# OpenDriveLab/Vista

Hardware: AMD Instinct MI355X
Metric: denoise steps/sec, 25-frame 576x1024 latent, 50-step EDM @ 1/2/4/8 GPU (higher is better)
Workload: dtype bf16; 1 GPU; 1xMI355X single GPU: 25x576x1024 (latent 25x4x72x128), 50-step EulerEDM, VanillaCFG 2.5 (N=50 images per UNet call), bf16, random-init 1.65B VideoUNet, synthetic latents; frames=25, cfg_images_per_call=50, sampler=EulerEDM s_churn=0, 50-step schedule, parallelism=single GPU

## Files before the change

### include/vista_hip.h

```cpp
#ifndef VISTA_HIP_H
#define VISTA_HIP_H
#include <stdint.h>
#ifdef __cplusplus
extern "C" {
#endif

enum { VK_AMODE_DENSE = 0, VK_AMODE_CONV3X3 = 1, VK_AMODE_TEMPORAL3 = 2, VK_AMODE_CONV3D = 3, VK_AMODE_UPCONV2X2 = 4 };
enum { VK_EPI_LINEAR = 0, VK_EPI_GEGLU = 1, VK_EPI_TRANS = 2 };

typedef struct VkGemmDesc {
    const void* A;
    const void* Wt;
    void* out;
    const float* bias;
    const float* rowvec;
    const void* res1;
    const void* res2;
    int32_t M, N, K;
    int32_t lda, ldc, ld_res1, ld_res2, ldv, rows_per_vec;
    float alpha, beta;
    int32_t amode, epi, out_f32;
    int32_t H, Wd, Cin, Hout, Wout, stride, ups;
    int32_t T, S;
    int32_t tile_cfg;
    const void* halo_prev;
    const void* halo_next;
    void* splitk_ws;
    int64_t splitk_ws_bytes;
    int32_t asym_pad;
    int32_t k_split;
    const void* A2;
    int32_t lda2;
    int32_t ln_parts;
    const float* ln_stats;
    const float* ln_colsum;
    float ln_eps;
    float* rowstat_out;
    const float* rowvec2;
    int32_t act;
    void* mx8_out;
    void* mx8_scales;
    int32_t mx8_cols, ld_mx8, ld_mx8s;
    int32_t m_begin, m_end;
    float* gnstat_out;
    int32_t gn_rows;
    int32_t alt_cols_from;
} VkGemmDesc;

int vk_gemm_bf16(const VkGemmDesc* d, void* stream);

int vk_gemm_rowstat_parts(const VkGemmDesc* d);
int vk_gemm_tile_choice(const VkGemmDesc* d);
int vk_gemm_tail_split(const VkGemmDesc* d);
int vk_gemm_gnstat_fit(const VkGemmDesc* d);

int vk_gemm_fp8(const VkGemmDesc* desc, const float* a_scale, const float* w_scale, int32_t k_real, void* stream);

typedef struct VkFp8Args {
    const float* a_scale;
    const float* w_scale;
    int32_t k_real;
    const void* a_mx;
    int32_t ld_mx;
    void* mx_out;
    int32_t ld_mx_out;
    int32_t a_scale_rows;
} VkFp8Args;
int vk_gemm_fp8_mx(const VkGemmDesc* desc, const VkFp8Args* args, void* stream);
int vk_gemm_fp8_rowstat_parts(const VkGemmDesc* d);

int vk_ff_fused_bf16(const VkGemmDesc* geglu, const VkGemmDesc* out_proj, void* stream);
int vk_ff_fused_rowstat_parts(void);

int vk_groupnorm_silu_fp8(const void* x1, const void* x2, void* y8, float* scale_out, const float* gamma, const float* beta, float* stats_ws,
                          int32_t n_img, int32_t S, int32_t C1, int32_t C2, int32_t frames_per_group, float eps, int32_t silu, void* stream);

int vk_layernorm_quant_fp8(const void* x, void* q, float* scale, const float* gamma, const float* beta, int32_t rows, int32_t C, float eps,
                           void* stream);

int vk_quantize_rows_fp8(const void* x, void* q, float* scale, int32_t M, int32_t K, int64_t ldx, int64_t ldq, void* stream);

int vk_attn_spatial_bf16(const void* q, const void* k, const void* vt, void* o, int32_t n_img, int32_t heads,
                         int32_t S, int32_t ldq, int32_t ldk, int32_t ldo, float scale, void* stream);

int vk_attn_spatial_qkv_bf16(const void* q, const void* k, const void* v, void* o, int32_t n_img, int32_t heads,
                             int32_t S, int32_t ldq, int32_t ldk, int32_t ldv, int32_t ldo, float scale, void* stream);

int vk_attn_spatial_qkv_log2_bf16(const void* q, const void* k, const void* v, void* o, int32_t n_img, int32_t heads,
                                  int32_t S, int32_t ldq, int32_t ldk, int32_t ldv, int32_t ldo, void* stream);

int vk_attn_small_bf16(const void* qkv, void* o, int32_t n_img, int32_t heads, int32_t S, int32_t D, int32_t ld, int32_t k_off,
                       int32_t v_off, int32_t ldo, float scale, void* stream);

int vk_clip_preprocess_patches(const float* img, void* out, int32_t n_img, int32_t H, int32_t W, int32_t out_hw, int32_t patch, int32_t ldo,
                               float sigma_y, float sigma_x, int32_t ks_y, int32_t ks_x, const float* mean3, const float* std3, void* stream);

int vk_attn_spatial_fp8qk(const void* q8, const void* k8, const void* q_scales, const void* k_scales, const void* v, void* o, void* o8,
                          void* o_scales, int32_t n_img, int32_t heads, int32_t S, int32_t ldq8, int32_t ldk8, int32_t ldqs, int32_t ldks,
                          int32_t ldv, int32_t ldo, int32_t ldo8, int32_t ldos, float scale, void* stream);

int vk_attn_temporal_bf16(const void* qkv, void* o, int32_t B, int32_t T, int32_t S, int32_t heads, int32_t ld,
                          int32_t k_off, int32_t v_off, int32_t ldo, float scale, void* stream);

int vk_softmax_rows_f32_bf16(const float* x, void* y, int64_t rows, int32_t cols, int64_t ldx, int64_t ldy, void* stream);

int vk_groupnorm_silu_bf16(const void* x, void* y, const float* gamma, const float* beta, float* stats_ws,
                           int32_t n_img, int32_t S, int32_t C, int32_t frames_per_group, float eps, int32_t silu,
                           void* stream);

int vk_groupnorm_stats_bf16(const void* x, float* sums, float* partial_ws, int32_t n_img, int32_t S, int32_t C,
                            int32_t frames_per_group, void* stream);
int vk_groupnorm_apply_bf16(const void* x, void* y, const float* gamma, const float* beta, const float* sums, int32_t n_img,
                            int32_t S, int32_t C, int32_t frames_per_group, float count, float eps, int32_t silu, void* stream);
int vk_groupnorm_finalize_partials(float* partial, float* sums, int32_t n_img, int32_t nchunks, int32_t frames_per_group, void* stream);
int vk_groupnorm_fold_max(void);
int vk_groupnorm_apply_partials_bf16(const void* x, void* y, const float* gamma, const float* beta, const float* partial, int32_t n_img,
                                     int32_t S, int32_t C, int32_t nchunks, int32_t frames_per_group, float count, float eps, int32_t silu,
                                     void* stream);

int vk_layernorm_bf16(const void* x, void* y, void* sum_out, const float* gamma, const float* beta,
                      const float* addvec, int32_t rows, int32_t C, int32_t rows_per_vec, int32_t ldv, float eps,
                      void* stream);

int vk_rowstats_bf16(const void* x, float* stats, int32_t rows, int32_t C, int64_t ldx, void* stream);

int vk_groupnorm_silu_cat_bf16(const void* x1, const void* x2, void* y, const float* gamma, const float* beta, float* stats_ws,
                               int32_t n_img, int32_t S, int32_t C1, int32_t C2, int32_t frames_per_group, float eps, int32_t silu,
                               void* stream);

int vk_concat_channels_bf16(const void* a, const void* b, void* out, int64_t rows, int32_t C1, int32_t C2, void* stream);

int vk_nchw_to_tokens_bf16(const float* x, void* out, int32_t n_img, int32_t C, int32_t HW, int32_t Cpad, void* stream);
int vk_tokens_to_nchw_f32(const float* x, float* out, int32_t n_img, int32_t C, int32_t HW, int32_t ldx, void* stream);

int vk_timestep_embedding_bf16(const float* t, void* out, int32_t n, int32_t dim, float max_period, void* stream);
int vk_timestep_embedding_f32(const float* t, float* out, int32_t n, int32_t dim, float max_period, void* stream);

int vk_emb_combine(const float* a, const float* b, const float* c, const float* mask, float* emb, void* silu_out,
                   int32_t n, int32_t dim, void* stream);

int vk_silu_f32_to_bf16(const float* x, void* y, int64_t count, void* stream);
int vk_cast_f32_to_bf16(const float* x, void* y, int64_t count, void* stream);

int vk_sampler_prepare(float* x, const float* cond_frame, const float* mask, const float* concat_uc,
                       const float* concat_c, void* net_in, int32_t T, int32_t HW, int32_t Cpad, float c_in,
                       int32_t replace, void* stream);
int vk_sampler_update(float* x, const float* net_out, const float* scale, int32_t T, int32_t HW, int32_t ld,
                      float c_out, float c_skip, float sigma, float sigma_next, void* stream);
int vk_sampler_update_2m(float* x, const float* net_out, const float* scale, float* hist, int32_t T, int32_t HW, int32_t ld,
                         float c_out, float c_skip, float a, float b, float c, int32_t first, void* stream);
int vk_dpmpp2m_step(const float* x, const float* den, const float* den_old, float* out, float a, float b, float c, int64_t n,
                    void* stream);

int vk_denoiser_combine(const float* net, const float* x, const float* c_out, const float* c_skip, float* out,
                        int32_t n_img, int32_t chw, void* stream);
int vk_cfg_combine(const float* x2, const float* scale, float* out, int32_t T, int32_t chw, void* stream);
int vk_euler_step(const float* x, const float* den, const float* sigma, const float* sigma_next, float* out,
                  int32_t n_img, int32_t chw, void* stream);
int vk_mask_replace(const float* x, const float* cond, const float* mask, float* out, int32_t n_img, int32_t chw,
                    void* stream);
int vk_scale_rows(const float* x, const float* s, float* out, int32_t n_img, int32_t chw, void* stream);

int vk_gaussian_sample(const float* moments, const float* noise, float* out, int32_t n_img, int32_t C, int32_t hw, float scale,
                       void* stream);

int vk_ensemble_variance_sum(const float* x, double* out, double* partial_ws, int32_t E, int64_t n, void* stream);

int vk_lanczos_resize_u8(const void* src, void* tmp, float* out, const int32_t* bounds_x, const int32_t* coef_x, int32_t ksize_x,
                         const int32_t* bounds_y, const int32_t* coef_y, int32_t ksize_y, const float* lut256, int32_t n_img,
                         int32_t src_h, int32_t src_w, int32_t left, int32_t top, int32_t crop_h, int32_t crop_w, int32_t out_h,
                         int32_t out_w, void* stream);
// ... 83 lines not shown
```

### vista_amd/_lib.py

```python
import ctypes as C
import os

_HERE = os.path.dirname(os.path.abspath(__file__))
ACT_DTYPE = os.environ.get("VISTA_ACT_DTYPE", "bf16").lower()
if ACT_DTYPE not in ("bf16", "fp16"):
    raise ValueError(f"VISTA_ACT_DTYPE must be 'bf16' or 'fp16', not {ACT_DTYPE!r}")
CURRENT = ACT_DTYPE
_LIB_FILES = {"bf16": "libvista_hip.so", "fp16": "libvista_hip_f16.so"}
LIB_PATH = os.environ.get("VISTA_HIP_LIB") or os.path.join(_HERE, "lib", _LIB_FILES[ACT_DTYPE])


def lib_path(dtype_name):
    return LIB_PATH if dtype_name == ACT_DTYPE else os.path.join(_HERE, "lib", _LIB_FILES[dtype_name])


_vp = C.c_void_p
_i32 = C.c_int32
_i64 = C.c_int64
_f32 = C.c_float


class VkFp8Args(C.Structure):
    _fields_ = [("a_scale", _vp), ("w_scale", _vp), ("k_real", _i32), ("a_mx", _vp), ("ld_mx", _i32), ("mx_out", _vp), ("ld_mx_out", _i32),
                ("a_scale_rows", _i32)]


class VkGemmDesc(C.Structure):
    _fields_ = [
        ("A", _vp), ("Wt", _vp), ("out", _vp), ("bias", _vp), ("rowvec", _vp), ("res1", _vp), ("res2", _vp),
        ("M", _i32), ("N", _i32), ("K", _i32),
        ("lda", _i32), ("ldc", _i32), ("ld_res1", _i32), ("ld_res2", _i32), ("ldv", _i32), ("rows_per_vec", _i32),
        ("alpha", _f32), ("beta", _f32),
        ("amode", _i32), ("epi", _i32), ("out_f32", _i32),
        ("H", _i32), ("Wd", _i32), ("Cin", _i32), ("Hout", _i32), ("Wout", _i32), ("stride", _i32), ("ups", _i32),
        ("T", _i32), ("S", _i32), ("tile_cfg", _i32), ("halo_prev", _vp), ("halo_next", _vp), ("splitk_ws", _vp), ("splitk_ws_bytes", _i64), ("asym_pad", _i32),
        ("k_split", _i32), ("A2", _vp), ("lda2", _i32),
        ("ln_parts", _i32), ("ln_stats", _vp), ("ln_colsum", _vp), ("ln_eps", _f32),
        ("rowstat_out", _vp), ("rowvec2", _vp), ("act", _i32),
        ("mx8_out", _vp), ("mx8_scales", _vp), ("mx8_cols", _i32), ("ld_mx8", _i32), ("ld_mx8s", _i32),
        ("m_begin", _i32), ("m_end", _i32),
        ("gnstat_out", _vp), ("gn_rows", _i32),
        ("alt_cols_from", _i32),
    ]


VK_RESHARD_MAX_BOXES = 32


class VkRowBox(C.Structure):
    _fields_ = [("src_row", _i64), ("dst_row", _i64), ("src_stride_b", _i64), ("src_stride_t", _i64), ("dst_stride_b", _i64), ("dst_stride_t", _i64),
                ("nb", _i32), ("nt", _i32), ("ns", _i32), ("reserved", _i32)]


class VkRowBoxes(C.Structure):
    _fields_ = [("n", _i32), ("reserved", _i32), ("box", VkRowBox * VK_RESHARD_MAX_BOXES)]


VK_OVERLAY_MAX_SETS, VK_OVERLAY_MAX_STROKES, VK_OVERLAY_MAX_SEGMENTS = 8, 32, 64


class VkStrokeSegment(C.Structure):
    _fields_ = [("ax", _f32), ("ay", _f32), ("bx", _f32), ("by", _f32), ("inv_len2", _f32)]


class VkStroke(C.Structure):
    _fields_ = [("color", _f32 * 3), ("alpha", _f32), ("r", _f32), ("seg_begin", _i32), ("seg_count", _i32)]


class VkStrokeSet(C.Structure):
    _fields_ = [("stroke_begin", _i32), ("stroke_count", _i32)]


class VkStrokePlan(C.Structure):
    _fields_ = [("n_sets", _i32), ("n_strokes", _i32), ("n_segments", _i32), ("reserved", _i32), ("set", VkStrokeSet * VK_OVERLAY_MAX_SETS),
                ("stroke", VkStroke * VK_OVERLAY_MAX_STROKES), ("seg", VkStrokeSegment * VK_OVERLAY_MAX_SEGMENTS)]


class VkJpegQuant(C.Structure):
    _fields_ = [("quality", _i32), ("reserved", _i32), ("luma", C.c_uint16 * 64), ("chroma", C.c_uint16 * 64)]


ABI_VERSION = 9

SIGNATURES = {
    "vk_gemm_bf16": [C.POINTER(VkGemmDesc), _vp],
    "vk_gemm_rowstat_parts": [C.POINTER(VkGemmDesc)],
    "vk_gemm_tile_choice": [C.POINTER(VkGemmDesc)],
    "vk_gemm_tail_split": [C.POINTER(VkGemmDesc)],
    "vk_gemm_gnstat_fit": [C.POINTER(VkGemmDesc)],
    "vk_gemm_fp8": [C.POINTER(VkGemmDesc), _vp, _vp, _i32, _vp],
    "vk_gemm_fp8_mx": [C.POINTER(VkGemmDesc), C.POINTER(VkFp8Args), _vp],
    "vk_gemm_fp8_rowstat_parts": [C.POINTER(VkGemmDesc)],
    "vk_ff_fused_bf16": [C.POINTER(VkGemmDesc), C.POINTER(VkGemmDesc), _vp],
    "vk_ff_fused_rowstat_parts": [],
    "vk_layernorm_quant_fp8": [_vp, _vp, _vp, _vp, _vp, _i32, _i32, _f32, _vp],
    "vk_groupnorm_silu_fp8": [_vp, _vp, _vp, _vp, _vp, _vp, _vp, _i32, _i32, _i32, _i32, _i32, _f32, _i32, _vp],
    "vk_quantize_rows_fp8": [_vp, _vp, _vp, _i32, _i32, _i64, _i64, _vp],
    "vk_attn_spatial_bf16": [_vp, _vp, _vp, _vp, _i32, _i32, _i32, _i32, _i32, _i32, _f32, _vp],
    "vk_attn_spatial_qkv_bf16": [_vp, _vp, _vp, _vp, _i32, _i32, _i32, _i32, _i32, _i32, _i32, _f32, _vp],
    "vk_attn_spatial_qkv_log2_bf16": [_vp, _vp, _vp, _vp, _i32, _i32, _i32, _i32, _i32, _i32, _i32, _vp],
    "vk_attn_spatial_fp8qk": [_vp, _vp, _vp, _vp, _vp, _vp, _vp, _vp, _i32, _i32, _i32, _i32, _i32, _i32, _i32, _i32, _i32, _i32, _i32, _f32, _vp],
    "vk_attn_small_bf16": [_vp, _vp, _i32, _i32, _i32, _i32, _i32, _i32, _i32, _i32, _f32, _vp],
    "vk_clip_preprocess_patches": [_vp, _vp, _i32, _i32, _i32, _i32, _i32, _i32, _f32, _f32, _i32, _i32, C.POINTER(_f32), C.POINTER(_f32), _vp],
    "vk_attn_temporal_bf16": [_vp, _vp, _i32, _i32, _i32, _i32, _i32, _i32, _i32, _i32, _f32, _vp],
    "vk_softmax_rows_f32_bf16": [_vp, _vp, _i64, _i32, _i64, _i64, _vp],
    "vk_groupnorm_silu_bf16": [_vp, _vp, _vp, _vp, _vp, _i32, _i32, _i32, _i32, _f32, _i32, _vp],
    "vk_groupnorm_stats_bf16": [_vp, _vp, _vp, _i32, _i32, _i32, _i32, _vp],
    "vk_groupnorm_apply_bf16": [_vp, _vp, _vp, _vp, _vp, _i32, _i32, _i32, _i32, _f32, _f32, _i32, _vp],
    "vk_groupnorm_finalize_partials": [_vp, _vp, _i32, _i32, _i32, _vp],
    "vk_groupnorm_fold_max": [],
    "vk_groupnorm_apply_partials_bf16": [_vp, _vp, _vp, _vp, _vp, _i32, _i32, _i32, _i32, _i32, _f32, _f32, _i32, _vp],
    "vk_layernorm_bf16": [_vp, _vp, _vp, _vp, _vp, _vp, _i32, _i32, _i32, _i32, _f32, _vp],
    "vk_rowstats_bf16": [_vp, _vp, _i32, _i32, _i64, _vp],
    "vk_groupnorm_silu_cat_bf16": [_vp, _vp, _vp, _vp, _vp, _vp, _i32, _i32, _i32, _i32, _i32, _f32, _i32, _vp],
    "vk_concat_channels_bf16": [_vp, _vp, _vp, _i64, _i32, _i32, _vp],
    "vk_nchw_to_tokens_bf16": [_vp, _vp, _i32, _i32, _i32, _i32, _vp],
    "vk_tokens_to_nchw_f32": [_vp, _vp, _i32, _i32, _i32, _i32, _vp],
    "vk_timestep_embedding_bf16": [_vp, _vp, _i32, _i32, _f32, _vp],
    "vk_timestep_embedding_f32": [_vp, _vp, _i32, _i32, _f32, _vp],
    "vk_emb_combine": [_vp, _vp, _vp, _vp, _vp, _vp, _i32, _i32, _vp],
    "vk_silu_f32_to_bf16": [_vp, _vp, _i64, _vp],
    "vk_cast_f32_to_bf16": [_vp, _vp, _i64, _vp],
    "vk_sampler_prepare": [_vp, _vp, _vp, _vp, _vp, _vp, _i32, _i32, _i32, _f32, _i32, _vp],
    "vk_sampler_update": [_vp, _vp, _vp, _i32, _i32, _i32, _f32, _f32, _f32, _f32, _vp],
    "vk_sampler_update_2m": [_vp, _vp, _vp, _vp, _i32, _i32, _i32, _f32, _f32, _f32, _f32, _f32, _i32, _vp],
    "vk_dpmpp2m_step": [_vp, _vp, _vp, _vp, _f32, _f32, _f32, _i64, _vp],
    "vk_denoiser_combine": [_vp, _vp, _vp, _vp, _vp, _i32, _i32, _vp],
    "vk_cfg_combine": [_vp, _vp, _vp, _i32, _i32, _vp],
    "vk_euler_step": [_vp, _vp, _vp, _vp, _vp, _i32, _i32, _vp],
    "vk_mask_replace": [_vp, _vp, _vp, _vp, _i32, _i32, _vp],
    "vk_scale_rows": [_vp, _vp, _vp, _i32, _i32, _vp],
    "vk_gaussian_sample": [_vp, _vp, _vp, _i32, _i32, _i32, _f32, _vp],
    "vk_ensemble_variance_sum": [_vp, _vp, _vp, _i32, _i64, _vp],
    "vk_lanczos_resize_u8": [_vp, _vp, _vp, _vp, _vp, _i32, _vp, _vp, _i32, _vp, _i32, _i32, _i32, _i32, _i32, _i32, _i32, _i32, _i32, _vp],
    "vk_frames_to_u8": [_vp, _vp, _i32, _i32, _i32, _i32, _i32, _i32, _vp],
    "vk_ensemble_frame_stats": [_vp, _vp, _vp, _vp, _i32, _i32, _i32, _i32, _vp],
    "vk_candidate_frame_stats": [_vp, _vp, _vp, _vp, _vp, _vp, _i32, _i32, _i32, _i32, _i32, _i32, _vp],
    "vk_heat_overlay_u8": [_vp, _vp, _vp, _i32, _i32, _i32, _i32, _f32, _f32, _vp],
    "vk_frame_fidelity_ws_bytes": [_i32, _i32],
    "vk_frame_fidelity_u8": [_vp, _vp, _vp, _vp, _vp, C.POINTER(_f32), _i32, _i32, _i32, _vp],
    "vk_copy_row_boxes": [_vp, _vp, C.POINTER(VkRowBoxes), _i64, _i64, _i32, _vp],
    "vk_stroke_overlay_u8": [_vp, _vp, _vp, C.POINTER(VkStrokePlan), _i32, _i32, _i32, _vp],
    "vk_loss_noise_input": [_vp, _vp, _vp, _vp, _vp, _f32, _vp, _i32, _i32, _i32, _vp],
    "vk_fourier_highpass_lds_bytes": [_i32, _i32],
    "vk_fourier_highpass": [_vp, _vp, _vp, _vp, _f32, _vp, _i32, _i32, _i32, _i32, _vp],
    "vk_loss_stats": [_vp, _vp, _vp, _vp, _vp, _vp, _i32, _i32, _i32, _i32, _i32, _vp],
    "vk_jpeg_dct_quant_u8": [_vp, _vp, C.POINTER(VkJpegQuant), _i32, _i32, _i32, _vp],
    "vk_jpeg_interval_sizes": [_vp, _vp, _i32, _i32, _i32, _i32, _vp],
    "vk_jpeg_entropy_write": [_vp, _vp, _vp, _i64, _i32, _i32, _i32, _i32, _vp],
    "vk_abi_version": [],
    "vk_act_dtype": [],
}

_libs = {}


class VistaHipError(RuntimeError):
    pass


def load(dtype_name=None):
    name = CURRENT if dtype_name is None else dtype_name
    lib = _libs.get(name)
    if lib is not None:
# ... 25 lines not shown
```

### vista_amd/csrc/gemm.hip

```cpp
#include <stdlib.h>

#include "common.h"
#include "vista_hip.h"

#include "gemm_common.h"

extern "C" int vk_gemm_pipe_fit(const VkGemmDesc* d);
extern "C" int vk_gemm_pipe_launch(const VkGemmDesc* d, void* stream, int ksplit);
extern "C" int vk_gemm_pipe_gnstat_ok(const VkGemmDesc* d, int ksplit);
extern "C" int vk_gemm_pipe2_fit(const VkGemmDesc* d);
extern "C" int vk_gemm_pipe2_launch(const VkGemmDesc* d, void* stream);
extern "C" int vk_gemm_stream_fit(const VkGemmDesc* d);
extern "C" int vk_gemm_stream_launch(const VkGemmDesc* d, void* stream);

namespace {

constexpr int TILE5_MAX_K_DEFAULT = 320;

__device__ uint4 g_zero16;

template <int AMODE, int EPI, bool OUT_F32, int WM, int WN, int FM, int FN>
__global__ __launch_bounds__(WM * WN * 64, (WM * WN == 16) ? 4 : 2) void gemm_kernel(const VkGemmDesc p, const int ksplit) {
    constexpr int BM = WM * FM * 32, BN = WN * FN * 32;
    constexpr int NT = WM * WN * 64;
// ... 284 lines not shown
            v[0] += b.x; v[1] += b.y; v[2] += b.z; v[3] += b.w;
        }
        if (p.rowvec) {
            const float4 b = *(const float4*)(p.rowvec + (size_t)(m / p.rows_per_vec) * p.ldv + n);
            v[0] += b.x; v[1] += b.y; v[2] += b.z; v[3] += b.w;
        }
        if (res1) {
            const uint2 r = *(const uint2*)(res1 + (size_t)m * p.ld_res1 + n);
            v[0] += bf16_lo(r.x); v[1] += bf16_hi(r.x); v[2] += bf16_lo(r.y); v[3] += bf16_hi(r.y);
        }
#pragma unroll
        for (int e = 0; e < 4; ++e) v[e] *= p.alpha;
        if (res2) {
            const uint2 r = *(const uint2*)(res2 + (size_t)m * p.ld_res2 + n);
            float t[4] = {bf16_lo(r.x), bf16_hi(r.x), bf16_lo(r.y), bf16_hi(r.y)};
            if (p.rowvec2) {
                const float4 b = *(const float4*)(p.rowvec2 + (size_t)(m / p.rows_per_vec) * p.ldv + n);
                t[0] += b.x; t[1] += b.y; t[2] += b.z; t[3] += b.w;
            }
            v[0] = fmaf(p.beta, t[0], v[0]); v[1] = fmaf(p.beta, t[1], v[1]); v[2] = fmaf(p.beta, t[2], v[2]); v[3] = fmaf(p.beta, t[3], v[3]);
        }
        if (OUT_F32) *(float4*)((float*)p.out + (size_t)m * p.ldc + n) = make_float4(v[0], v[1], v[2], v[3]);
        else *(uint2*)((uint16_t*)p.out + (size_t)m * p.ldc + n) = make_uint2(pack_bf16(v[0], v[1]), pack_bf16(v[2], v[3]));
    }
}

template <int AMODE, int EPI, bool OUT_F32, int WM, int WN, int FM, int FN>
int launch_cfg(const VkGemmDesc* d, hipStream_t stream, int ksplit = 1) {
    constexpr int BM = WM * FM * 32, BN = WN * FN * 32;
    const int tilesN = (d->N + BN - 1) / BN;
    const int tilesM = (d->m_end - d->m_begin + BM - 1) / BM;
    VkGemmDesc desc = *d;
    desc.tile_cfg = (desc.tile_cfg & ~32) | ((AMODE == AMODE_DENSE && tilesN <= 4) ? 32 : 0);
    int grid = tilesM * tilesN * ksplit;
    if (EPI == EPI_GEGLU) {
        const int resident = 256 * ((WM * WN == 16) ? 1 : 2);
        if (grid > resident) grid = resident;
    }
    hipLaunchKernelGGL((gemm_kernel<AMODE, EPI, OUT_F32, WM, WN, FM, FN>), dim3(grid), dim3(WM * WN * 64), 0, stream, desc, ksplit);
    VK_CHECK_LAUNCH();
    return VK_OK;
}

int launch_splitk_finish(const VkGemmDesc* d, hipStream_t stream, int ksplit) {
    const long long quads = (long long)d->M * (d->N >> 2);
    const int grid = (int)((quads + 255) / 256 < 4096 ? (quads + 255) / 256 : 4096);
    if (d->out_f32) hipLaunchKernelGGL((splitk_finish_kernel<true>), dim3(grid), dim3(256), 0, stream, *d, ksplit);
    else hipLaunchKernelGGL((splitk_finish_kernel<false>), dim3(grid), dim3(256), 0, stream, *d, ksplit);
    VK_CHECK_LAUNCH();
    return VK_OK;
}

struct TileChoice { int cfg, ksplit; };

inline bool cfg5_ok(const VkGemmDesc* d) { return d->amode == AMODE_DENSE && d->epi == EPI_LINEAR && !d->out_f32 && (d->N % 160) == 0; }
inline TileChoice choose_tile(const VkGemmDesc* d, bool rowstat, bool gnstat) {
    static const int tile5_max_k = [] { const char* e = getenv("VISTA_TILE5_MAXK"); return e ? atoi(e) : TILE5_MAX_K_DEFAULT; }();
    const int amode = d->amode, epi = d->epi;
    const int force = d->tile_cfg & 7;
    if ((d->tile_cfg & 16) && force == 0 && !gnstat && vk_gemm_pipe2_fit(d)) return {7, 1};
    int cfg = force;
    if (d->mx8_out) cfg = 4;
    if (cfg == 5 && !cfg5_ok(d)) cfg = 4;
    if (cfg == 7 && !vk_gemm_pipe_fit(d)) cfg = 4;
    if (cfg == 4 && amode == AMODE_CONV3D) cfg = 3;
    if (cfg == 0) {
        const int rows = d->m_end - d->m_begin;
        auto wgs = [&](int bm, int bn) { return (long long)((rows + bm - 1) / bm) * ((d->N + bn - 1) / bn); };
        const int n256 = (d->N + 255) / 256 * 256;
        const bool ok320 = (epi != EPI_GEGLU) && (amode != AMODE_CONV3D) && (d->N % 320 == 0);
        const bool ok256 = n256 * 10 <= d->N * 11;
        const long long need = 192;
        if (cfg5_ok(d) && tile5_max_k > 0 && d->K <= tile5_max_k && d->N <= d->K && wgs(128, 160) >= 1024) cfg = 5;
        else if (ok320 && wgs(256, 320) >= need) cfg = 4;
        else if (ok256 && wgs(256, 256) >= need) cfg = 3;
        else if (wgs(256, 128) >= need) cfg = 2;
        else cfg = 1;
        if (epi == EPI_GEGLU && amode == AMODE_DENSE && (d->N % 320) == 0 && cfg == 3) {
            const long long r3 = (wgs(256, 256) + 255) / 256, r4 = (wgs(256, 320) + 255) / 256;
            if (r4 * 320 * 100 < r3 * 256 * (d->K >= 640 ? 103 : 95)) cfg = 4;
        }
        if (cfg5_ok(d) && cfg != 5 && tile5_max_k > 0 && wgs(128, 160) >= need) {
            int bm = 256, bn = 320, slots = 256;
            if (cfg == 3) bn = 256;
            else if (cfg == 2) bn = 128;
            else if (cfg == 1) { bm = 128; bn = 128; slots = 512; }
            const long long w = wgs(bm, bn), rounds = (w + slots - 1) / slots;
            if (w * 100 < rounds * slots * 75) cfg = 5;
        }
    }
    int ksplit = 1;
    if (epi == EPI_LINEAR && force == 0 && d->splitk_ws && cfg != 4 && cfg != 3 && cfg != 5 && !d->ln_stats && !rowstat && !d->act && !d->alt_cols_from &&
        d->m_begin == 0 && d->m_end == d->M) {
        const bool ok320s = (amode != AMODE_CONV3D) && (d->N % 320 == 0);
        const int bn = ok320s ? 320 : 256;
        const long long tiles = (long long)((d->m_end - d->m_begin + 255) / 256) * ((d->N + bn - 1) / bn);
        const int nk = d->K / BK;
        int s = (int)(256 / tiles);
        if (s > 8) s = 8;
        if (s > nk / 8) s = nk / 8;
        if (s >= 2 && tiles * s >= 128 && (long long)s * d->M * d->N * 4 <= d->splitk_ws_bytes) {
            ksplit = s;
            cfg = ok320s ? 4 : 3;
        }
    }
    static const bool pipe_on = [] { const char* e = getenv("VISTA_GEMM_PIPE"); return !e || atoi(e) != 0; }();
    if (cfg == 4 && force == 0 && pipe_on && !d->out_f32 && vk_gemm_pipe_fit(d)) cfg = 7;
    if (epi == EPI_GEGLU && (cfg == 3 || cfg == 4) && force == 0 && pipe_on && d->K >= 640 && vk_gemm_pipe_fit(d)) cfg = 7;
    if (epi == EPI_GEGLU && cfg == 7 && force == 0 && d->K < 640) cfg = 3;
    return {cfg, ksplit};
}

inline void tile_geometry(int cfg, int& bn, int& wn) {
    if (cfg == 5) { bn = 160; wn = 1; }
    else if (cfg == 4 || cfg == 7) { bn = 320; wn = 2; }
    else if (cfg == 3) { bn = 256; wn = 4; }
    else if (cfg == 2) { bn = 128; wn = 4; }
    else { bn = 128; wn = 2; }
}

inline int tail_split_row(const VkGemmDesc* d, const TileChoice& t) {
    const int max_pct = 40;
    if (!(d->tile_cfg & 64) || t.cfg != 7 || t.ksplit != 1 || (d->tile_cfg & 7) != 0 || d->epi != EPI_LINEAR || d->out_f32 || (d->N % 320) != 0) return 0;
    const int rows = d->m_end - d->m_begin;
    const long long tilesN = d->N / 320, tilesM = (rows + 255) / 256, ntiles = tilesM * tilesN;
    const long long full = ntiles / 256, rem = ntiles % 256;
    if (full == 0 || rem == 0 || rem * 100 > (long long)max_pct * 256) return 0;
    const long long tm_main = full * 256 / tilesN;
    if (tm_main <= 0 || tm_main >= tilesM) return 0;
    const int m_split = d->m_begin + (int)tm_main * 256;
    const long long small = (long long)((d->m_end - m_split + 127) / 128) * (d->N / 160);
    if (small > 512) return 0;
    return m_split;
}

inline bool pipe2_wanted(const VkGemmDesc* d, const TileChoice& t, bool gnstat) {
    if (!(d->tile_cfg & 16) || gnstat || t.ksplit != 1 || d->amode != AMODE_DENSE || d->out_f32) return false;
    if (d->epi == EPI_LINEAR && t.cfg != 4 && t.cfg != 5 && t.cfg != 7) return false;
    return vk_gemm_pipe2_fit(d) != 0;
}

enum GemmFamily { FAM_NONE = -1, FAM_STREAM, FAM_PIPE2, FAM_PIPE, FAM_TILED };
struct GemmPlan {
    int family;
    int cfg;
    int ksplit;
    int tail_row;
    int rowstat_slabs;
    int gnstat_slots;
};

GemmPlan plan_gemm(VkGemmDesc& d, bool rowstat, bool gnstat) {
    static const bool stream_on = [] { const char* e = getenv("VISTA_GEMM_STREAM"); return !e || atoi(e) != 0; }();
    const int force = d.tile_cfg & 7;
    if (d.amode == AMODE_UPCONV2X2) {
        VkGemmDesc nine = d;
        nine.amode = AMODE_CONV3X3;
        nine.K = 9 * d.Cin;
        nine.tile_cfg &= ~8;
        const TileChoice t = choose_tile(&nine, false, false);
        const bool ok = t.cfg == 7 && t.ksplit == 1 && !rowstat && !gnstat && vk_gemm_pipe_fit(&d);
        return {ok ? FAM_PIPE : FAM_NONE, 7, 1, 0, 0, 0};
    }
    if (d.m_begin == 0 && d.m_end == d.M && !(d.tile_cfg & 16) && (force == 6 || (stream_on && !rowstat))) {
        if (const int fit = vk_gemm_stream_fit(&d)) return {FAM_STREAM, 6, 1, 0, d.N / (32 * fit), 0};
    }
    if (force == 6) d.tile_cfg &= ~7;
    const TileChoice t = choose_tile(&d, rowstat, gnstat);
    GemmPlan p{FAM_TILED, t.cfg, t.ksplit, 0, 0, 0};
    if (pipe2_wanted(&d, t, gnstat)) p.family = FAM_PIPE2;
    else if (t.cfg == 7) p.family = FAM_PIPE;
    if (p.family == FAM_PIPE) p.tail_row = tail_split_row(&d, t);
    int bn, wn;
    tile_geometry(t.cfg, bn, wn);
    p.rowstat_slabs = ((d.N + bn - 1) / bn) * wn;
    if (p.family == FAM_PIPE && p.ksplit == 1 && p.tail_row == 0 && !rowstat && vk_gemm_pipe_gnstat_ok(&d, 1)) p.gnstat_slots = d.M / 64;
    return p;
}

template <int AMODE, int EPI, bool OUT_F32>
int launch(const VkGemmDesc* d, hipStream_t stream, int cfg, int ksplit) {
    if constexpr (EPI == EPI_LINEAR && !OUT_F32 && AMODE != AMODE_CONV3D) {
        if (cfg == 5) return launch_cfg<AMODE, EPI, OUT_F32, 4, 1, 1, 5>(d, stream);
    }
    if constexpr (AMODE != AMODE_CONV3D) {
        if (cfg == 4) return launch_cfg<AMODE, EPI, OUT_F32, 8, 2, 1, 5>(d, stream, ksplit);
    }
    if (cfg == 3) return launch_cfg<AMODE, EPI, OUT_F32, 4, 4, 2, 2>(d, stream, ksplit);
    if (cfg == 2) return launch_cfg<AMODE, EPI, OUT_F32, 4, 4, 2, 1>(d, stream);
    return launch_cfg<AMODE, EPI, OUT_F32, 4, 2, 1, 2>(d, stream);
}

int launch_tiled(const VkGemmDesc* d, hipStream_t stream, int cfg, int ksplit) {
    const bool f32 = d->out_f32 != 0;
    switch (d->epi) {
        case EPI_LINEAR:
            if (d->amode == AMODE_DENSE) return f32 ? launch<AMODE_DENSE, EPI_LINEAR, true>(d, stream, cfg, ksplit) : launch<AMODE_DENSE, EPI_LINEAR, false>(d, stream, cfg, ksplit);
            if (d->amode == AMODE_CONV3X3) return f32 ? launch<AMODE_CONV3X3, EPI_LINEAR, true>(d, stream, cfg, ksplit) : launch<AMODE_CONV3X3, EPI_LINEAR, false>(d, stream, cfg, ksplit);
            if (d->amode == AMODE_TEMPORAL3) return f32 ? launch<AMODE_TEMPORAL3, EPI_LINEAR, true>(d, stream, cfg, ksplit) : launch<AMODE_TEMPORAL3, EPI_LINEAR, false>(d, stream, cfg, ksplit);
            if (d->amode == AMODE_CONV3D) return f32 ? launch<AMODE_CONV3D, EPI_LINEAR, true>(d, stream, cfg, ksplit) : launch<AMODE_CONV3D, EPI_LINEAR, false>(d, stream, cfg, ksplit);
            return VK_EINVAL;
        case EPI_GEGLU: return launch<AMODE_DENSE, EPI_GEGLU, false>(d, stream, cfg, ksplit);
        case EPI_TRANS: return launch<AMODE_DENSE, EPI_TRANS, false>(d, stream, cfg, ksplit);
    }
    return VK_EINVAL;
}

inline int check_epilogue(const VkGemmDesc* d) {
    if (d->epi == EPI_LINEAR) return (d->ldc % 4) != 0 ? VK_EINVAL : VK_OK;
    if (d->amode != AMODE_DENSE || d->out_f32) return VK_EINVAL;
    if (d->epi == EPI_GEGLU) return (d->N % 32) != 0 ? VK_EINVAL : VK_OK;
    if (d->epi == EPI_TRANS) return (d->S <= 0 || (d->S % 4) != 0) ? VK_EINVAL : VK_OK;
    return VK_EINVAL;
}

int run_plan(const VkGemmDesc* d, const GemmPlan& p, hipStream_t stream) {
    if (p.family == FAM_STREAM) return vk_gemm_stream_launch(d, stream);
    int rc = check_epilogue(d);
    if (rc != VK_OK) return rc;
    if (p.family == FAM_PIPE2) return vk_gemm_pipe2_launch(d, stream);
    if (p.family == FAM_PIPE && p.tail_row) {
        VkGemmDesc head = *d, tail = *d;
        head.m_end = p.tail_row;
        tail.m_begin = p.tail_row;
        rc = vk_gemm_pipe_launch(&head, stream, 1);
        return rc != VK_OK ? rc : launch_tiled(&tail, stream, 5, 1);
    }
    rc = (p.family == FAM_PIPE) ? vk_gemm_pipe_launch(d, stream, p.ksplit) : launch_tiled(d, stream, p.cfg, p.ksplit);
    if (rc != VK_OK || p.ksplit == 1) return rc;
    return launch_splitk_finish(d, stream, p.ksplit);
}

inline int validate(const VkGemmDesc* d) {
    if (!d || !d->A || !d->Wt || !d->out) return VK_EINVAL;
    const int upc_bits = d->amode == AMODE_UPCONV2X2 ? 8 : 0;
    if (d->M <= 0 || d->N <= 0 || d->K <= 0 || (d->K % BK) != 0 || (d->N % 4) != 0 || d->tile_cfg < 0 || (d->tile_cfg & ~(64 | 16 | upc_bits)) > 7) return VK_EINVAL;
    if (d->amode < AMODE_DENSE || d->amode > AMODE_UPCONV2X2) return VK_EINVAL;
    if (d->m_begin < 0 || d->m_end < 0 || d->m_end > d->M || (d->m_end != 0 && d->m_begin >= d->m_end) || (d->m_end == 0 && d->m_begin >= d->M)) return VK_EINVAL;
    if ((d->m_begin != 0 || (d->m_end != 0 && d->m_end != d->M)) && d->epi == EPI_TRANS) return VK_EINVAL;
    if (d->amode != AMODE_DENSE && (d->Cin <= 0 || (d->Cin % BK) != 0)) return VK_EINVAL;
    if (d->amode == AMODE_DENSE && (d->lda % 8) != 0) return VK_EINVAL;
    if (d->amode == AMODE_CONV3X3 && (d->K != 9 * d->Cin || d->stride < 1 || d->stride > 2 || d->ups < 1 || d->ups > 2)) return VK_EINVAL;
    if (d->amode == AMODE_TEMPORAL3 && (d->K != 3 * d->Cin || d->T <= 0 || d->S <= 0)) return VK_EINVAL;
    if (d->amode == AMODE_UPCONV2X2) {
        if (d->K != 4 * d->Cin || d->ups != 2 || d->stride != 1 || d->asym_pad || d->H <= 0 || d->Wd <= 0 || d->Hout != 2 * d->H || d->Wout != 2 * d->Wd) return VK_EINVAL;
        const long long hw4 = 4ll * d->H * d->Wd;
        if ((d->M % hw4) != 0 || (d->rowvec && d->rows_per_vec != hw4)) return VK_EINVAL;
        if (d->epi != EPI_LINEAR || d->out_f32 || d->res1 || d->res2 || d->rowvec2 || d->gnstat_out || d->rowstat_out || d->mx8_out || d->ln_stats || d->A2 ||
            d->halo_prev || d->halo_next || d->act || d->alt_cols_from)
            return VK_EINVAL;
        if (d->m_begin != 0 || (d->m_end != 0 && d->m_end != d->M)) return VK_EINVAL;
        if ((d->tile_cfg & (64 | 16)) != 0 || ((d->tile_cfg & 7) != 0 && (d->tile_cfg & 7) != 7)) return VK_EINVAL;
    }
    if (d->amode == AMODE_CONV3D && (d->K != 27 * d->Cin || d->T <= 0 || d->H <= 0 || d->Wd <= 0 || d->H >= 4096 || d->Wd >= 4096 ||
                                     (long long)d->M != (long long)(d->M / (d->H * d->Wd)) * d->H * d->Wd)) return VK_EINVAL;
    if ((d->rowvec || d->rowvec2) && d->rows_per_vec <= 0) return VK_EINVAL;
    if (d->rowvec2 && (!d->res2 || d->epi != EPI_LINEAR)) return VK_EINVAL;
    if (d->A2 && (d->amode != AMODE_DENSE || d->k_split <= 0 || d->k_split >= d->K || (d->k_split % BK) != 0 || (d->lda2 % 8) != 0)) return VK_EINVAL;
    if (d->ln_stats && (d->amode != AMODE_DENSE || d->A2 || !d->ln_colsum || d->ln_parts <= 0 || d->ln_parts > 64 || !(d->ln_eps > 0.f))) return VK_EINVAL;
    if (d->rowstat_out && (d->epi != EPI_LINEAR || d->out_f32)) return VK_EINVAL;
    if (d->act != 0 && (d->act != 1 || d->epi != EPI_LINEAR)) return VK_EINVAL;
    if (d->mx8_out && (!d->mx8_scales || d->epi != EPI_LINEAR || d->out_f32 || (d->N % 320) != 0 || d->mx8_cols <= 0 || (d->mx8_cols % 320) != 0 ||
                       d->mx8_cols > d->N || (d->ld_mx8 % 16) != 0 || d->ld_mx8 < d->mx8_cols || d->ld_mx8s * 32 < d->mx8_cols ||
                       (((size_t)d->mx8_out) & 15) != 0 || d->rowstat_out || (d->ldc % 8) != 0 || (((size_t)d->out) & 15) != 0 ||
                       (d->amode != AMODE_DENSE) || d->res1 || d->res2 || d->rowvec || d->rowvec2 ||
                       (unsigned long long)d->M * 2ull * (unsigned)d->ldc >= 0xfffff000ull))
        return VK_EINVAL;
    if (d->alt_cols_from != 0 && (d->alt_cols_from < 0 || (d->alt_cols_from % 32) != 0 || d->alt_cols_from >= d->N || d->epi != EPI_LINEAR || d->out_f32 ||
                                  d->rowstat_out || d->gnstat_out || d->mx8_out))
        return VK_EINVAL;
    return operands_ok(d) ? VK_OK : VK_EINVAL;
}

int plan_for(const VkGemmDesc* d, VkGemmDesc& q, bool rowstat, bool gnstat, GemmPlan& p) {
    const int rc = validate(d);
    if (rc != VK_OK) return rc;
    q = *d;
    norm_row_range(q);
    p = plan_gemm(q, rowstat || q.rowstat_out != nullptr, gnstat || q.gnstat_out != nullptr);
    return p.family == FAM_NONE ? VK_EINVAL : VK_OK;
}

}

extern "C" int vk_gemm_rowstat_parts(const VkGemmDesc* d) {
    VkGemmDesc q;
    GemmPlan p;
    const int rc = plan_for(d, q, true, false, p);
    if (rc != VK_OK) return rc;
    return (q.epi != EPI_LINEAR || q.out_f32) ? VK_EINVAL : p.rowstat_slabs;
}

extern "C" int vk_gemm_tile_choice(const VkGemmDesc* d) {
    VkGemmDesc q;
    GemmPlan p;
    const int rc = plan_for(d, q, false, false, p);
    return rc != VK_OK ? rc : p.cfg * 16 + p.ksplit;
}

extern "C" int vk_gemm_tail_split(const VkGemmDesc* d) {
    VkGemmDesc q;
    GemmPlan p;
    const int rc = plan_for(d, q, false, false, p);
    return rc != VK_OK ? rc : p.tail_row;
}

extern "C" int vk_gemm_gnstat_fit(const VkGemmDesc* d) {
    VkGemmDesc q;
// ... 14 lines not shown
```

### vista_amd/csrc/gemm_common.h

```cpp
#pragma once
#include "common.h"
#include "vista_hip.h"

namespace {

enum { AMODE_DENSE = 0, AMODE_CONV3X3 = 1, AMODE_TEMPORAL3 = 2, AMODE_CONV3D = 3, AMODE_UPCONV2X2 = 4 };
enum { EPI_LINEAR = 0, EPI_GEGLU = 1, EPI_TRANS = 2 };

constexpr int BK = 64;

inline bool norm_row_range(VkGemmDesc& d) {
    if (d.m_end == 0) d.m_end = d.M;
    return d.m_begin >= 0 && d.m_begin < d.m_end && d.m_end <= d.M;
}



#ifndef VK_EPI_NT_STORES
#define VK_EPI_NT_STORES 0
#endif
__device__ __forceinline__ void epi_st16(void* p, const uint4 v) {
#if VK_EPI_NT_STORES
    typedef unsigned epi_u32x4_t __attribute__((ext_vector_type(4)));
    const epi_u32x4_t w = {v.x, v.y, v.z, v.w};
// ... 284 lines not shown
    if (p.out_f32 || epi == EPI_TRANS) return false;
    if ((p.ldc % 8) != 0 || (((size_t)p.out) & 15) != 0) return false;
    const unsigned long long lim = 0xfffff000ull, rows = (unsigned long long)p.M * 2ull;
    if (rows * (unsigned)p.ldc >= lim || (p.res1 && rows * (unsigned)p.ld_res1 >= lim) || (p.res2 && rows * (unsigned)p.ld_res2 >= lim)) return false;
    if (p.bias && (((size_t)p.bias) & 15) != 0) return false;
    if (p.ln_stats && (((size_t)p.ln_colsum) & 15) != 0) return false;
    if (epi == EPI_GEGLU) return true;
    if (p.res1 && ((p.ld_res1 % 8) != 0 || (((size_t)p.res1) & 15) != 0)) return false;
    if (p.res2 && ((p.ld_res2 % 8) != 0 || (((size_t)p.res2) & 15) != 0)) return false;
    if (p.rowvec || p.rowvec2) {
        if ((p.ldv % 4) != 0 || (p.rowvec && (((size_t)p.rowvec) & 15) != 0) || (p.rowvec2 && (((size_t)p.rowvec2) & 15) != 0)) return false;
        if ((bm - 1) / p.rows_per_vec + 2 > EPI_NI) return false;
    }
    return true;
}

inline bool epilogue_operands_ok(const VkGemmDesc* d) {
    if (!aligned_to(d->out, d->out_f32 ? 16 : 8)) return false;
    if (d->epi != EPI_TRANS && (d->ldc % 4) != 0) return false;
    if (d->res1 && (!aligned_to(d->res1, 8) || (d->ld_res1 % 4) != 0)) return false;
    if (d->res2 && (!aligned_to(d->res2, 8) || (d->ld_res2 % 4) != 0)) return false;
    const size_t vec = d->epi == EPI_TRANS ? 4 : 16;
    if (!aligned_to(d->bias, vec) || (d->ln_stats && !aligned_to(d->ln_colsum, vec))) return false;
    if ((d->rowvec || d->rowvec2) && (!aligned_to(d->rowvec, 16) || !aligned_to(d->rowvec2, 16) || (d->ldv % 4) != 0)) return false;
    if (!aligned_to(d->ln_stats, 8) || !aligned_to(d->rowstat_out, 8) || !aligned_to(d->gnstat_out, 4) || !aligned_to(d->splitk_ws, 16)) return false;
    return true;
}
inline bool operands_ok(const VkGemmDesc* d) {
    if (!aligned_to(d->A, 16) || !aligned_to(d->Wt, 16) || !aligned_to(d->A2, 16) || !aligned_to(d->halo_prev, 16) || !aligned_to(d->halo_next, 16)) return false;
    return epilogue_operands_ok(d);
}

template <int BN, int NT>
__device__ __forceinline__ void epi_stage_vectors(const VkGemmDesc& p, float* ev, int n0, const EpiPlan& e, int tid) {
    constexpr int QN = BN / 4, NSEC = 2 + 2 * EPI_NI;
#pragma unroll
    for (int idx0 = 0; idx0 < NSEC * QN; idx0 += NT) {
        const int idx = idx0 + tid;
        if (idx < NSEC * QN) {
            const int sec = idx / QN, q = idx - sec * QN;
            const float* src = nullptr;
            if (sec == 0) src = p.bias;
            else if (sec == 1) src = p.ln_stats ? p.ln_colsum : nullptr;
            else if (sec < 2 + EPI_NI) { if (p.rowvec && sec - 2 < e.nimg) src = p.rowvec + (size_t)(e.img0 + sec - 2) * p.ldv; }
            else { if (p.rowvec2 && sec - 2 - EPI_NI < e.nimg) src = p.rowvec2 + (size_t)(e.img0 + sec - 2 - EPI_NI) * p.ldv; }
            float4 v = make_float4(0.f, 0.f, 0.f, 0.f);
            if (src) v = *(const float4*)(src + n0 + 4 * q);
            *(float4*)(ev + sec * BN + 4 * q) = v;
        }
    }
}

template <int NG>
__device__ __forceinline__ void gn_reduce_store(float (&gs)[NG], float (&gq)[NG], float* __restrict__ slot, int gb, int lane, bool valid) {
    static_assert(NG == 16 || NG == 8 || NG == 4, "160-column wave tiles of 10 / 20 / 40-channel groups");
    float r[NG];
#pragma unroll
    for (int i = 0; i < NG; ++i) {
        const auto sw = __builtin_amdgcn_permlane32_swap(__builtin_bit_cast(uint32_t, gs[i]), __builtin_bit_cast(uint32_t, gq[i]), false, false);
        r[i] = __builtin_bit_cast(float, (uint32_t)sw[0]) + __builtin_bit_cast(float, (uint32_t)sw[1]);
    }
    int k = 16;
#pragma unroll
    for (int n = NG; n > 1; n >>= 1, k >>= 1) {
        const bool up = (lane & k) != 0;
#pragma unroll
        for (int i = 0; i < n / 2; ++i) {
            float lo = r[i], hi = r[i + n / 2];
            asm volatile("" : "+v"(lo), "+v"(hi));
            const float keep = up ? hi : lo;
            const float give = up ? lo : hi;
            r[i] = keep + __shfl_xor(give, k, 64);
        }
    }
#pragma unroll
    for (; k >= 1; k >>= 1) r[0] += __shfl_xor(r[0], k, 64);
    constexpr int SH = NG == 16 ? 1 : (NG == 8 ? 2 : 3);
    if (valid && (lane & ((1 << SH) - 1)) == 0) slot[32 * (lane >> 5) + gb + ((lane & 31) >> SH)] = r[0];
}

template <int CPG, int NG>
__device__ __forceinline__ void gn_accumulate_quad(float (&gs)[NG], float (&gq)[NG], const int fi, const int g, const uint2 packed, const uint32_t lo_mask) {
    constexpr uint32_t one = VK_ONE_PAIR;
#pragma unroll
    for (int h = 0; h < 2; ++h) {
        const uint32_t w = h ? packed.y : packed.x;
        const int c0 = 32 * fi + 8 * g + 2 * h;
        const int G0 = c0 / CPG, G1 = (c0 + 4) / CPG;
        if (G0 == G1) {
            gs[G0] = vk_dot2(w, one, gs[G0]);
            gq[G0] = vk_dot2(w, w, gq[G0]);
        } else {
            const uint32_t v0 = w & lo_mask, v1 = w & ~lo_mask;
            gs[G0] = vk_dot2(v0, one, gs[G0]);
            gq[G0] = vk_dot2(v0, v0, gq[G0]);
            gs[G1] = vk_dot2(v1, one, gs[G1]);
            gq[G1] = vk_dot2(v1, v1, gq[G1]);
        }
    }
}

template <int NRES, bool LN, bool MX, int FX, int FY, int FM, int FN, int BN, int CAP, int GNC = 0, bool UPC = false>
__device__ __forceinline__ void epilogue_linear_lds_body(const VkGemmDesc& p, f32x16_t (&acc)[FX][FY], int m0, int n0, int wm, int wn, int l31, int lh,
                                                         int stat_part, const float2* lnrow, const float* ev, int img0, int cls = 0) {
    constexpr int MW = FM * 32, NW = FN * 32, U = FX * FY;
    constexpr int GN_NG = GNC ? NW / GNC : 1;
    constexpr int ROOM = (CAP - 16 * U - 36) / 8;
    constexpr int DA = NRES == 0 ? 0 : ((ROOM / NRES < 1 ? 1 : ROOM / NRES) < U ? (ROOM / NRES < 1 ? 1 : ROOM / NRES) : U);
    constexpr bool mx_tile = MX;
    const bool a_is_r1 = p.res1 != nullptr;
    const uint16_t* __restrict__ ra = (const uint16_t*)(a_is_r1 ? p.res1 : p.res2);
    const uint16_t* __restrict__ rb = (const uint16_t*)p.res2;
    const int lda_ = a_is_r1 ? p.ld_res1 : p.ld_res2;
    const int c0 = wn * NW + 4 * lh;
    const int wide_off = n0 + wn * NW + 8 * lh;
    bool row_ok[FY];
    int mrow[FY];
    uint32_t rao[FY], rbo[FY], oo[FY];
    char* const outb = (char*)p.out;
#pragma unroll
    for (int fj = 0; fj < FY; ++fj) {
        const int m = m0 + wm * MW + fj * 32 + l31;
        row_ok[fj] = m < p.m_end;
        mrow[fj] = row_ok[fj] ? m : p.m_end - 1;
        if (NRES >= 1) rao[fj] = ((uint32_t)mrow[fj] * (uint32_t)lda_ + (uint32_t)wide_off) * 2u;
        if (NRES == 2) rbo[fj] = ((uint32_t)mrow[fj] * (uint32_t)p.ld_res2 + (uint32_t)wide_off) * 2u;
        if constexpr (UPC) {
            const int hw = p.H * p.Wd, img = mrow[fj] / hw, rem = mrow[fj] - img * hw, sy = rem / p.Wd, sx = rem - sy * p.Wd;
            const uint32_t orow = (uint32_t)(img * 4 * hw + (2 * sy + (cls >> 1)) * 2 * p.Wd + 2 * sx + (cls & 1));
            oo[fj] = (orow * (uint32_t)p.ldc + (uint32_t)wide_off) * 2u;
        } else
        oo[fj] = ((uint32_t)mrow[fj] * (uint32_t)p.ldc + (uint32_t)(wide_off - (p.mx8_out ? p.mx8_cols : 0))) * 2u;
    }
    static_assert(GNC == 0 || (MW % 64 == 0 && NW == 160 && NW % GNC == 0 && !MX), "gnstat_out: wave tiles of 64-row blocks x 160 columns of whole channel groups");
    float gs[GN_NG], gq[GN_NG];
    if constexpr (GNC != 0) {
#pragma unroll
        for (int i = 0; i < GN_NG; ++i) { gs[i] = 0.f; gq[i] = 0.f; }
    }
    const uint32_t gn_lo_mask = lh ? 0u : 0xffffffffu;
    uint4 wa[U][2], wb[U][2];
    auto issue = [&](int fj, int fi, int u) {
        if (NRES >= 1) { wa[u][0] = *(const uint4*)((const char*)ra + rao[fj] + fi * 64); wa[u][1] = *(const uint4*)((const char*)ra + rao[fj] + fi * 64 + 32); }
        if (NRES == 2) { wb[u][0] = *(const uint4*)((const char*)rb + rbo[fj] + fi * 64); wb[u][1] = *(const uint4*)((const char*)rb + rbo[fj] + fi * 64 + 32); }
    };
#pragma unroll
    for (int u = 0; u < DA; ++u) issue(u / FX, u % FX, u);
    __builtin_amdgcn_sched_barrier(0);
#pragma unroll
    for (int fj = 0; fj < FY; ++fj) {
        float nrm = 0.f, rs = 1.f;
        if (LN) { const float2 t = lnrow[mrow[fj] - m0]; rs = t.y; nrm = -t.x * t.y; }
        const int iv = (p.rowvec || p.rowvec2) ? mrow[fj] / p.rows_per_vec - img0 : 0;
        const float* evb = ev + c0;
        const float* evc = ev + BN + c0;
        const float* evr = ev + (2 + iv) * BN + c0;
        const float* evr2 = ev + (2 + EPI_NI + iv) * BN + c0;
        float ssum = 0.f, qsum = 0.f;
#pragma unroll
        for (int fi = 0; fi < FX; ++fi) {
            const int u = fj * FX + fi;
            uint2 packed[4], qa[4], qb[4];
            [[maybe_unused]] float vq[4][4];
            if (NRES >= 1) { unwiden_pair(wa[u][0], qa[0], qa[1]); unwiden_pair(wa[u][1], qa[2], qa[3]); }
            if (NRES == 2) { unwiden_pair(wb[u][0], qb[0], qb[1]); unwiden_pair(wb[u][1], qb[2], qb[3]); }
#pragma unroll
            for (int g = 0; g < 4; ++g) {
                const int co = fi * 32 + 8 * g;
                const float4 b = *(const float4*)(evb + co);
                const float4 rv = *(const float4*)(evr + co);
                float v[4];
#pragma unroll
                for (int e = 0; e < 4; ++e) v[e] = acc[fi][fj][4 * g + e];
                if (LN) {
                    const float4 c = *(const float4*)(evc + co);
                    v[0] = fmaf(rs, v[0], fmaf(nrm, c.x, b.x)); v[1] = fmaf(rs, v[1], fmaf(nrm, c.y, b.y));
                    v[2] = fmaf(rs, v[2], fmaf(nrm, c.z, b.z)); v[3] = fmaf(rs, v[3], fmaf(nrm, c.w, b.w));
                } else {
                    v[0] += b.x; v[1] += b.y; v[2] += b.z; v[3] += b.w;
                }
                v[0] += rv.x; v[1] += rv.y; v[2] += rv.z; v[3] += rv.w;
                if (GNC == 0 && p.act == 1) { v[0] = gelu_erf_f(v[0]); v[1] = gelu_erf_f(v[1]); v[2] = gelu_erf_f(v[2]); v[3] = gelu_erf_f(v[3]); }
                if (NRES >= 1 && a_is_r1) {
                    const uint2 r = qa[g];
                    v[0] += bf16_lo(r.x); v[1] += bf16_hi(r.x); v[2] += bf16_lo(r.y); v[3] += bf16_hi(r.y);
                }
#pragma unroll
                for (int e = 0; e < 4; ++e) v[e] *= p.alpha;
                if (NRES == 2 || (NRES == 1 && !a_is_r1)) {
                    const uint2 r = NRES == 2 ? qb[g] : qa[g];
                    const float4 b2 = *(const float4*)(evr2 + co);
                    const float t0 = bf16_lo(r.x) + b2.x, t1 = bf16_hi(r.x) + b2.y, t2 = bf16_lo(r.y) + b2.z, t3 = bf16_hi(r.y) + b2.w;
                    v[0] = fmaf(p.beta, t0, v[0]); v[1] = fmaf(p.beta, t1, v[1]); v[2] = fmaf(p.beta, t2, v[2]); v[3] = fmaf(p.beta, t3, v[3]);
                }
                if constexpr (mx_tile) {
#pragma unroll
                    for (int e = 0; e < 4; ++e) vq[g][e] = v[e];
                }
                packed[g].x = pack_out(v[0], v[1], p, n0 + wn * NW + fi * 32);
                packed[g].y = pack_out(v[2], v[3], p, n0 + wn * NW + fi * 32);
                if (GNC == 0 && p.rowstat_out) {
                    const float a0 = bf16_lo(packed[g].x), a1 = bf16_hi(packed[g].x), a2 = bf16_lo(packed[g].y), a3 = bf16_hi(packed[g].y);
                    ssum += (a0 + a1) + (a2 + a3);
                    qsum = fmaf(a0, a0, fmaf(a1, a1, fmaf(a2, a2, fmaf(a3, a3, qsum))));
                }
                if constexpr (GNC != 0) gn_accumulate_quad<GNC, GN_NG>(gs, gq, fi, g, packed[g], gn_lo_mask);
                __builtin_amdgcn_sched_barrier(0);
            }
            if constexpr (mx_tile) {
                int e8;
                const uint4 q16 = mx_quant_block(vq, e8);
                if (row_ok[fj]) {
                    const int col = n0 + wn * NW + fi * 32;
                    *(uint4*)((uint8_t*)p.mx8_out + (size_t)mrow[fj] * p.ld_mx8 + col + 16 * lh) = q16;
                    if (lh == 0) ((uint8_t*)p.mx8_scales)[(size_t)mrow[fj] * p.ld_mx8s + (col >> 5)] = (uint8_t)e8;
                }
            } else {
                const uint4 s0 = widen_pair(packed[0], packed[1]), s1 = widen_pair(packed[2], packed[3]);
                if (row_ok[fj]) {
                    epi_st16(outb + oo[fj] + fi * 64, s0);
                    epi_st16(outb + oo[fj] + fi * 64 + 32, s1);
                }
            }
            if (NRES >= 1 && u + DA < U) issue((u + DA) / FX, (u + DA) % FX, u + DA);
            __builtin_amdgcn_sched_barrier(0);
        }
        if (GNC == 0 && p.rowstat_out) {
            const float so = __shfl_xor(ssum, 32, 64), qo = __shfl_xor(qsum, 32, 64);
            if (lh == 0 && row_ok[fj]) ((float2*)p.rowstat_out)[(size_t)stat_part * p.M + mrow[fj]] = make_float2(ssum + so, qsum + qo);
        }
        if constexpr (GNC != 0 && FY > 2) {
            if ((fj & 1) == 1) {
                const int mb = m0 + wm * MW + (fj >> 1) * 64;
                gn_reduce_store<GN_NG>(gs, gq, (float*)p.gnstat_out + (size_t)(mb >> 6) * 64, (n0 + wn * NW) / GNC, l31 | (lh << 5), mb < p.m_end);
#pragma unroll
                for (int i = 0; i < GN_NG; ++i) { gs[i] = 0.f; gq[i] = 0.f; }
            }
        }
    }
    if constexpr (GNC != 0 && FY == 2) {
        const int mb = m0 + wm * MW;
        gn_reduce_store<GN_NG>(gs, gq, (float*)p.gnstat_out + (size_t)(mb >> 6) * 64, (n0 + wn * NW) / GNC, l31 | (lh << 5), mb < p.m_end);
    }
}

template <int FX, int FY, int FM, int FN, int BN, int CAP = 128, int GN_CPG = 0, int GN_NRES = 0, bool UPC = false>
__device__ __forceinline__ void gemm_epilogue_linear_lds(const VkGemmDesc& p, f32x16_t (&acc)[FX][FY], int m0, int n0, int wm, int wn, int l31, int lh,
                                                         int stat_part, const float2* lnrow, const float* ev, int img0, int cls = 0) {
    if constexpr (UPC) {
        epilogue_linear_lds_body<0, false, false, FX, FY, FM, FN, BN, CAP, 0, true>(p, acc, m0, n0, wm, wn, l31, lh, stat_part, nullptr, ev, img0, cls);
        return;
    }
    if constexpr (GN_CPG != 0) {
        epilogue_linear_lds_body<GN_NRES, false, false, FX, FY, FM, FN, BN, CAP, GN_CPG>(p, acc, m0, n0, wm, wn, l31, lh, stat_part, nullptr, ev, img0);
        return;
    }
    const int nres = (p.res1 != nullptr) + (p.res2 != nullptr);
    if constexpr (BN == 320) {
        if (p.mx8_out != nullptr && n0 < p.mx8_cols) {
            if (lnrow != nullptr) epilogue_linear_lds_body<0, true, true, FX, FY, FM, FN, BN, CAP>(p, acc, m0, n0, wm, wn, l31, lh, stat_part, lnrow, ev, img0);
            else epilogue_linear_lds_body<0, false, true, FX, FY, FM, FN, BN, CAP>(p, acc, m0, n0, wm, wn, l31, lh, stat_part, lnrow, ev, img0);
            return;
        }
    }
#define VK_EPI_BODY(NR, LNF) epilogue_linear_lds_body<NR, LNF, false, FX, FY, FM, FN, BN, CAP>(p, acc, m0, n0, wm, wn, l31, lh, stat_part, lnrow, ev, img0)
    if (lnrow != nullptr) {
        if (nres == 0) VK_EPI_BODY(0, true);
        else if (nres == 1) VK_EPI_BODY(1, true);
        else VK_EPI_BODY(2, true);
    } else {
        if (nres == 0) VK_EPI_BODY(0, false);
        else if (nres == 1) VK_EPI_BODY(1, false);
        else VK_EPI_BODY(2, false);
    }
#undef VK_EPI_BODY
}

template <int FX, int FY, int FM, int FN, int BN>
__device__ __forceinline__ void gemm_epilogue_geglu_lds(const VkGemmDesc& p, f32x16_t (&acc)[FX][FY], int m0, int n0, int wm, int wn, int l31, int lh,
                                                        const float2* lnrow, const float* ev) {
    constexpr int MW = FM * 32, NW = FN * 32;
    const bool has_ln = lnrow != nullptr;
    const float* evb = ev + wn * NW + 4 * lh;
    const float* evc = evb + BN;
#pragma unroll
    for (int fj = 0; fj < FY; ++fj) {
        const int m = m0 + wm * MW + fj * 32 + l31;
        const bool row_ok = m < p.m_end;
        const int mc = row_ok ? m : p.m_end - 1;
        float nrm = 0.f, rs = 1.f;
        if (has_ln) { const float2 t = lnrow[mc - m0]; rs = t.y; nrm = -t.x * t.y; }
        uint16_t* op = (uint16_t*)p.out + (size_t)mc * p.ldc + ((n0 + wn * NW) >> 1) + 8 * lh;
#pragma unroll
        for (int fi = 0; fi < FX; ++fi) {
            uint2 packed[2];
#pragma unroll
            for (int g = 0; g < 2; ++g) {
                const int co = fi * 32 + 8 * g;
                float a[4], gt[4];
#pragma unroll
                for (int e = 0; e < 4; ++e) { a[e] = acc[fi][fj][4 * g + e]; gt[e] = acc[fi][fj][4 * (g + 2) + e]; }
                const float4 ba = *(const float4*)(evb + co), bg = *(const float4*)(evb + co + 16);
                if (has_ln) {
// ... 20 lines not shown
```

### vista_amd/csrc/gemm_pipe.hip

```cpp
#include "common.h"
#include "vista_hip.h"

#include "gemm_common.h"

namespace {

constexpr int PBM = 256, PBN = 320, PNT = 512;
constexpr int PFX = 5, PFY = 2;
constexpr int PRPP = PNT / 8;
constexpr int PAP = PBM / PRPP, PWP = PBN / PRPP;
constexpr int PA_BYTES = PBM * 128, PSTAGE = (PBM + PBN) * 128;
constexpr int PCAP = 256;
constexpr int APAR0 = 6 * PAP;
typedef unsigned amask_t;
constexpr unsigned P_OOB = 0xffffff00u;
constexpr unsigned long long P_LIMIT = 0xfffff000ull;
static_assert(PAP + PWP <= PFX * PFY && 8 * PAP <= 32, "the piece schedule issues one piece after each MFMA of the first k-substep");

typedef __attribute__((address_space(3))) void* lptr_t;

#define PIPE_MMA(FI, X, Y, C) C = vk_mfma(X, Y, C)

#define PIPE_SB() __builtin_amdgcn_sched_barrier(0)

template <int AMODE, int EPI, bool NT_A, bool SPLIT, int GN_CPG = 0, int GN_NRES = 0, bool PF = false>
__global__ __launch_bounds__(PNT, 2) void gemm_pipe_kernel(const VkGemmDesc p, const int ksplit) {
    static_assert(!PF || AMODE == AMODE_DENSE, "the L2 prefetch is written for the dense loader");
    constexpr int LN_OFF = 2 * PSTAGE, EV_OFF = LN_OFF + PBM * 8;
    constexpr int NTAPS = (AMODE == AMODE_CONV3X3) ? 9 : (AMODE == AMODE_TEMPORAL3) ? 3 : (AMODE == AMODE_UPCONV2X2) ? 4 : 1;
    constexpr bool UPC = (AMODE == AMODE_UPCONV2X2);
    static_assert(!UPC || (EPI == EPI_LINEAR && !SPLIT && GN_CPG == 0), "the folded upsample convolution: plain LINEAR epilogue, one launch");
    constexpr bool WALK = (EPI == EPI_GEGLU);
    __shared__ __attribute__((aligned(16))) char smem[2 * PSTAGE + PBM * 8 + epi_vec_floats(PBN) * 4];
#ifdef PIPE_TIMING
    unsigned long long tm_k0, tm_dma = 0, tm_bar = 0, tm_loop = 0, tm_epi = 0, tm_ksteps = 0;
    asm volatile("s_memtime %0\n s_waitcnt lgkmcnt(0)" : "=s"(tm_k0) :: "memory");
#endif

    const int tilesN = p.N / PBN;
    const int tilesM = (p.m_end - p.m_begin + PBM - 1) / PBM;
    const int ntiles = tilesM * tilesN;
    const int tid = threadIdx.x;
    const int lane = tid & 63, wave = tid >> 6;
    const int wm = wave >> 1, wn = wave & 1;
    const int l31 = lane & 31, lh = lane >> 5;
    int kslice = 0;
    int cls = 0;
    auto tile_of = [&](const int bid, int& tm, int& tn) __attribute__((always_inline)) {
        int logical = xcd_remap(bid, SPLIT ? ntiles * ksplit : UPC ? ntiles * 4 : ntiles);
        if (SPLIT) { kslice = logical / ntiles; logical -= kslice * ntiles; }
        if (UPC) {
            if (p.tile_cfg & 8) { cls = logical & 3; logical >>= 2; }
            else { cls = logical / ntiles; logical -= cls * ntiles; }
        }
        if (tilesN < 8 || (long long)p.N * p.K * 2 <= (3LL << 20)) {
            tn = logical % tilesN;
            tm = logical / tilesN;
        } else {
            constexpr int GM = 8;
            const int panel = logical / (GM * tilesN), r = logical - panel * (GM * tilesN);
            const int gm = (tilesM - panel * GM < GM) ? tilesM - panel * GM : GM;
            tm = panel * GM + r % gm;
            tn = r / gm;
        }
        if constexpr (AMODE == AMODE_TEMPORAL3) {
            if (p.tile_cfg & 8) return;
            const int nblk = p.S / PBM;
            if (nblk * PBM == p.S && p.m_begin == 0 && tilesM == (p.M / p.S) * nblk && (long long)p.S * p.Cin * 2 > (3LL << 20)) {
                const int per_clip = p.T * nblk, clip = tm / per_clip, r = tm - clip * per_clip;
                const int j = r / p.T, t = r - j * p.T;
                tm = clip * per_clip + t * nblk + j;
            }
        }
    };

    const int lc = tid & 7, lr = tid >> 3;
    const int lsrc = lc ^ ((lr >> 1) & 7);
    const int wave_u = __builtin_amdgcn_readfirstlane(wave);
    const unsigned voff_w = ((unsigned)lr * (unsigned)p.K + (unsigned)lsrc * 8u) * 2u;
    const unsigned wpass = (unsigned)PRPP * (unsigned)p.K * 2u;
    const unsigned apass = (unsigned)PRPP * (unsigned)(AMODE == AMODE_DENSE ? p.lda : p.Cin) * 2u;

    __amdgpu_buffer_rsrc_t rw, ra;
    unsigned voff_a[PAP];
// ... 265 lines not shown
        const int nbid = bid + (int)gridDim.x;
        const bool more = WALK && nbid < ntiles;
        int ntm = 0, ntn = 0;
        if (more) {
            tile_of(nbid, ntm, ntn);
            setup(p.m_begin + ntm * PBM, ntn * PBN);
            kb = 0; tap = 0; c0b = 0;
#pragma unroll
            for (int q = 0; q < PWP + PAP; ++q) dma_q(q, st ^ 1);
            dma_next();
        }
        PIPE_SB();

        int te = tid;
        asm volatile("" : "+v"(te));
        const int e_wave = te >> 6, e_l31 = te & 31, e_lh = (te >> 5) & 1;
        const int e_wm = e_wave >> 1, e_wn = e_wave & 1;
        const float2* const lnp = p.ln_stats != nullptr ? lnrow : nullptr;
        if constexpr (SPLIT) {
            VkGemmDesc q = p;
            q.out = (float*)p.splitk_ws + (size_t)kslice * p.M * p.N;
            q.ldc = p.N;
            q.bias = nullptr; q.rowvec = nullptr; q.res1 = nullptr; q.res2 = nullptr;
            q.alpha = 1.f; q.beta = 0.f;
            q.rowvec2 = nullptr; q.ln_stats = nullptr; q.rowstat_out = nullptr; q.act = 0;
            gemm_epilogue<EPI_LINEAR, true, PFX, PFY, PFY, 5>(q, acc, m0, n0, e_wm, e_wn, e_l31, e_lh);
        } else if constexpr (EPI == EPI_GEGLU) gemm_epilogue_geglu_lds<PFX, PFY, PFY, 5, PBN>(p, acc, m0, n0, e_wm, e_wn, e_l31, e_lh, lnp, epi_vec);
        else gemm_epilogue_linear_lds<PFX, PFY, PFY, 5, PBN, PCAP, GN_CPG, GN_NRES, UPC>(p, acc, m0, n0, e_wm, e_wn, e_l31, e_lh, tn * 2 + e_wn, lnp, epi_vec, eplan.img0, cls);
#ifdef PIPE_TIMING
        unsigned long long tm_t2;
        asm volatile("s_memtime %0\n s_waitcnt lgkmcnt(0)" : "=s"(tm_t2) :: "memory");
        tm_epi += tm_t2 - tm_t1;
#endif
        if (!more) break;
        __syncthreads();
        bid = nbid; tm = ntm; tn = ntn;
        m0 = p.m_begin + tm * PBM; n0 = tn * PBN;
        eplan = plan_of(m0);
        stage_tile_vectors(m0, n0, eplan);
        __syncthreads();
        st ^= 1;
    }
    if constexpr (PF) asm volatile("" :: "v"(pf_dummy));
#ifdef PIPE_TIMING
    if (blockIdx.x == 8 && lane == 0 && p.splitk_ws) {
        unsigned long long tm_end;
        asm volatile("s_waitcnt vmcnt(0)\n s_memtime %0\n s_waitcnt lgkmcnt(0)" : "=s"(tm_end) :: "memory");
        float* o = (float*)p.splitk_ws + wave * 8;
        o[0] = (float)tm_dma; o[1] = (float)tm_bar; o[2] = (float)tm_ksteps; o[3] = (float)tm_loop; o[4] = (float)tm_epi; o[5] = (float)(tm_end - tm_k0);
    }
#endif
}

template <int AMODE, int EPI>
int pipe_launch(const VkGemmDesc* d, hipStream_t stream, int ksplit) {
    const int tilesN = d->N / PBN, tilesM = (d->m_end - d->m_begin + PBM - 1) / PBM;
    const int ntiles = tilesM * tilesN;
    const bool nt_a = (AMODE == AMODE_DENSE && tilesN <= 4);
    if constexpr (EPI == EPI_LINEAR) {
        if (ksplit > 1) {
            if (nt_a) hipLaunchKernelGGL((gemm_pipe_kernel<AMODE, EPI, AMODE == AMODE_DENSE, true>), dim3(ntiles * ksplit), dim3(PNT), 0, stream, *d, ksplit);
            else hipLaunchKernelGGL((gemm_pipe_kernel<AMODE, EPI, false, true>), dim3(ntiles * ksplit), dim3(PNT), 0, stream, *d, ksplit);
            VK_CHECK_LAUNCH();
            return VK_OK;
        }
    }
    if (ksplit > 1) return VK_EINVAL;
    const int grid = (EPI == EPI_GEGLU && ntiles > 256) ? 256 : ntiles;
    if constexpr (EPI == EPI_LINEAR && AMODE != AMODE_DENSE) {
        if (d->gnstat_out) {
            const int nres = (d->res1 != nullptr) + (d->res2 != nullptr);
#define VK_PIPE_GN(CPG, NR) hipLaunchKernelGGL((gemm_pipe_kernel<AMODE, EPI, false, false, CPG, NR>), dim3(grid), dim3(PNT), 0, stream, *d, 1)
            if (d->N == 320) { if (nres == 0) VK_PIPE_GN(10, 0); else VK_PIPE_GN(10, 1); }
            else if (d->N == 640) { if (nres == 0) VK_PIPE_GN(20, 0); else VK_PIPE_GN(20, 1); }
            else { if (nres == 0) VK_PIPE_GN(40, 0); else VK_PIPE_GN(40, 1); }
#undef VK_PIPE_GN
            VK_CHECK_LAUNCH();
            return VK_OK;
        }
    }
    if constexpr (AMODE == AMODE_DENSE) {
        if (ntiles <= 256 && d->K >= 3 * BK && (d->lda % 64) == 0 && (((size_t)d->A) & 127) == 0) {
            if (nt_a) hipLaunchKernelGGL((gemm_pipe_kernel<AMODE, EPI, true, false, 0, 0, true>), dim3(grid), dim3(PNT), 0, stream, *d, 1);
            else hipLaunchKernelGGL((gemm_pipe_kernel<AMODE, EPI, false, false, 0, 0, true>), dim3(grid), dim3(PNT), 0, stream, *d, 1);
            VK_CHECK_LAUNCH();
            return VK_OK;
        }
    }
    if (nt_a) hipLaunchKernelGGL((gemm_pipe_kernel<AMODE, EPI, AMODE == AMODE_DENSE, false>), dim3(grid), dim3(PNT), 0, stream, *d, 1);
    else hipLaunchKernelGGL((gemm_pipe_kernel<AMODE, EPI, false, false>), dim3(grid), dim3(PNT), 0, stream, *d, 1);
    VK_CHECK_LAUNCH();
    return VK_OK;
}

inline VkGemmDesc upconv_class_desc(const VkGemmDesc* d) {
    VkGemmDesc q = *d;
    q.M = d->M / 4;
    q.m_begin = 0;
    q.m_end = q.M;
    q.rows_per_vec = d->H * d->Wd;
    return q;
}

int upconv_fit(const VkGemmDesc* d) {
    if (d->epi != EPI_LINEAR || d->out_f32 || (d->N % PBN) != 0 || d->mx8_out || d->A2 || d->res1 || d->res2 || d->rowvec2 || d->gnstat_out || d->rowstat_out ||
        d->ln_stats || d->act || d->alt_cols_from || d->halo_prev || d->halo_next)
        return 0;
    if (d->m_begin != 0 || (d->m_end != 0 && d->m_end != d->M)) return 0;
    VkGemmDesc q = *d;
    q.rows_per_vec = d->H * d->Wd;
    if (!epi_fast_everywhere(q, EPI_LINEAR, PBM)) return 0;
    if ((unsigned long long)PBN * d->K * 2ull >= P_LIMIT) return 0;
    return ((unsigned long long)(d->M / 4) * d->Cin * 2ull < P_LIMIT) ? 1 : 0;
}

int upconv_launch(const VkGemmDesc* d, hipStream_t stream) {
    const VkGemmDesc q = upconv_class_desc(d);
    const int tilesN = q.N / PBN, tilesM = (q.M + PBM - 1) / PBM;
    hipLaunchKernelGGL((gemm_pipe_kernel<AMODE_UPCONV2X2, EPI_LINEAR, false, false>), dim3(4 * tilesM * tilesN), dim3(PNT), 0, stream, q, 1);
    VK_CHECK_LAUNCH();
    return VK_OK;
}

}

extern "C" int vk_gemm_pipe_fit(const VkGemmDesc* d) {
    if (d->amode == AMODE_UPCONV2X2) return upconv_fit(d);
    if ((d->epi != EPI_LINEAR && d->epi != EPI_GEGLU) || d->out_f32 || (d->N % PBN) != 0 || d->mx8_out || d->A2) return 0;
    if (d->epi == EPI_GEGLU && d->amode != AMODE_DENSE) return 0;
    if (!epi_fast_everywhere(*d, d->epi, PBM)) return 0;
    if ((unsigned long long)PBN * d->K * 2ull >= P_LIMIT) return 0;
    if (d->amode == AMODE_DENSE) return ((unsigned long long)PBM * d->lda * 2ull < P_LIMIT) ? 1 : 0;
    if (d->amode == AMODE_CONV3X3) {
        if (d->ups == 2 && (d->stride != 1 || d->asym_pad)) return 0;
        const long long hw = (long long)d->Hout * d->Wout;
        if (hw <= 0 || (d->M % hw) != 0) return 0;
        return ((unsigned long long)(d->M / hw) * d->H * d->Wd * d->Cin * 2ull < P_LIMIT) ? 1 : 0;
    }
    if (d->amode == AMODE_TEMPORAL3) {
        if (d->halo_prev || d->halo_next) return 0;
        return ((unsigned long long)d->M * d->Cin * 2ull < P_LIMIT) ? 1 : 0;
    }
    return 0;
}

extern "C" int vk_gemm_pipe_gnstat_ok(const VkGemmDesc* d, int ksplit) {
    if (!vk_gemm_pipe_fit(d) || ksplit != 1 || d->epi != EPI_LINEAR || d->out_f32) return 0;
    if (d->amode != AMODE_CONV3X3 && d->amode != AMODE_TEMPORAL3) return 0;
    if (d->N != 320 && d->N != 640 && d->N != 1280) return 0;
    if (d->ln_stats || d->mx8_out || d->act || d->rowstat_out || (d->res1 && d->res2)) return 0;
    if (d->gn_rows <= 0 || (d->gn_rows % 64) != 0 || (d->M % d->gn_rows) != 0) return 0;
    if (d->m_begin != 0 || (d->m_end != 0 && d->m_end != d->M)) return 0;
    return 1;
}

extern "C" int vk_gemm_pipe_launch(const VkGemmDesc* d, void* stream_, int ksplit) {
    hipStream_t stream = (hipStream_t)stream_;
    if (!vk_gemm_pipe_fit(d)) return VK_EINVAL;
    if (d->amode == AMODE_UPCONV2X2) return ksplit == 1 ? upconv_launch(d, stream) : VK_EINVAL;
    if (ksplit > 1 && (d->epi != EPI_LINEAR || !d->splitk_ws || d->ln_stats || d->rowstat_out || d->act)) return VK_EINVAL;
    if (d->gnstat_out && !vk_gemm_pipe_gnstat_ok(d, ksplit)) return VK_EINVAL;
    if (d->amode == AMODE_DENSE) return d->epi == EPI_GEGLU ? pipe_launch<AMODE_DENSE, EPI_GEGLU>(d, stream, ksplit) : pipe_launch<AMODE_DENSE, EPI_LINEAR>(d, stream, ksplit);
    if (d->amode == AMODE_CONV3X3) return pipe_launch<AMODE_CONV3X3, EPI_LINEAR>(d, stream, ksplit);
    if (d->amode == AMODE_TEMPORAL3) return pipe_launch<AMODE_TEMPORAL3, EPI_LINEAR>(d, stream, ksplit);
    return VK_EINVAL;
}
```

### vista_amd/csrc/norm.hip

```cpp
#include <stdlib.h>

#include "common.h"
#include "vista_hip.h"

namespace {

constexpr int GN_TOK = 128;
constexpr bool GN_PIVOT = VK_F16 != 0;

__device__ __forceinline__ float gn_pivot(const uint16_t* __restrict__ x, const uint16_t* __restrict__ x2, int C1, int C, int S, int img0, int c0) {
    const bool second = x2 != nullptr && c0 >= C1;
    const int ld = x2 == nullptr ? C : (second ? C - C1 : C1);
    return bf16_to_f32((second ? x2 + (c0 - C1) : x + c0)[((size_t)img0 * S) * ld]);
}

template <bool AMAX, bool PIVOT>
__global__ void gn_stats_kernel(const uint16_t* __restrict__ x, const uint16_t* __restrict__ x2, int C1, float* __restrict__ partial, int S, int C,
                                int CG, int R, int tok_per_wg, float* __restrict__ amax_part, int frames_per_group) {
    __shared__ float wave_amax[16];
    extern __shared__ float lds[];
    const int tid = threadIdx.x;
    const int img = blockIdx.y;
    const int tok0 = blockIdx.x * tok_per_wg;
    const int tok1 = min(tok0 + tok_per_wg, S);
// ... 77 lines not shown
        dst[32 + tid] = b;
    }
}

__global__ void gn_finalize_kernel(float* __restrict__ partial, float* __restrict__ sums, int nparts, int per, int in_place) {
    __shared__ float red[4][64];
    const int v = threadIdx.x & 63, j = threadIdx.x >> 6;
    const int first = blockIdx.y * per;
    const int cnt = min(per, nparts - first);
    float* src = partial + ((size_t)blockIdx.x * nparts + first) * 64 + v;
    float a = 0.f;
    for (int i = j; i < cnt; i += 4) a += src[(size_t)i * 64];
    red[j][v] = a;
    __syncthreads();
    if (threadIdx.x < 64) {
        const float t = (red[0][v] + red[1][v]) + (red[2][v] + red[3][v]);
        if (in_place) src[0] = t;
        else sums[(size_t)blockIdx.x * 64 + v] = t;
    }
}

__global__ void gn_finalize_level2_kernel(const float* __restrict__ partial, float* __restrict__ sums, int nparts, int per, int splits) {
    __shared__ float red[4][64];
    const int v = threadIdx.x & 63, j = threadIdx.x >> 6;
    const float* src = partial + (size_t)blockIdx.x * nparts * 64 + v;
    float a = 0.f;
    for (int i = j; i < splits; i += 4) a += src[(size_t)i * per * 64];
    red[j][v] = a;
    __syncthreads();
    if (threadIdx.x < 64) sums[(size_t)blockIdx.x * 64 + v] = (red[0][v] + red[1][v]) + (red[2][v] + red[3][v]);
}

typedef unsigned gn_u32x4_t __attribute__((ext_vector_type(4)));
template <bool NT>
__device__ __forceinline__ uint4 gn_ld16(const uint16_t* p) {
    if constexpr (NT) {
        const gn_u32x4_t v = __builtin_nontemporal_load((const gn_u32x4_t*)p);
        return make_uint4(v[0], v[1], v[2], v[3]);
    } else {
        return *(const uint4*)p;
    }
}
template <bool NT>
__device__ __forceinline__ void gn_st16(uint16_t* p, const uint4 v) {
    if constexpr (NT) {
        const gn_u32x4_t w = {v.x, v.y, v.z, v.w};
        __builtin_nontemporal_store(w, (gn_u32x4_t*)p);
    } else {
        *(uint4*)p = v;
    }
}

constexpr int GN_FOLD_MAX = 256;
template <bool NTL, bool NTS, bool FOLD, bool PIVOT>
__global__ void gn_apply_kernel(const uint16_t* __restrict__ x, const uint16_t* __restrict__ x2, int C1, uint16_t* __restrict__ y, const float* __restrict__ gamma,
                                const float* __restrict__ beta, const float* __restrict__ stats, int S, int C, int CG, int R,
                                int frames_per_group, float inv_cnt, float eps, int do_silu, int tok_per_wg, int nparts) {
    __shared__ float fold_red[FOLD ? 4 : 1][64];
    __shared__ float fold_tot[64];
    const int tid = threadIdx.x;
    const int img = blockIdx.y;
    const int tok0 = blockIdx.x * tok_per_wg;
    const int tok1 = min(tok0 + tok_per_wg, S);
    const int chunk = tid % CG, r = tid / CG;
    const float* st = stats + (size_t)(img / frames_per_group) * 64;
    if constexpr (FOLD) {
        const float* src = stats + (size_t)(img / frames_per_group) * nparts * 64;
        for (int idx = tid; idx < 256; idx += blockDim.x) {
            const int v = idx & 63, j = idx >> 6;
            float a = 0.f;
            for (int i = j; i < nparts; i += 4) a += src[(size_t)i * 64 + v];
            fold_red[j][v] = a;
        }
        __syncthreads();
        if (tid < 64) fold_tot[tid] = (fold_red[0][tid] + fold_red[1][tid]) + (fold_red[2][tid] + fold_red[3][tid]);
        __syncthreads();
        st = fold_tot;
    }
    if (r >= R) return;
    const int cpg = C >> 5;
    float a[8], b[8];
#pragma unroll
    for (int e = 0; e < 8; ++e) {
        const int c = chunk * 8 + e;
        const int g = c / cpg;
        float mean = st[g] * inv_cnt;
        const float var = fmaxf(st[32 + g] * inv_cnt - mean * mean, 0.f);
        if constexpr (PIVOT) mean += gn_pivot(x, x2, C1, C, S, (img / frames_per_group) * frames_per_group, g * cpg);
        a[e] = gamma[c] * rsqrtf(var + eps);
        b[e] = beta[c] - mean * a[e];
    }
    const size_t base = ((size_t)img * S) * C + chunk * 8;
    const bool second = x2 != nullptr && chunk * 8 >= C1;
    const int ld = x2 == nullptr ? C : (second ? C - C1 : C1);
    const uint16_t* xs = (second ? x2 + (chunk * 8 - C1) : x + chunk * 8) + ((size_t)img * S) * ld;
    int t = tok0 + r;
    for (; t + 3 * R < tok1; t += 4 * R) {
        uint4 v[4];
#pragma unroll
        for (int u = 0; u < 4; ++u) v[u] = gn_ld16<NTL>(xs + (size_t)(t + u * R) * ld);
#pragma unroll
        for (int u = 0; u < 4; ++u) {
            float f[8];
            unpack8(v[u], f);
#pragma unroll
            for (int e = 0; e < 8; ++e) {
                const float w = fmaf(f[e], a[e], b[e]);
                f[e] = do_silu ? silu_f(w) : w;
            }
            gn_st16<NTS>(y + base + (size_t)(t + u * R) * C, pack8(f));
        }
    }
    for (; t < tok1; t += R) {
        const uint4 v = gn_ld16<NTL>(xs + (size_t)t * ld);
        float f[8];
        unpack8(v, f);
#pragma unroll
        for (int e = 0; e < 8; ++e) {
            const float w = fmaf(f[e], a[e], b[e]);
// ... 250 lines not shown
    g.tok = (g.R >= 2) ? GN_TOK : 32;
    g.nchunks = (S + g.tok - 1) / g.tok;
    g.ngroups = n_img / fpg;
    return true;
}
}

namespace {
int gn_finalize(float* partial_ws, float* sums, int ngroups, int nparts, hipStream_t stream) {
    if (nparts <= 256) {
        hipLaunchKernelGGL(gn_finalize_kernel, dim3(ngroups), dim3(256), 0, stream, partial_ws, sums, nparts, nparts, 0);
    } else {
        int per = 16;
        while ((long long)per * per < nparts) per += 4;
        const int splits = (nparts + per - 1) / per;
        hipLaunchKernelGGL(gn_finalize_kernel, dim3(ngroups, splits), dim3(256), 0, stream, partial_ws, sums, nparts, per, 1);
        VK_CHECK_LAUNCH();
        hipLaunchKernelGGL(gn_finalize_level2_kernel, dim3(ngroups), dim3(256), 0, stream, (const float*)partial_ws, sums, nparts, per, splits);
    }
    VK_CHECK_LAUNCH();
    return VK_OK;
}

int gn_stats(const void* x, const void* x2, int C1, float* sums, float* partial_ws, int32_t n_img, int32_t S, int32_t C, int32_t frames_per_group,
             void* stream_, float* amax_part = nullptr, bool finalize = true, bool pivot = false) {
    hipStream_t stream = (hipStream_t)stream_;
    GnGeom g;
    if (!x || !sums || !partial_ws || !gn_geom(n_img, S, C, frames_per_group, g) || (pivot && amax_part)) return VK_EINVAL;
    if (!aligned_to(x, 16) || !aligned_to(x2, 16) || !aligned_to(sums, 4) || !aligned_to(partial_ws, 4) || !aligned_to(amax_part, 4)) return VK_EINVAL;
    dim3 grid(g.nchunks, n_img);
    const size_t lds_bytes = (size_t)2 * g.R * C * sizeof(float);
    if (amax_part)
        hipLaunchKernelGGL((gn_stats_kernel<true, false>), grid, dim3(g.threads), lds_bytes, stream, (const uint16_t*)x, (const uint16_t*)x2, C1, partial_ws,
                           S, C, g.CG, g.R, g.tok, amax_part, frames_per_group);
    else if (pivot)
        hipLaunchKernelGGL((gn_stats_kernel<false, GN_PIVOT>), grid, dim3(g.threads), lds_bytes, stream, (const uint16_t*)x, (const uint16_t*)x2, C1, partial_ws,
                           S, C, g.CG, g.R, g.tok, (float*)nullptr, frames_per_group);
    else
        hipLaunchKernelGGL((gn_stats_kernel<false, false>), grid, dim3(g.threads), lds_bytes, stream, (const uint16_t*)x, (const uint16_t*)x2, C1, partial_ws,
                           S, C, g.CG, g.R, g.tok, (float*)nullptr, frames_per_group);
    VK_CHECK_LAUNCH();
    if (!finalize) return VK_OK;
    return gn_finalize(partial_ws, sums, g.ngroups, frames_per_group * g.nchunks, stream);
}

int gn_fold_parts(int32_t n_img, int32_t S, int32_t C, int32_t frames_per_group) {
    GnGeom g;
    if (!gn_geom(n_img, S, C, frames_per_group, g)) return 0;
    const long long np = (long long)frames_per_group * g.nchunks;
    return np <= GN_FOLD_MAX ? (int)np : 0;
}

int gn_apply(const void* x, const void* x2, int C1, void* y, const float* gamma, const float* beta, const float* sums, int32_t n_img, int32_t S,
             int32_t C, int32_t frames_per_group, float count, float eps, int32_t silu, void* stream_, int fold_nparts = 0, bool pivot = false) {
    hipStream_t stream = (hipStream_t)stream_;
    GnGeom g;
    if (!x || !y || !gamma || !beta || !sums || count <= 0.f || !gn_geom(n_img, S, C, frames_per_group, g)) return VK_EINVAL;
    if (!aligned_to(x, 16) || !aligned_to(x2, 16) || !aligned_to(y, 16) || !aligned_to(gamma, 4) || !aligned_to(beta, 4) || !aligned_to(sums, 4)) return VK_EINVAL;
    const int tok_per_wg = g.tok;
    dim3 grid(g.nchunks, n_img);
    static const int nt_env = [] { const char* e = getenv("VISTA_GN_NT"); return e ? atoi(e) & 3 : -1; }();
    const int nt_mode = nt_env >= 0 ? nt_env : ((long long)n_img * S * C * 2 >= (96LL << 20) ? 3 : 0);
    if (fold_nparts < 0 || fold_nparts > GN_FOLD_MAX) return VK_EINVAL;
    if (pivot && (y == x || y == x2)) return VK_EINVAL;
#define VK_GN_APPLY_(NL, NS, FO, PV) hipLaunchKernelGGL((gn_apply_kernel<NL, NS, FO, PV>), grid, dim3(g.threads), 0, stream, (const uint16_t*)x, (const uint16_t*)x2, C1, \
                                                       (uint16_t*)y, gamma, beta, sums, S, C, g.CG, g.R, frames_per_group, 1.f / count, eps, silu, tok_per_wg, fold_nparts)
#define VK_GN_APPLY(NL, NS, FO) do { if (pivot) VK_GN_APPLY_(NL, NS, FO, GN_PIVOT); else VK_GN_APPLY_(NL, NS, FO, false); } while (0)
    if (fold_nparts > 0) {
        if (nt_mode == 3) VK_GN_APPLY(true, true, true);
        else if (nt_mode == 2) VK_GN_APPLY(false, true, true);
        else if (nt_mode == 1) VK_GN_APPLY(true, false, true);
        else VK_GN_APPLY(false, false, true);
    } else {
        if (nt_mode == 3) VK_GN_APPLY(true, true, false);
        else if (nt_mode == 2) VK_GN_APPLY(false, true, false);
        else if (nt_mode == 1) VK_GN_APPLY(true, false, false);
        else VK_GN_APPLY(false, false, false);
    }
#undef VK_GN_APPLY
#undef VK_GN_APPLY_
    VK_CHECK_LAUNCH();
    return VK_OK;
}
}

extern "C" int vk_groupnorm_stats_bf16(const void* x, float* sums, float* partial_ws, int32_t n_img, int32_t S, int32_t C,
                                       int32_t frames_per_group, void* stream_) {
    return gn_stats(x, nullptr, 0, sums, partial_ws, n_img, S, C, frames_per_group, stream_);
}

extern "C" int vk_groupnorm_apply_bf16(const void* x, void* y, const float* gamma, const float* beta, const float* sums, int32_t n_img,
                                       int32_t S, int32_t C, int32_t frames_per_group, float count, float eps, int32_t silu, void* stream_) {
    return gn_apply(x, nullptr, 0, y, gamma, beta, sums, n_img, S, C, frames_per_group, count, eps, silu, stream_);
}

extern "C" int vk_groupnorm_fold_max(void) { return GN_FOLD_MAX; }

extern "C" int vk_groupnorm_apply_partials_bf16(const void* x, void* y, const float* gamma, const float* beta, const float* partial, int32_t n_img,
                                                int32_t S, int32_t C, int32_t nchunks, int32_t frames_per_group, float count, float eps, int32_t silu,
                                                void* stream_) {
    if (!partial || nchunks <= 0 || frames_per_group <= 0 || (long long)frames_per_group * nchunks > GN_FOLD_MAX) return VK_EINVAL;
    return gn_apply(x, nullptr, 0, y, gamma, beta, partial, n_img, S, C, frames_per_group, count, eps, silu, stream_, frames_per_group * nchunks);
}

extern "C" int vk_groupnorm_finalize_partials(float* partial, float* sums, int32_t n_img, int32_t nchunks, int32_t frames_per_group, void* stream_) {
    if (!partial || !sums || n_img <= 0 || nchunks <= 0 || frames_per_group <= 0 || (n_img % frames_per_group) != 0) return VK_EINVAL;
    if ((long long)frames_per_group * nchunks > (1LL << 24) || !aligned_to(partial, 4) || !aligned_to(sums, 4)) return VK_EINVAL;
    return gn_finalize(partial, sums, n_img / frames_per_group, frames_per_group * nchunks, (hipStream_t)stream_);
}

extern "C" int vk_groupnorm_silu_cat_bf16(const void* x1, const void* x2, void* y, const float* gamma, const float* beta, float* stats_ws,
                                          int32_t n_img, int32_t S, int32_t C1, int32_t C2, int32_t frames_per_group, float eps, int32_t silu,
                                          void* stream_) {
    if (!x1 || !x2 || !stats_ws || frames_per_group <= 0 || n_img <= 0 || C1 <= 0 || C2 <= 0 || (C1 % 8) != 0 || (C2 % 8) != 0) return VK_EINVAL;
    if (!y || !gamma || !beta || !aligned_to(x1, 16) || !aligned_to(x2, 16) || !aligned_to(y, 16) || !aligned_to(gamma, 4) || !aligned_to(beta, 4) || !aligned_to(stats_ws, 4))
        return VK_EINVAL;
    const int C = C1 + C2;
    float* partial = stats_ws + (size_t)(n_img / frames_per_group) * 64;
    const int fold = gn_fold_parts(n_img, S, C, frames_per_group);
    int rc = gn_stats(x1, x2, C1, stats_ws, partial, n_img, S, C, frames_per_group, stream_, nullptr, fold == 0, GN_PIVOT);
    if (rc != VK_OK) return rc;
    const float count = (float)(C / 32) * (float)S * (float)frames_per_group;
    return gn_apply(x1, x2, C1, y, gamma, beta, fold ? partial : stats_ws, n_img, S, C, frames_per_group, count, eps, silu, stream_, fold, GN_PIVOT);
}

extern "C" int vk_groupnorm_silu_fp8(const void* x1, const void* x2, void* y8, float* scale_out, const float* gamma, const float* beta,
                                     float* stats_ws, int32_t n_img, int32_t S, int32_t C1, int32_t C2, int32_t frames_per_group, float eps,
                                     int32_t silu, void* stream_) {
    if (!x1 || !y8 || !scale_out || !gamma || !beta || !stats_ws || frames_per_group <= 0 || n_img <= 0 || C1 <= 0 || C2 < 0 || (C1 % 8) != 0 ||
        (C2 % 8) != 0 || (x2 == nullptr) != (C2 == 0))
        return VK_EINVAL;
    const int C = C1 + C2;
    GnGeom g;
    if (!gn_geom(n_img, S, C, frames_per_group, g)) return VK_EINVAL;
    float* amax = stats_ws + (size_t)g.ngroups * 64;
    float* partial = amax + (size_t)n_img * g.nchunks;
    int rc = gn_stats(x1, x2, C1, stats_ws, partial, n_img, S, C, frames_per_group, stream_, amax);
    if (rc != VK_OK) return rc;
    const float count = (float)(C / 32) * (float)S * (float)frames_per_group;
    dim3 grid(g.nchunks, n_img);
    hipLaunchKernelGGL(gn_apply_fp8_kernel, grid, dim3(g.threads), 0, (hipStream_t)stream_, (const uint16_t*)x1, (const uint16_t*)x2, C1, (uint8_t*)y8,
                       scale_out, gamma, beta, (const float*)stats_ws, (const float*)amax, S, C, g.CG, g.R, frames_per_group, 1.f / count, eps, silu,
                       g.tok);
    VK_CHECK_LAUNCH();
    return VK_OK;
}

extern "C" int vk_rowstats_bf16(const void* x, float* stats, int32_t rows, int32_t C, int64_t ldx, void* stream_) {
    if (!x || !stats || rows <= 0 || C <= 0 || (C % 8) != 0 || C > 1536 || ldx < C || (ldx % 8) != 0) return VK_EINVAL;
    if (!aligned_to(x, 16) || !aligned_to(stats, 8)) return VK_EINVAL;
    long long want = ((long long)rows + 3) / 4;
    const long long cap = 256LL * 16;
    hipLaunchKernelGGL(rowstats_kernel, dim3((int)(want < cap ? want : cap)), dim3(256), 0, (hipStream_t)stream_, (const uint16_t*)x, (float2*)stats,
                       rows, C, (long long)ldx);
    VK_CHECK_LAUNCH();
// ... 56 lines not shown
```

### vista_amd/modules/diffusionmodules/openaimodel.py

```python
import os
from typing import Iterable

import torch.nn as nn

from ... import ops
from ..attention import FP8, Packable
from .util import Dropout, SiLU, conv_nd, linear, normalization, timestep_embedding, zero_module


class TimestepBlock(nn.Module):
    """Any module where forward() takes timestep embeddings as a second argument."""


class TimestepEmbedSequential(nn.Sequential, TimestepBlock):

    def forward(self, x, emb_silu, context=None, frame_idx=None, num_frames=None, H=None, W=None, shard=None, full=None):
        from ..video_attention import SpatialVideoTransformer
        from .video_model import VideoResBlock
        layers = list(self)
        x_gn = None
        for i, layer in enumerate(layers):
            if isinstance(layer, VideoResBlock):
                x_gn = ops.GnPartials() if i + 1 < len(layers) and isinstance(layers[i + 1], SpatialVideoTransformer) else None
                x = layer(x, emb_silu, num_frames, H, W, shard=shard, full=full, out_gn=x_gn)
            elif isinstance(layer, SpatialVideoTransformer):
                x = layer(x, context, frame_idx, num_frames, H, W, shard=shard, full=full, x_gn=x_gn)
                x_gn = None
            elif isinstance(layer, (Upsample, Downsample)):
                x, H, W = layer(x, H, W)
            else:
                raise TypeError(f"unexpected layer {type(layer).__name__} in TimestepEmbedSequential")
        return x, H, W


class Upsample(nn.Module, Packable):
    def __init__(self, channels, use_conv, dims=2, out_channels=None, padding=1, third_up=False, kernel_size=3, scale_factor=2):
        super().__init__()
        if dims != 2 or not use_conv or kernel_size != 3 or scale_factor != 2 or padding != 1:
            raise NotImplementedError("Vista uses Upsample(dims=2, use_conv=True, k=3, x2)")
        self.channels = channels
        self.out_channels = out_channels or channels
        self.use_conv, self.dims = use_conv, dims
        self.conv = conv_nd(dims, self.channels, self.out_channels, kernel_size, padding=padding)

    _nine = None

    def _pack(self, dev):
        if os.environ.get("VISTA_UPCONV_FOLD", "1") != "0" and self.channels % 64 == 0:
            return ops.pack_upconv2x2(self.conv.weight, self.conv.bias, device=dev)
        return ops.pack_conv3x3(self.conv.weight, self.conv.bias, device=dev)

    def forward(self, x, H, W):
        assert x.shape[-1] == self.channels
        pw = self.packed()
        if pw.classes == 4:
            if ops.upconv2x2_fits(x, pw, x.shape[0], H, W):
                return ops.upconv2x2(x, pw, x.shape[0], H, W)
            if self._nine is None or self._nine[1] is not pw:
                object.__setattr__(self, "_nine", (ops.pack_conv3x3(self.conv.weight, self.conv.bias, device=x.device), pw))
            pw = self._nine[0]
        out, Ho, Wo = ops.conv3x3(x, pw, x.shape[0], H, W, ups=2)
        return out, Ho, Wo


class Downsample(nn.Module, Packable):
    def __init__(self, channels, use_conv, dims=2, out_channels=None, padding=1, third_down=False):
        super().__init__()
        if dims != 2 or not use_conv or padding != 1:
            raise NotImplementedError("Vista uses Downsample(dims=2, use_conv=True)")
        self.channels = channels
        self.out_channels = out_channels or channels
        self.use_conv, self.dims = use_conv, dims
        self.op = conv_nd(dims, self.channels, self.out_channels, 3, stride=2, padding=padding)

    def _pack(self, dev):
        return ops.pack_conv3x3(self.op.weight, self.op.bias, device=dev)

    def forward(self, x, H, W):
        assert x.shape[-1] == self.channels
        out, Ho, Wo = ops.conv3x3(x, self.packed(), x.shape[0], H, W, stride=2)
        return out, Ho, Wo


class ResBlock(TimestepBlock, Packable):

    def __init__(self, channels, emb_channels, dropout, out_channels=None, use_conv=False, use_scale_shift_norm=False, dims=2,
                 use_checkpoint=False, up=False, down=False, kernel_size=3, exchange_temb_dims=False, skip_t_emb=False, causal=False):
        super().__init__()
        if up or down or use_scale_shift_norm or use_conv or causal:
            raise NotImplementedError("resblock_updown / scale-shift norm / causal are not used by Vista")
        self.channels, self.emb_channels, self.dropout = channels, emb_channels, dropout
        self.out_channels = out_channels or channels
        self.use_checkpoint = use_checkpoint
        self.exchange_temb_dims = exchange_temb_dims and not skip_t_emb
        self.skip_t_emb = skip_t_emb
        self.dims = dims
        if isinstance(kernel_size, Iterable):
            kernel_size = tuple(kernel_size)
            padding = [k // 2 for k in kernel_size]
        else:
            padding = kernel_size // 2
        if dims == 2 and kernel_size not in (3, (3, 3)):
            raise NotImplementedError("2-D ResBlock kernel must be 3x3")
        if dims == 3 and kernel_size not in (3, (3, 3, 3), (3, 1, 1)):
            raise NotImplementedError("3-D ResBlock kernel must be (3,1,1) (video_kernel_size: [3,1,1]) or 3x3x3")
        self.full3d = dims == 3 and kernel_size != (3, 1, 1)
        self.in_layers = nn.Sequential(normalization(channels), SiLU(), conv_nd(dims, channels, self.out_channels, kernel_size, padding=padding))
        self.updown = False
        self.emb_layers = None if skip_t_emb else nn.Sequential(SiLU(), linear(emb_channels, self.out_channels))
        self.out_layers = nn.Sequential(normalization(self.out_channels), SiLU(), Dropout(p=dropout),
                                        zero_module(conv_nd(dims, self.out_channels, self.out_channels, kernel_size, padding=padding)))
        if self.out_channels == channels:
            self.skip_connection = nn.Identity()
        else:
            self.skip_connection = conv_nd(dims, channels, self.out_channels, 1)

    def _pack(self, dev):
        pc = ops.pack_conv3x3 if self.dims == 2 else (ops.pack_conv3d if self.full3d else ops.pack_conv_t3)
        pk = {"conv1": pc(self.in_layers[2].weight, self.in_layers[2].bias, device=dev),
              "conv2": pc(self.out_layers[3].weight, self.out_layers[3].bias, device=dev)}
        if self.emb_layers is not None:
            pk["emb"] = ops.pack_linear(self.emb_layers[1].weight, self.emb_layers[1].bias, dev)
        if not isinstance(self.skip_connection, nn.Identity):
            pk["skip"] = ops.pack_linear(self.skip_connection.weight, self.skip_connection.bias, dev)
        if FP8["conv"] and not self.full3d and self.emb_layers is not None:
            pc8 = ops.pack_conv3x3_fp8 if self.dims == 2 else ops.pack_conv_t3_fp8
            pk["conv1_8"] = pc8(self.in_layers[2].weight, self.in_layers[2].bias, device=dev)
            pk["conv2_8"] = pc8(self.out_layers[3].weight, self.out_layers[3].bias, device=dev)
        return pk

    def forward(self, x, emb_silu, H, W, T=None, out_alpha=1.0, shard=None, T_global=None, x_gn=None, out_gn=None):
        pk = self.packed()
        xb = None
        if isinstance(x, tuple):
            x, xb = x
            if self.dims != 2 or "skip" not in pk:
                raise ValueError("a concatenated input needs the 2-D ResBlock with a 1x1 skip convolution")
        n_img, S, _ = x.shape
        gn1, gn2 = self.in_layers[0], self.out_layers[0]
        fpg = 1 if self.dims == 2 else T
        src = getattr(self, "_emb_src", None)
        table = getattr(src[0], "table", None) if src is not None else None
        table = table.get("emb") if table is not None else None
        if self.emb_layers is None:
            emb_out = None
        elif table is not None and table.shape[0] == n_img:
            emb_out = table[:, src[1]:src[1] + src[2]]
        else:
            emb_out = ops.linear(emb_silu, pk["emb"], out_f32=True)

        def gnorm(t, gn, part=None):
            if shard is None or self.dims == 2:
                return ops.groupnorm(t, gn.weight, gn.bias, gn.eps, silu=True, frames_per_group=fpg, gn=part)
            cnt = float(t.shape[-1] // 32) * float(S) * float(T_global)
            return ops.groupnorm_sharded(t, gn.weight, gn.bias, gn.eps, True, fpg, shard.all_reduce_sum, cnt, gn=part)

        def halo(t):
            return shard.halo_exchange(t) if (shard is not None and self.dims == 3) else (None, None)
        if FP8["conv"] and shard is None and not self.full3d and self.emb_layers is not None:
            if "conv1_8" not in pk:
                self.invalidate_packed()
                pk = self.packed()
            h8, hs = ops.groupnorm_fp8(x, gn1.weight, gn1.bias, gn1.eps, True, fpg, x2=xb)
            if self.dims == 2:
                h = ops.conv3x3_fp8(h8, hs, pk["conv1_8"], n_img, H, W, rowvec=emb_out)
                h8, hs = ops.groupnorm_fp8(h, gn2.weight, gn2.bias, gn2.eps, True)
                skip = x if "skip" not in pk else ops.linear(x, pk["skip"], x2=xb)
                return ops.conv3x3_fp8(h8, hs, pk["conv2_8"], n_img, H, W, res1=skip)
            h = ops.conv_t3_fp8(h8, hs, pk["conv1_8"], T, S, rowvec=emb_out)
            h8, hs = ops.groupnorm_fp8(h, gn2.weight, gn2.bias, gn2.eps, True, fpg)
            return ops.conv_t3_fp8(h8, hs, pk["conv2_8"], T, S, alpha=out_alpha, res2=x, beta=1.0)
        h = gnorm(x, gn1, x_gn) if xb is None else ops.groupnorm_cat(x, xb, gn1.weight, gn1.bias, gn1.eps, silu=True)
        mid_gn = ops.GnPartials()
        if self.dims == 2:
            h, _, _ = ops.conv3x3(h, pk["conv1"], n_img, H, W, rowvec=emb_out, gn=mid_gn)
            h = ops.groupnorm(h, gn2.weight, gn2.bias, gn2.eps, silu=True, gn=mid_gn)
            skip = x if "skip" not in pk else ops.linear(x, pk["skip"], x2=xb)
            out, _, _ = ops.conv3x3(h, pk["conv2"], n_img, H, W, res1=skip, gn=out_gn)
            return out
        if self.full3d:
            if shard is not None or emb_out is not None:
                raise NotImplementedError("3x3x3 time_stack: no frame sharding / embedding branch")
            h = ops.conv3d(h, pk["conv1"], T, H, W)
            h = gnorm(h, gn2)
            return ops.conv3d(h, pk["conv2"], T, H, W, alpha=out_alpha, res2=x, beta=1.0)
        prev, nxt = halo(h)
        h = ops.conv_t3(h, pk["conv1"], T, S, rowvec=emb_out, halo_prev=prev, halo_next=nxt, gn=mid_gn)
        h = gnorm(h, gn2, mid_gn)
        prev, nxt = halo(h)
        return ops.conv_t3(h, pk["conv2"], T, S, alpha=out_alpha, res2=x, beta=1.0, halo_prev=prev, halo_next=nxt, gn=out_gn)


class Timestep(nn.Module):
    def __init__(self, dim):
        super().__init__()
        self.dim = dim

    def forward(self, t):
        return timestep_embedding(t, self.dim)
```

### vista_amd/modules/diffusionmodules/sampling.py

```python
import os
from typing import Dict, Union

import torch

from ... import ops
from ...util import append_dims, default, instantiate_from_config
from .guiders import IdentityGuider


class FusedDenoiser:

    def __init__(self, denoiser, network):
        self.denoiser, self.network = denoiser, network

    def __call__(self, x, sigma, cond, cond_mask):
        return self.denoiser(self.network, x, sigma, cond, cond_mask)


class BaseDiffusionSampler:
    def __init__(self, discretization_config: Union[Dict, None], num_steps: Union[int, None] = None,
                 guider_config: Union[Dict, None] = None, verbose: bool = False, device: str = "cuda"):
        self.num_steps = num_steps
        self.discretization = instantiate_from_config(discretization_config)
        self.guider = instantiate_from_config(default(guider_config, {"target": "vista_amd.modules.diffusionmodules.guiders.IdentityGuider"}))
# ... 128 lines not shown
    def _unet(self, net_in, n_ts, c_noise):
        use = self._graph_mode == "force" or (self._graph_mode == "1" and self.unet_shard is None)
        if self._split:
            return self._unet_halves(net_in, c_noise, use)
        if use and self.unet_shard is not None and getattr(self.unet_shard.comm, "backend", None) == "nccl" \
                and os.environ.get("VISTA_HIPGRAPH_RCCL", "0") != "1":
            raise RuntimeError("VISTA_HIPGRAPH=force / bench.py --graph with a frame-sharded forward over RCCL: capturing its collectives hangs on this "
                               "software stack (see DESIGN section 6); run the sharded step eagerly, or set VISTA_HIPGRAPH_RCCL=1 to try anyway")
        if not use:
            ts = torch.full((n_ts,), c_noise, device=self.xw.device)
            return self.unet.forward_tokens(net_in, ts, self.ctx2, self.y2, self.mask2, self.T, self.H, self.W, shard=self.unet_shard)
        g = self._graph
        if g is None:
            g = self._graph = self._graph_for(net_in, n_ts)
        g["in"].copy_(net_in)
        g["ts"].fill_(c_noise)
        g["graph"].replay()
        return g["out"]

    def _unet_halves(self, net_in, c_noise, graph):
        n = self.n
        half = lambda t, h: t[h * n:(h + 1) * n]
        if not graph:
            ts = torch.full((n,), c_noise, device=self.xw.device)
            return torch.cat([self.unet.forward_tokens(half(net_in, h), ts, half(self.ctx2, h), half(self.y2, h), half(self.mask2, h), self.T, self.H, self.W)
                              for h in (0, 1)])
        gs = self._graph
        if gs is None:
            gs = self._graph = [self._graph_for(half(net_in, h), n, ctx=half(self.ctx2, h), y=half(self.y2, h), mask=half(self.mask2, h), slot=h) for h in (0, 1)]
        for h in (0, 1):
            gs[h]["in"].copy_(half(net_in, h))
            gs[h]["ts"].fill_(c_noise)
        dev = net_in.device
        side = FusedLoop._CFG_STREAMS.get(dev.index)
        if side is None:
            side = FusedLoop._CFG_STREAMS[dev.index] = torch.cuda.Stream(device=dev)
        cur = torch.cuda.current_stream()
        side.wait_stream(cur)
        with torch.cuda.stream(side):
            gs[1]["graph"].replay()
        gs[0]["graph"].replay()
        cur.wait_stream(side)
        return torch.cat([gs[0]["out"], gs[1]["out"]])

    _WARM_STREAMS = {}
    _CFG_STREAMS = {}

    def _graph_for(self, net_in, n_ts, ctx=None, y=None, mask=None, slot=0):
        unet = self.unet
        cache = unet.__dict__.setdefault("_hipgraph_cache", {})
        from .. import attention as _att
        if ctx is None:
            ctx, y, mask = self.ctx2, self.y2, self.mask2
        switches = (tuple(sorted(_att.FP8.items())), _att.FF_FUSED, _att.QKV_SPLIT, _att.Q_LOG2, ops.TILE_CFG, ops.GN_EPI,
                    None if self.unet_shard is None else getattr(self.unet_shard, "a2a_chunks", None))
        key = (tuple(net_in.shape), n_ts, tuple(ctx.shape), tuple(y.shape), tuple(mask.shape), self.T, self.H, self.W,
               None if self.unet_shard is None else id(self.unet_shard), str(net_in.device), switches, slot)
        g = cache.get(key)
        wkey = (_att.pack_generation(),) + tuple((id(q), _att.Packable._param_version(q)) for q in unet.parameters())
        if g is not None and g["wkey"] != wkey:
            g = None
        if g is None:
            if ops.PROFILE_ATTN is not None:
                raise RuntimeError("ops.PROFILE_ATTN records timing events around attention launches; clear it before capturing a hipGraph")
            dev = net_in.device
            g = {"in": torch.empty_like(net_in), "ts": torch.empty((n_ts,), device=dev), "ctx": ctx.clone(), "y": y.clone(),
                 "mask": mask.clone(), "wkey": wkey}
            g["in"].copy_(net_in)
            g["ts"].fill_(0.0)
            fwd = lambda: unet.forward_tokens(g["in"], g["ts"], g["ctx"], g["y"], g["mask"], self.T, self.H, self.W, shard=self.unet_shard)
            side = FusedLoop._WARM_STREAMS.get(dev.index)
            if side is None:
                side = FusedLoop._WARM_STREAMS[dev.index] = torch.cuda.Stream(device=dev)
            with ops.graph_workspace(slot):
                side.wait_stream(torch.cuda.current_stream())
                with torch.cuda.stream(side):
                    fwd()
                torch.cuda.current_stream().wait_stream(side)
                g["wkey"] = (_att.pack_generation(),) + tuple((id(q), _att.Packable._param_version(q)) for q in unet.parameters())
                g["ws"] = ops.graph_workspace_tensor()
                g["graph"] = torch.cuda.CUDAGraph()
                mode = "global" if self.unet_shard is None else "thread_local"
                with torch.cuda.graph(g["graph"], capture_error_mode=mode):
                    g["out"] = fwd()
            cache[key] = g
        else:
            g["ctx"].copy_(ctx)
            g["y"].copy_(y)
            g["mask"].copy_(mask)
        return g

    def step(self, i):
        c_skip, c_out, c_in, c_noise = self.coef[i]
        net_in = ops.sampler_prepare(self.xw, self.cf, self.maskf, self.cu, self.cc, self.cin_pad, c_in, self.replace)
        if self.half is None:
            net_out = self._unet(net_in, 2 * self.n, c_noise)
        else:
            tl = self.xw.shape[0]
            mine = self._unet(net_in[self.half * tl:(self.half + 1) * tl], self.n, c_noise)
            net_out = self.shard.exchange_cfg_halves(mine)
        self._update(i, net_out, c_out, c_skip)

    def _update(self, i, net_out, c_out, c_skip):
        ops.sampler_update(self.xw, net_out, self.scales, c_out, c_skip, self.sig[i], self.sig[i + 1])

    def finish(self):
        if self.replace:
# ... 75 lines not shown
```

### vista_amd/modules/diffusionmodules/video_model.py

```python
from typing import List, Optional, Union

import threading

import torch
import torch.nn as nn

from ... import ops
from ...util import default, repeat_as_img_seq
from ..attention import Packable, _invalidate_after_load as _drop_packs_after_load
from ..video_attention import SpatialVideoTransformer
from .openaimodel import Downsample, ResBlock, Timestep, TimestepEmbedSequential, Upsample
from .util import AlphaBlender, SiLU, conv_nd, linear, mlp_f32, normalization, timestep_embedding, zero_module

CIN_PAD = 64


class _ThreadTable:

    def __init__(self):
        self._slots = {}

    @property
    def table(self):
        return self._slots.get(threading.get_ident())

    @table.setter
    def table(self, value):
        if value is None:
            self._slots.pop(threading.get_ident(), None)
        else:
            self._slots[threading.get_ident()] = value

    def __deepcopy__(self, memo):
        return _ThreadTable()

    def __reduce__(self):
        return (_ThreadTable, ())


class VideoResBlock(ResBlock):

    def __init__(self, channels, emb_channels, dropout, video_kernel_size=3, merge_strategy="fixed", merge_factor=0.5,
                 out_channels=None, use_conv=False, use_scale_shift_norm=False, dims=2, use_checkpoint=False, up=False, down=False):
        super().__init__(channels, emb_channels, dropout, out_channels=out_channels, use_conv=use_conv,
                         use_scale_shift_norm=use_scale_shift_norm, dims=dims, use_checkpoint=use_checkpoint, up=up, down=down)
        oc = default(out_channels, channels)
        self.time_stack = ResBlock(oc, emb_channels, dropout=dropout, dims=3, out_channels=oc, use_scale_shift_norm=False,
                                   use_conv=False, up=False, down=False, kernel_size=video_kernel_size, use_checkpoint=use_checkpoint,
                                   exchange_temb_dims=True, causal=False)
        self.time_mixer = AlphaBlender(alpha=merge_factor, merge_strategy=merge_strategy, rearrange_pattern="b t -> b 1 t 1 1")

    def _pack_params(self):
        return [p for n, p in self.named_parameters() if not n.startswith("time_stack.")]

    def _pack(self, dev):
        pk = super()._pack(dev)
        pk["alpha"] = self.time_mixer.alpha_value()
        return pk

    def forward(self, x, emb_silu, num_frames, H, W, shard=None, full=None, out_gn=None):
        mid = ops.GnPartials()
        x = super().forward(x, emb_silu, H, W, out_gn=mid)
        alpha = self.packed()["alpha"]
        if shard is None:
            return self.time_stack(x, emb_silu, H, W, T=num_frames, out_alpha=1.0 - alpha, x_gn=mid, out_gn=out_gn)
        return self.time_stack(x, emb_silu, H, W, T=shard.t_local, out_alpha=1.0 - alpha, shard=shard, T_global=num_frames, x_gn=mid, out_gn=out_gn)


class VideoUNet(nn.Module, Packable):
    def __init__(
            self,
            in_channels: int,
            model_channels: int,
            out_channels: int,
            num_res_blocks: int,
            attention_resolutions: int,
            dropout: float = 0.0,
            channel_mult: List[int] = (1, 2, 4, 8),
            conv_resample: bool = True,
            dims: int = 2,
            num_classes: Optional[int] = None,
            use_checkpoint: bool = False,
            num_heads: int = -1,
            num_head_channels: int = -1,
            num_heads_upsample: int = -1,
            use_scale_shift_norm: bool = False,
            resblock_updown: bool = False,
            transformer_depth: Union[List[int], int] = 1,
            transformer_depth_middle: Optional[int] = None,
            context_dim: Optional[int] = None,
            time_downup: bool = False,
            time_context_dim: Optional[int] = None,
            extra_ff_mix_layer: bool = False,
            use_spatial_context: bool = False,
            merge_strategy: str = "learned_with_images",
            merge_factor: float = 0.5,
            spatial_transformer_attn_type: str = "softmax",
            video_kernel_size: Union[int, List[int]] = 3,
            use_linear_in_transformer: bool = False,
            adm_in_channels: Optional[int] = None,
            disable_temporal_crossattention: bool = False,
            max_ddpm_temb_period: int = 10000,
            add_lora: bool = False,
            action_control: bool = False
    ):
        super().__init__()
        assert context_dim is not None
        if num_heads_upsample == -1:
            num_heads_upsample = num_heads
        if num_heads == -1:
            assert num_head_channels != -1
        if num_head_channels == -1:
            assert num_heads != -1
        if dims != 2 or resblock_updown or time_downup or not conv_resample or use_scale_shift_norm:
            raise NotImplementedError("only the shipped Vista topology options are implemented (dims=2, conv resample)")
# ... 147 lines not shown
        key = (n_img, T, str(device))
        if key not in self._frame_idx_cache:
            self._frame_idx_cache[key] = torch.arange(T, dtype=torch.float32).repeat(n_img // T).to(device)
        return self._frame_idx_cache[key]

    @torch.no_grad()
    def forward(self, x: torch.Tensor, timesteps: torch.Tensor, context: Optional[torch.Tensor] = None, y: Optional[torch.Tensor] = None,
                time_context: Optional[torch.Tensor] = None, cond_mask: Optional[torch.Tensor] = None, num_frames: Optional[int] = None):
        assert (y is not None) == (self.num_classes is not None), "Must specify y if and only if the model is class-conditional"
        if time_context is not None:
            raise NotImplementedError("separate time_context is not used with use_spatial_context=True")
        n_img, _, H, W = x.shape
        T = int(num_frames)
        assert n_img % T == 0
        tokens = ops.nchw_to_tokens(x.float(), CIN_PAD)
        out_tok = self.forward_tokens(tokens, timesteps, context, y, cond_mask, T, H, W)
        return ops.tokens_to_nchw(out_tok, n_img, self.out_channels, H, W).to(x.dtype)

    @torch.no_grad()
    def forward_tokens(self, tokens, timesteps, context, y, cond_mask, T, H, W, shard=None):
        pk = self.packed()
        n_img = timesteps.shape[0]
        dev = tokens.device
        t_emb = timestep_embedding(timesteps, self.model_channels, max_period=10000)
        te = mlp_f32(t_emb, *pk["time_embed"])
        if context.shape[0] != n_img:
            assert context.shape[0] == n_img // T, f"{context.shape} {n_img}"
            context = repeat_as_img_seq(context, T)
        if y.shape[0] != n_img:
            assert y.shape[0] == n_img // T, f"{y.shape} {n_img}"
            y = repeat_as_img_seq(y, T)
        le = mlp_f32(ops.cast_to_bf16(y.float()), *pk["label"])
        if cond_mask is not None:
            ce = mlp_f32(t_emb, *pk["cond"])
            emb, emb_silu = ops.emb_combine(ce, te, le, cond_mask.float().contiguous())
        else:
            emb, emb_silu = ops.emb_combine(None, te, le, None)
        if context.dim() != 3 or context.shape[1] != 1:
            raise NotImplementedError("Vista's cross-attention context is one token per image (crossattn: (N, 1, 3456))")
        ctx = ops.cast_to_bf16(context.float().reshape(n_img, -1))
        frame_idx = self._frame_idx(n_img, T, dev)
        full = None
        if shard is not None:
            full = {"emb_silu": emb_silu, "ctx": ctx}
            emb_silu = shard.take_local_rows(emb_silu)
            ctx = shard.take_local_rows(ctx)
        kw = dict(frame_idx=frame_idx, num_frames=T, shard=shard, full=full)

        clip_ctx = (ctx if full is None else full["ctx"]).view(n_img // T, T, -1)[:, 0]
        self._emb_tls.table = {"emb": ops.linear(emb_silu, pk["emb_cat"], out_f32=True),
                               "ctx_s": ops.linear(ctx, pk["ctx_s"], out_f32=True) if "ctx_s" in pk else None,
                               "ctx_t": ops.linear(clip_ctx, pk["ctx_t"], out_f32=True) if "ctx_t" in pk else None}
        try:
            hs = []
            h = tokens
            for module in self.input_blocks:
                h, H, W = module(h, emb_silu, context=ctx, H=H, W=W, **kw)
                hs.append(h)
            h, H, W = self.middle_block(h, emb_silu, context=ctx, H=H, W=W, **kw)
            for module in self.output_blocks:
                h, H, W = module((h, hs.pop()), emb_silu, context=ctx, H=H, W=W, **kw)
        finally:
            self._emb_tls.table = None
        gn = self.out[0]
        h = ops.groupnorm(h, gn.weight, gn.bias, gn.eps, silu=True)
        out, _, _ = ops.conv3x3(h, pk["out"], tokens.shape[0], H, W, out_f32=True)
        return out


class _InputConv(TimestepEmbedSequential, Packable):

    def __init__(self, in_channels, model_channels):
        super().__init__(conv_nd(2, in_channels, model_channels, 3, padding=1))

    def _pack(self, dev):
        return ops.pack_conv3x3(self[0].weight, self[0].bias, cin_pad=CIN_PAD, device=dev)

    def forward(self, x, emb_silu, context=None, frame_idx=None, num_frames=None, H=None, W=None, shard=None, full=None):
        out, H, W = ops.conv3x3(x, self.packed(), x.shape[0], H, W)
        return out, H, W
```

### vista_amd/modules/video_attention.py

```python
import torch
import torch.nn as nn

from .. import ops
from .attention import FeedForward, MemoryEfficientCrossAttention, Packable, SpatialTransformer
from .diffusionmodules.util import AlphaBlender, LayerNorm, Linear, SiLU, mlp_f32, timestep_embedding


class VideoTransformerBlock(nn.Module, Packable):
    ATTENTION_MODES = {"softmax": MemoryEfficientCrossAttention, "softmax-xformers": MemoryEfficientCrossAttention}

    def __init__(self, dim, n_heads, d_head, dropout=0.0, context_dim=None, gated_ff=True, use_checkpoint=False, timesteps=None,
                 ff_in=False, inner_dim=None, attn_mode="softmax", disable_self_attn=False, disable_temporal_crossattention=False,
                 switch_temporal_ca_to_sa=False, add_lora=False, action_control=False):
        super().__init__()
        attn_cls = self.ATTENTION_MODES[attn_mode]
        self.ff_in = ff_in or inner_dim is not None
        if inner_dim is None:
            inner_dim = dim
        assert int(n_heads * d_head) == inner_dim
        self.is_res = inner_dim == dim
        if not self.is_res:
            raise NotImplementedError("inner_dim != dim is not the Vista configuration")
        if disable_self_attn or switch_temporal_ca_to_sa:
            raise NotImplementedError("disable_self_attn / switch_temporal_ca_to_sa are not used by Vista")
# ... 35 lines not shown
            cv = self.attn2.context_vector(clip_context)
            x, st = ops.linear(att, a1["out"], res1=x, rowvec=cv, rows_per_vec=T * S, emit_stats=True)
        else:
            x, st = ops.linear(att, a1["out"], res1=x, emit_stats=True)
        r = self.ff.forward_folded(x, st, pk["ff_in"], self.norm3, res1=x, alpha=1.0 - alpha, res2=x_mix, rowvec2=emb_rows.neg_rows,
                                   beta=alpha, rows_per_vec=S, emit_stats=emit_stats)
        return r if emit_stats else (r, None)


class _EmbRows:

    __slots__ = ("rows", "neg_rows")

    def __init__(self, rows):
        self.rows, self.neg_rows = rows, rows.neg()


class SpatialVideoTransformer(SpatialTransformer):

    def __init__(self, in_channels, n_heads, d_head, depth=1, dropout=0.0, use_linear=False, context_dim=None,
                 use_spatial_context=False, timesteps=None, merge_strategy="fixed", merge_factor=0.5, time_context_dim=None,
                 ff_in=False, use_checkpoint=False, time_depth=1, attn_mode="softmax", disable_self_attn=False,
                 disable_temporal_crossattention=False, max_time_embed_period=10000, add_lora=False, action_control=False):
        super().__init__(in_channels, n_heads, d_head, depth=depth, dropout=dropout, attn_type=attn_mode, use_checkpoint=use_checkpoint,
                         context_dim=context_dim, use_linear=use_linear, disable_self_attn=disable_self_attn, add_lora=add_lora,
                         action_control=action_control)
        self.time_depth = time_depth
        self.depth = depth
        self.max_time_embed_period = max_time_embed_period
        inner_dim = n_heads * d_head
        if not use_spatial_context:
            raise NotImplementedError("use_spatial_context=False (separate time_context) is not the Vista configuration")
        time_context_dim = context_dim
        self.time_stack = nn.ModuleList([
            VideoTransformerBlock(inner_dim, n_heads, d_head, dropout=dropout, context_dim=time_context_dim, timesteps=timesteps,
                                  use_checkpoint=use_checkpoint, ff_in=ff_in, inner_dim=inner_dim, attn_mode=attn_mode,
                                  disable_self_attn=disable_self_attn, disable_temporal_crossattention=disable_temporal_crossattention,
                                  add_lora=add_lora, action_control=action_control) for _ in range(self.depth)])
        assert len(self.time_stack) == len(self.transformer_blocks)
        self.use_spatial_context = use_spatial_context
        self.in_channels = in_channels
        time_embed_dim = in_channels * 4
        self.time_pos_embed = nn.Sequential(Linear(in_channels, time_embed_dim), SiLU(), Linear(time_embed_dim, in_channels))
        self.time_mixer = AlphaBlender(alpha=merge_factor, merge_strategy=merge_strategy, rearrange_pattern="b t -> (b t) 1 1")
        self.n_heads = n_heads

    def _pack(self, dev):
        return {"proj_in": ops.pack_linear(self.proj_in.weight, self.proj_in.bias, dev),
                "proj_out": ops.pack_linear(self.proj_out.weight, self.proj_out.bias, dev),
                "tpe0": ops.pack_linear(self.time_pos_embed[0].weight, self.time_pos_embed[0].bias, dev),
                "tpe2": ops.pack_linear(self.time_pos_embed[2].weight, self.time_pos_embed[2].bias, dev),
                "alpha": self.time_mixer.alpha_value()}

    def forward(self, x, context, frame_idx, T, H, W, shard=None, full=None, x_gn=None):
        pk = self.packed()
        n_img, S, C = x.shape
        x_in = x
        h = ops.groupnorm(x, self.norm.weight, self.norm.bias, self.norm.eps, silu=False, gn=x_gn)
        h, st = ops.linear(h, pk["proj_in"], emit_stats=True)
        tc = pk.get("_tpe_rows")
        fv = Packable._param_version(frame_idx)
        if tc is not None and tc[0] is frame_idx and tc[1] == fv:
            emb = tc[2]
        else:
            emb = _EmbRows(mlp_f32(timestep_embedding(frame_idx, self.in_channels, self.max_time_embed_period), pk["tpe0"], pk["tpe2"]))
            pk["_tpe_rows"] = (frame_idx, fv, emb)
        ctx_full = context if shard is None else full["ctx"]
        B = ctx_full.shape[0] // T
        clip_context = ctx_full.view(B, T, -1)[:, 0]
        emb_local = emb.rows if shard is None else shard.take_local_rows(emb.rows)
        last = len(self.transformer_blocks) - 1
        for i, (block, mix_block) in enumerate(zip(self.transformer_blocks, self.time_stack)):
            h, st = block(h, st, context, n_img, S, out_rowvec=emb_local, emit_stats=shard is None)
            if shard is None:
                h, st = mix_block(h, st, emb, clip_context, B, T, S, alpha=pk["alpha"], emit_stats=i != last)
            else:
                hp = shard.to_pixels(h.view(n_img, S, C))
                s_r = hp.shape[1]
                nch = min(getattr(shard, "a2a_chunks", 1), min(shard.pixel_counts(S)))
                if nch <= 1:
                    hp = hp.view(-1, C)
                    hp, _ = mix_block(hp, ops.rowstats(hp), emb, clip_context, B, T, s_r, alpha=pk["alpha"])
                    h = shard.to_frames(hp.view(B * T, s_r, C), S).view(-1, C)
                else:
                    out = torch.empty((n_img, S, C), dtype=hp.dtype, device=hp.device)
                    pending = []
                    for ci, (lo, hi) in enumerate(shard.pixel_chunks(S, nch)):
                        part = hp[:, lo:hi].contiguous().view(-1, C)
                        part, _ = mix_block(part, ops.rowstats(part), emb, clip_context, B, T, hi - lo, alpha=pk["alpha"])
                        pending.append(shard.to_frames_begin(part.view(B * T, hi - lo, C), S, nch, ci))
                    for pnd in pending:
                        shard.to_frames_end(pnd, out)
                    h = out.view(-1, C)
                st = ops.rowstats(h) if i != last else None
        out = ops.linear(h, pk["proj_out"], res1=x_in)
        return out.view(n_img, S, C)
```

### vista_amd/ops.py

```python
import ctypes as C
import math
import os
import threading

import torch

from . import _lib
from ._lib import VkFp8Args, VkGemmDesc, check

AMODE_DENSE, AMODE_CONV3X3, AMODE_TEMPORAL3, AMODE_CONV3D, AMODE_UPCONV2X2 = 0, 1, 2, 3, 4
EPI_LINEAR, EPI_GEGLU, EPI_TRANS = 0, 1, 2
ACT = torch.float16 if _lib.ACT_DTYPE == "fp16" else torch.bfloat16
BF16 = ACT
F32 = torch.float32


class storage:

    def __init__(self, dtype):
        if dtype not in (torch.bfloat16, torch.float16):
            raise ValueError("ops.storage: torch.bfloat16 or torch.float16")
        self.dtype, self.name = dtype, ("fp16" if dtype is torch.float16 else "bf16")

    def __enter__(self):
# ... 284 lines not shown
            if torch.cuda.is_current_stream_capturing():
                raise RuntimeError("ops.graph_workspace must be entered before the capture starts")
            _GRAPH_TLS.ws[key] = torch.empty(SPLITK_WS_BYTES // 4, dtype=F32, device=f"cuda:{dev}")
        _GRAPH_TLS.depth += 1
        self._outer, _GRAPH_TLS.slot = _GRAPH_TLS.slot, self.slot
        return self

    def __exit__(self, *exc):
        _GRAPH_TLS.depth -= 1
        _GRAPH_TLS.slot = self._outer
        return False


def _graph_ws_key():
    dev, slot = torch._C._cuda_getDevice(), _GRAPH_TLS.slot
    return dev if slot == 0 else (dev, slot)


def graph_workspace_tensor():
    return _GRAPH_TLS.ws.get(_graph_ws_key())


def _splitk_workspace(stream):
    if _GRAPH_TLS.depth > 0:
        return _GRAPH_TLS.ws[_graph_ws_key()]
    key = (torch._C._cuda_getDevice(), stream.value)
    ws = _SPLITK_WS.ws.get(key)
    if ws is None:
        ws = _SPLITK_WS.ws[key] = torch.empty(SPLITK_WS_BYTES // 4, dtype=F32, device=f"cuda:{key[0]}")
    return ws


class RowStats:

    __slots__ = ("t", "parts", "M")

    def __init__(self, t, parts, M):
        self.t, self.parts, self.M = t, parts, M


ROW_RANGE = None

GN_EPI = int(os.environ.get("VISTA_GN_EPI", "1"))


class GnPartials:

    __slots__ = ("t", "nchunks", "rows", "C")

    def __init__(self):
        self.t, self.nchunks, self.rows, self.C = None, 0, 0, 0


def _prepare(desc):
    desc.tile_cfg = TILE_CFG
    if ROW_RANGE is not None:
        desc.m_begin, desc.m_end = ROW_RANGE
    stream = _stream()
    if SPLITK_WS_BYTES:
        ws = _splitk_workspace(stream)
        desc.splitk_ws, desc.splitk_ws_bytes = _p(ws), ws.numel() * 4
    return stream


def _ask_gn(d, gn, rows_per_image, device):
    if gn is None or not GN_EPI or ROW_RANGE is not None:
        return
    d.gn_rows = int(rows_per_image)
    _prepare(d)
    slots = _lib.load().vk_gemm_gnstat_fit(C.byref(d))
    if slots < 0:
        raise _lib.VistaHipError(f"vk_gemm_gnstat_fit failed with code {slots}")
    if slots > 0:
        gn.t = torch.empty(slots * 64, dtype=F32, device=device)
        gn.nchunks, gn.rows, gn.C = int(rows_per_image) // 64, d.M, d.N
        d.gnstat_out = _p(gn.t)


def _gemm(desc, emit_stats=False, device=None):
    lib = _lib.load()
    stream = _prepare(desc)
    stats = None
    if emit_stats:
        parts = lib.vk_gemm_rowstat_parts(C.byref(desc))
        if parts <= 0:
            raise _lib.VistaHipError(f"vk_gemm_rowstat_parts failed with code {parts}")
        stats = RowStats(torch.empty((parts, desc.M, 2), dtype=F32, device=device), parts, desc.M)
        desc.rowstat_out = _p(stats.t)
    check(lib.vk_gemm_bf16(C.byref(desc), stream), "vk_gemm_bf16")
    return stats


def _fill_ln(d, pw, ln, M):
    if (ln is None) != (pw.colsum is None):
        raise ValueError("a weight packed with a folded LayerNorm needs the input's RowStats (ln=...), and only such a weight takes them")
    if ln is not None:
        if ln.M != M:
            raise ValueError(f"RowStats of {ln.M} rows passed to a GEMM over {M} rows")
        d.ln_stats, d.ln_parts, d.ln_colsum, d.ln_eps = _p(ln.t), ln.parts, _p(pw.colsum), pw.ln_eps


def _fill_epilogue(d, pw, out, M, rowvec, rows_per_vec, res1, res2, alpha, beta, rowvec2=None, ncols=None, out_dtype=None):
    dev = pw.wt.get_device()
    d.Wt = _p(pw.wt)
    d.bias = _p(pw.bias)
    d.M, d.N, d.K = M, pw.N, pw.K
    if out is None:
        f32, d.out, d.ldc = False, d.Wt, pw.N
    else:
        f32 = out.dtype is F32
        d.ldc = _operand(out, "out", out_dtype or (F32 if f32 else BF16), dev, 16 if (f32 or out_dtype is not None) else 8, M, pw.N if ncols is None else ncols, 4,
                         exact_cols=True)
        d.out = _p(out)
    d.out_f32 = 1 if f32 else 0
    d.alpha, d.beta = float(alpha), float(beta)
    if rowvec is not None or rowvec2 is not None:
        if int(rows_per_vec) <= 0:
            raise ValueError("rowvec / rowvec2: rows_per_vec must be positive")
        nvec = (M + int(rows_per_vec) - 1) // int(rows_per_vec)
    if rowvec is not None:
        d.rowvec, d.ldv, d.rows_per_vec = _p(rowvec), _operand(rowvec, "rowvec", F32, dev, 16, nvec, pw.N, 4), int(rows_per_vec)
    if res1 is not None:
        r, ld = _rows2d(res1, "res1")
        d.res1, d.ld_res1 = _p(r), _operand(r, "res1", BF16, dev, 8, M, pw.N, 4)
    if res2 is not None:
        r, ld = _rows2d(res2, "res2")
        d.res2, d.ld_res2 = _p(r), _operand(r, "res2", BF16, dev, 8, M, pw.N, 4)
    if rowvec2 is not None:
        if res2 is None:
            raise ValueError("rowvec2 is added to res2 (out = alpha*(...) + beta*(res2 + rowvec2))")
        if rowvec is not None and rowvec.stride(0) != rowvec2.stride(0):
            raise ValueError("rowvec and rowvec2 share one row stride")
        d.rowvec2, d.ldv, d.rows_per_vec = _p(rowvec2), _operand(rowvec2, "rowvec2", F32, dev, 16, nvec, pw.N, 4), int(rows_per_vec)


def linear(x, pw, *, out=None, out_f32=False, rowvec=None, rows_per_vec=0, res1=None, res2=None, alpha=1.0, beta=0.0, rowvec2=None,
           x2=None, ln=None, emit_stats=False, act=None, mx8_cols=0, alt_cols_from=0):
    x2d, lda = _rows2d(x, "x")
    M = x2d.shape[0]
    k_in = x2d.shape[1]
    _operand(x2d, "x", BF16, pw.wt.get_device(), 16, M, k_in, 8)
    d = VkGemmDesc()
    if x2 is not None:
        b2d, ldb = _rows2d(x2, "x2")
        if b2d.shape[0] != M:
            raise ValueError("linear: x and x2 must have the same rows")
        _operand(b2d, "x2", BF16, pw.wt.get_device(), 16, M, b2d.shape[1], 8)
        d.A2, d.lda2, d.k_split = _p(b2d), ldb, k_in
        k_in += b2d.shape[1]
    if k_in != pw.K:
        raise ValueError(f"linear: K mismatch {k_in} vs {pw.K}")
    if pw.ffout:
        raise ValueError("linear: this weight is laid out for ff_fused (pack_ff_out), not for vk_gemm_bf16")
    if pw.geglu:
        nout = pw.N // 2
        if out is None:
            out = torch.empty((M, nout), dtype=BF16, device=x.device)
    elif out is None:
        out = torch.empty((M, pw.N - mx8_cols), dtype=F32 if out_f32 else BF16, device=x.device)
    d.A, d.lda = _p(x2d), lda
    d.amode = AMODE_DENSE
    d.epi = EPI_GEGLU if pw.geglu else EPI_LINEAR
    _fill_epilogue(d, pw, out, M, rowvec, rows_per_vec, res1, res2, alpha, beta, rowvec2, ncols=pw.N // 2 if pw.geglu else pw.N - mx8_cols)
    _fill_ln(d, pw, ln, M)
    mx = None
    if mx8_cols:
        if pw.geglu or emit_stats or mx8_cols % 320 or pw.N % 320 or out.shape[1] != pw.N - mx8_cols:
            raise ValueError("linear: mx8_cols needs a LINEAR weight, N and mx8_cols multiples of 320, no emit_stats")
        mx = (torch.empty((M, mx8_cols), dtype=torch.uint8, device=x.device), torch.empty((M, mx8_cols // 32), dtype=torch.uint8, device=x.device))
        d.mx8_out, d.mx8_scales, d.mx8_cols, d.ld_mx8, d.ld_mx8s = _p(mx[0]), _p(mx[1]), mx8_cols, mx8_cols, mx8_cols // 32
    if act is not None:
        if act != "gelu" or pw.geglu:
            raise ValueError("linear: act must be None or 'gelu' (exact-erf GELU in the LINEAR epilogue)")
        d.act = 1
    d.alt_cols_from = int(alt_cols_from)
    stats = _gemm(d, emit_stats, x.device)
    if mx is not None:
        return out, mx[0], mx[1]
    return (out, stats) if emit_stats else out


def linear_vt(x, pw, S, out=None, ln=None):
    x2, lda = _rows2d(x, "x")
    M = x2.shape[0]
    _operand(x2, "x", BF16, pw.wt.get_device(), 16, M, pw.K, 8, exact_cols=True)
    if S <= 0 or M % S:
        raise ValueError(f"linear_vt: x has {M} rows, not a multiple of S = {S}")
    if out is None:
        out = torch.empty((M // S, pw.N, S), dtype=BF16, device=x.device)
    elif out.dtype != BF16 or not out.is_contiguous() or out.shape != (M // S, pw.N, S):
        raise ValueError("linear_vt: out must be contiguous bf16 (n_img, N, S)")
    _dense(out, "out", BF16, pw.wt.get_device(), 8, M * pw.N)
    d = VkGemmDesc()
    d.A, d.lda = _p(x2), lda
    d.amode, d.epi = AMODE_DENSE, EPI_TRANS
    d.bias = _p(pw.bias)
    d.Wt, d.M, d.N, d.K, d.out, d.ldc, d.S = _p(pw.wt), M, pw.N, pw.K, _p(out), S, S
    d.alpha = 1.0
    _fill_ln(d, pw, ln, M)
    _gemm(d)
    return out


def rowstats(x):
    x2, ldx = _rows2d(x, "x")
    M, Cc = x2.shape
    _operand(x2, "x", BF16, x.get_device(), 16, M, Cc, 8)
    st = torch.empty((1, M, 2), dtype=F32, device=x.device)
    check(_lib.load().vk_rowstats_bf16(_p(x2), _p(st), M, Cc, ldx, _stream()), "vk_rowstats_bf16")
    return RowStats(st, 1, M)


FF_FUSED_WIDTH, FF_FUSED_MAX_HIDDEN = 320, 1280
FF_FUSED_DBG_BUF = None
FF_FUSED_DBG = 0


def ff_fused_ok(pw_in, pw_out):
    return (pw_in.geglu and pw_in.K == FF_FUSED_WIDTH and pw_out.N == FF_FUSED_WIDTH and pw_in.N == 2 * pw_out.K
            and pw_out.K % 64 == 0 and 128 <= pw_out.K <= FF_FUSED_MAX_HIDDEN)


def ff_fused(x, pw_in, pw_out, *, out=None, rowvec=None, rows_per_vec=0, res1=None, res2=None, alpha=1.0, beta=0.0, rowvec2=None, ln=None,
             emit_stats=False):
    x2d, lda = _rows2d(x, "x")
    M = x2d.shape[0]
    _operand(x2d, "x", BF16, pw_in.wt.get_device(), 16, M, x2d.shape[1], 8)
    if not ff_fused_ok(pw_in, pw_out) or not pw_out.ffout or x2d.shape[1] != pw_in.K:
# ... 19 lines not shown
    if emit_stats:
        parts = lib.vk_ff_fused_rowstat_parts()
        stats = RowStats(torch.empty((parts, M, 2), dtype=F32, device=x.device), parts, M)
        d.rowstat_out = _p(stats.t)
    check(lib.vk_ff_fused_bf16(C.byref(g), C.byref(d), _stream()), "vk_ff_fused_bf16")
    return (out, stats) if emit_stats else out


def conv3x3(x, pw, n_img, H, W, *, stride=1, ups=1, out=None, out_f32=False, rowvec=None, res1=None, res2=None, alpha=1.0,
            beta=0.0, asym_pad=False, gn=None):
    cin = x.shape[-1]
    _dense(x, "x", BF16, pw.wt.get_device(), 16, n_img * H * W * cin)
    if pw.K != 9 * cin:
        raise ValueError(f"conv3x3: weight K {pw.K} != 9*{cin}")
    He, We = H * ups, W * ups
    pad = 1 if asym_pad else 2
    Hout = (He + pad - 3) // stride + 1
    Wout = (We + pad - 3) // stride + 1
    M = n_img * Hout * Wout
    if out is None:
        out = torch.empty((M, pw.N), dtype=F32 if out_f32 else BF16, device=x.device)
    d = VkGemmDesc()
    d.A, d.lda = _p(x), cin
    d.amode, d.epi = AMODE_CONV3X3, EPI_LINEAR
    d.H, d.Wd, d.Cin, d.Hout, d.Wout, d.stride, d.ups = H, W, cin, Hout, Wout, stride, ups
    d.asym_pad = 1 if asym_pad else 0
    _fill_epilogue(d, pw, out, M, rowvec, Hout * Wout, res1, res2, alpha, beta)
    _ask_gn(d, gn, Hout * Wout, x.device)
    _gemm(d)
    return (out.view(n_img, Hout * Wout, pw.N) if out.is_contiguous() else out), Hout, Wout


UPCONV_CLASS_FASTEST = int(os.environ.get("VISTA_UPCONV_ORDER", "0")) != 0


def _upconv_desc(x, pw, n_img, H, W, rowvec, out):
    cin = x.shape[-1]
    d = VkGemmDesc()
    d.A, d.lda = _p(x), cin
    d.amode, d.epi = AMODE_UPCONV2X2, EPI_LINEAR
    d.H, d.Wd, d.Cin, d.Hout, d.Wout, d.stride, d.ups = H, W, cin, 2 * H, 2 * W, 1, 2
    _fill_epilogue(d, pw, out, n_img * 4 * H * W, rowvec, 4 * H * W, None, None, 1.0, 0.0)
    stream = _prepare(d)
    if UPCONV_CLASS_FASTEST:
        d.tile_cfg |= 8
    return d, stream


def upconv2x2_fits(x, pw, n_img, H, W, rowvec=None, out=None):
    d, _ = _upconv_desc(x, pw, n_img, H, W, rowvec, out)
    return _lib.load().vk_gemm_tile_choice(C.byref(d)) > 0


def upconv2x2(x, pw, n_img, H, W, rowvec=None, out=None):
    cin = x.shape[-1]
    _dense(x, "x", BF16, pw.wt.get_device(), 16, n_img * H * W * cin)
    if pw.classes != 4 or pw.K != 4 * cin:
        raise ValueError(f"upconv2x2: needs a pack_upconv2x2 weight with K = 4*{cin}")
    M = n_img * 4 * H * W
    if out is None:
        out = torch.empty((M, pw.N), dtype=BF16, device=x.device)
    d, stream = _upconv_desc(x, pw, n_img, H, W, rowvec, out)
    check(_lib.load().vk_gemm_bf16(C.byref(d), stream), "vk_gemm_bf16 (folded upsample convolution)")
    return (out.view(n_img, 4 * H * W, pw.N) if out.is_contiguous() else out), 2 * H, 2 * W


def conv_t3(x, pw, T, S, *, out=None, out_f32=False, rowvec=None, res1=None, res2=None, alpha=1.0, beta=0.0, halo_prev=None,
            halo_next=None, gn=None):
    cin = x.shape[-1]
    if x.dim() != 3 or T <= 0 or x.shape[0] % T or x.shape[1] != S:
        raise ValueError(f"conv_t3: x must be ((b t), S, C) with (b t) a multiple of T = {T} and S = {S}, got {tuple(x.shape)}")
    _dense(x, "x", BF16, pw.wt.get_device(), 16, x.shape[0] * S * cin)
    if pw.K != 3 * cin:
        raise ValueError("conv_t3: weight K mismatch")
    M = x.shape[0] * x.shape[1]
    if out is None:
        out = torch.empty((M, pw.N), dtype=F32 if out_f32 else BF16, device=x.device)
    d = VkGemmDesc()
    d.A, d.lda = _p(x), cin
    d.amode, d.epi = AMODE_TEMPORAL3, EPI_LINEAR
    d.Cin, d.T, d.S = cin, T, S
    for name, h in (("halo_prev", halo_prev), ("halo_next", halo_next)):
        if h is not None:
            if h.shape != (x.shape[0] // T, S, cin):
                raise ValueError(f"{name}: expected contiguous (clips, S, C) = {(x.shape[0] // T, S, cin)}, got {tuple(h.shape)}")
            _dense(h, name, BF16, pw.wt.get_device(), 16, h.numel())
            setattr(d, name, _p(h))
    _fill_epilogue(d, pw, out, M, rowvec, S, res1, res2, alpha, beta)
    _ask_gn(d, gn, S, x.device)
    _gemm(d)
    return out.view(x.shape[0], S, pw.N)


def pack_conv3d(weight, bias=None, device="cuda", cin_pad=None):
    w = weight.detach().float().permute(0, 2, 3, 4, 1).contiguous()
    cout, _, _, _, cin = w.shape
    cp = cin_pad or ceil_to(cin, 64)
    if cp != cin:
        w = torch.nn.functional.pad(w, (0, cp - cin))
    return _finish_pack(_slab_major(w.reshape(cout, 27, cp)), None if bias is None else bias.detach().float(), device)


def conv3d(x, pw, T, H, W, *, out=None, out_f32=False, res1=None, res2=None, alpha=1.0, beta=0.0):
    cin = x.shape[-1]
    if T <= 0 or x.shape[0] % T:
        raise ValueError(f"conv3d: x has {x.shape[0]} frames, not a multiple of T = {T}")
    _dense(x, "x", BF16, pw.wt.get_device(), 16, x.shape[0] * H * W * cin)
    if pw.K != 27 * cin:
        raise ValueError(f"conv3d: weight K {pw.K} != 27*{cin}")
    M = x.shape[0] * H * W
    if out is None:
        out = torch.empty((M, pw.N), dtype=F32 if out_f32 else BF16, device=x.device)
    d = VkGemmDesc()
    d.A, d.lda = _p(x), cin
    d.amode, d.epi = AMODE_CONV3D, EPI_LINEAR
# ... 271 lines not shown
    sigma = max((factor - 1.0) / 2.0, 0.001)
    ks = int(max(2.0 * 2 * sigma, 3))
    if ks % 2 == 0:
        ks += 1
    return sigma, ks


CLIP_MEAN = (0.48145466, 0.4578275, 0.40821073)
CLIP_STD = (0.26862954, 0.26130258, 0.27577711)


def clip_preprocess_patches(img, out_hw=224, patch=14, kpad=None, antialias=True, mean=CLIP_MEAN, std=CLIP_STD):
    _need(img, F32, "img")
    img = img.contiguous()
    n, c, H, W = img.shape
    if c != 3:
        raise ValueError("clip_preprocess_patches: 3-channel images")
    g = out_hw // patch
    kp = kpad or ceil_to(3 * patch * patch, 64)
    out = torch.zeros((n * (1 + g * g), kp), dtype=BF16, device=img.device)
    down = antialias and max(H / out_hw, W / out_hw) > 1
    (sy, ky), (sx, kx) = (antialias_blur_params(H, out_hw), antialias_blur_params(W, out_hw)) if down else ((1.0, 1), (1.0, 1))
    m3, s3 = (C.c_float * 3)(*mean), (C.c_float * 3)(*std)
    check(_lib.load().vk_clip_preprocess_patches(_p(img), _p(out), n, H, W, out_hw, patch, kp, sy, sx, ky, kx, m3, s3, _stream()),
          "vk_clip_preprocess_patches")
    return out


def attn_temporal(qkv, B, T, S, heads, scale=None):
    c = heads * 64
    _operand(qkv, "qkv", BF16, qkv.get_device(), 16, B * T * S, 3 * c, 8, exact_cols=True)
    if qkv.shape[0] != B * T * S:
        _refuse("qkv", qkv, f"must be ((b t) s, 3*heads*64) = {(B * T * S, 3 * c)}")
    o = torch.empty((B * T * S, c), dtype=BF16, device=qkv.device)
    lib = _lib.load()
    check(lib.vk_attn_temporal_bf16(_p(qkv), _p(o), B, T, S, heads, qkv.stride(0), c, 2 * c, o.stride(0),
                                    float(scale if scale is not None else 1.0 / math.sqrt(64)), _stream()), "vk_attn_temporal_bf16")
    return o


def softmax_rows(x, out=None):
    if x.dim() != 2:
        _refuse("x", x, "must be 2-D")
    rows, cols = x.shape
    _operand(x, "x", F32, x.get_device(), 16, rows, cols, 4)
    if out is None:
        out = torch.empty((rows, cols), dtype=BF16, device=x.device)
    else:
        _operand(out, "out", BF16, x.get_device(), 8, rows, cols, 4, exact_cols=True)
    check(_lib.load().vk_softmax_rows_f32_bf16(_p(x), _p(out), rows, cols, x.stride(0), out.stride(0), _stream()), "vk_softmax_rows_f32_bf16")
    return out


def _gn_partials_ok(gn, n_img, S, Cc):
    if gn is None or gn.t is None:
        return False
    if gn.rows != n_img * S or gn.C != Cc or gn.nchunks * 64 != S:
        raise ValueError(f"GnPartials of a ({gn.rows} rows, {gn.C} channels, {gn.nchunks * 64} rows per image) tensor passed to a GroupNorm over ({n_img}, {S}, {Cc})")
    return True


def groupnorm(x, gamma, beta, eps, silu, frames_per_group=1, out=None, gn=None):
    if x.dim() != 3:
        _refuse("x", x, "must be (n_img, S, C)")
    n_img, S, Cc = x.shape
    _dense(x, "x", BF16, x.get_device(), 16, n_img * S * Cc)
    _affine(gamma, beta, Cc, x.get_device())
    if out is None:
        out = torch.empty_like(x)
    else:
        _dense(out, "out", BF16, x.get_device(), 16, n_img * S * Cc)
    if _gn_partials_ok(gn, n_img, S, Cc):
        lib = _lib.load()
        count = float(Cc // 32) * float(S) * float(frames_per_group)
        if frames_per_group * gn.nchunks <= lib.vk_groupnorm_fold_max():
            check(lib.vk_groupnorm_apply_partials_bf16(_p(x), _p(out), _p(gamma), _p(beta), _p(gn.t), n_img, S, Cc, gn.nchunks, frames_per_group, count,
                                                       float(eps), 1 if silu else 0, _stream()), "vk_groupnorm_apply_partials_bf16")
            gn.t = None
            return out
        sums = torch.empty((n_img // frames_per_group) * 64, dtype=F32, device=x.device)
        check(lib.vk_groupnorm_finalize_partials(_p(gn.t), _p(sums), n_img, gn.nchunks, frames_per_group, _stream()), "vk_groupnorm_finalize_partials")
        gn.t = None
        check(lib.vk_groupnorm_apply_bf16(_p(x), _p(out), _p(gamma), _p(beta), _p(sums), n_img, S, Cc, frames_per_group, count, float(eps),
                                          1 if silu else 0, _stream()), "vk_groupnorm_apply_bf16")
        return out
    ws = torch.empty(((n_img // frames_per_group) + n_img * ((S + 31) // 32)) * 64, dtype=F32, device=x.device)
    lib = _lib.load()
    check(lib.vk_groupnorm_silu_bf16(_p(x), _p(out), _p(gamma), _p(beta), _p(ws), n_img, S, Cc, frames_per_group, float(eps),
                                     1 if silu else 0, _stream()), "vk_groupnorm_silu_bf16")
    return out


def groupnorm_cat(a, b, gamma, beta, eps, silu, frames_per_group=1):
    if a.dim() != 3 or b.dim() != 3 or a.shape[:2] != b.shape[:2]:
        raise ValueError("groupnorm_cat: contiguous (n_img, S, C) inputs with equal n_img, S required")
    n_img, S, c1 = a.shape
    c2 = b.shape[2]
    _dense(a, "a", BF16, a.get_device(), 16, n_img * S * c1)
    _dense(b, "b", BF16, a.get_device(), 16, n_img * S * c2)
    _affine(gamma, beta, c1 + c2, a.get_device())
    out = torch.empty((n_img, S, c1 + c2), dtype=BF16, device=a.device)
    ws = torch.empty(((n_img // frames_per_group) + n_img * ((S + 31) // 32)) * 64, dtype=F32, device=a.device)
    check(_lib.load().vk_groupnorm_silu_cat_bf16(_p(a), _p(b), _p(out), _p(gamma), _p(beta), _p(ws), n_img, S, c1, c2, frames_per_group,
                                                 float(eps), 1 if silu else 0, _stream()), "vk_groupnorm_silu_cat_bf16")
    return out


def groupnorm_sharded(x, gamma, beta, eps, silu, frames_per_group, allreduce, global_count, gn=None):
    if x.dim() != 3:
        _refuse("x", x, "must be (n_img, S, C)")
    n_img, S, Cc = x.shape
    _dense(x, "x", BF16, x.get_device(), 16, n_img * S * Cc)
    _affine(gamma, beta, Cc, x.get_device())
    out = torch.empty_like(x)
    ng = n_img // frames_per_group
    sums = torch.empty(ng * 64, dtype=F32, device=x.device)
    lib = _lib.load()
    if _gn_partials_ok(gn, n_img, S, Cc):
        check(lib.vk_groupnorm_finalize_partials(_p(gn.t), _p(sums), n_img, gn.nchunks, frames_per_group, _stream()), "vk_groupnorm_finalize_partials")
        gn.t = None
    else:
        part = torch.empty(n_img * ((S + 31) // 32) * 64, dtype=F32, device=x.device)
        check(lib.vk_groupnorm_stats_bf16(_p(x), _p(sums), _p(part), n_img, S, Cc, frames_per_group, _stream()), "vk_groupnorm_stats_bf16")
    allreduce(sums)
    check(lib.vk_groupnorm_apply_bf16(_p(x), _p(out), _p(gamma), _p(beta), _p(sums), n_img, S, Cc, frames_per_group, float(global_count),
                                      float(eps), 1 if silu else 0, _stream()), "vk_groupnorm_apply_bf16")
    return out


def layernorm(x, gamma, beta, eps=1e-5, addvec=None, rows_per_vec=0, want_sum=False):
    Cc = x.shape[-1]
    rows = x.numel() // Cc
    _dense(x, "x", BF16, x.get_device(), 16, rows * Cc)
    _affine(gamma, beta, Cc, x.get_device())
    if addvec is not None:
        if int(rows_per_vec) <= 0:
            raise ValueError("layernorm: addvec needs rows_per_vec > 0")
        _operand(addvec, "addvec", F32, x.get_device(), 4, (rows + int(rows_per_vec) - 1) // int(rows_per_vec), Cc)
    y = torch.empty_like(x)
    s = torch.empty_like(x) if (want_sum and addvec is not None) else None
    lib = _lib.load()
    check(lib.vk_layernorm_bf16(_p(x), _p(y), _p(s), _p(gamma), _p(beta), _p(addvec), rows, Cc, int(rows_per_vec),
                                addvec.stride(0) if addvec is not None else 0, float(eps), _stream()), "vk_layernorm_bf16")
    return (y, s) if want_sum else y


def concat_channels(a, b):
    c1, c2 = a.shape[-1], b.shape[-1]
    rows = a.numel() // c1
    if a.shape[:-1] != b.shape[:-1]:
        raise ValueError("concat_channels: a and b must agree in every dim but the last")
    _dense(a, "a", BF16, a.get_device(), 16, rows * c1)
    _dense(b, "b", BF16, a.get_device(), 16, rows * c2)
    out = torch.empty(a.shape[:-1] + (c1 + c2,), dtype=BF16, device=a.device)
# ... 557 lines not shown
```

Before: 6.474 steps/s.

## Emit GroupNorm partial stats in finer channel units from producing GEMMs, including skip-concat inputs

Producing GEMMs (dense proj_out, upsample conv, conv3x3) can now write per-64-row GroupNorm sum and sum-of-squares partials at a configurable channel-unit granularity (gn_unit). Consuming GroupNorms, including the one over the decoder skip concatenation, can then apply normalization straight from those partials through a new apply_units kernel. This removes the separate statistics pass over activations before GroupNorm in the UNet decoder and output head. It also forces the pipe GEMM family and tile config 4 when stats are requested, which may give up faster tile choices. It adds GEMM kernel template variants and new routing conditions.

```diff
diff --git a/include/vista_hip.h b/include/vista_hip.h
--- a/include/vista_hip.h
+++ b/include/vista_hip.h
@@ -45,6 +45,7 @@
     float* gnstat_out;
     int32_t gn_rows;
     int32_t alt_cols_from;
+    int32_t gn_unit;
 } VkGemmDesc;
 
 int vk_gemm_bf16(const VkGemmDesc* d, void* stream);
@@ -117,6 +118,8 @@
 int vk_groupnorm_apply_partials_bf16(const void* x, void* y, const float* gamma, const float* beta, const float* partial, int32_t n_img,
                                      int32_t S, int32_t C, int32_t nchunks, int32_t frames_per_group, float count, float eps, int32_t silu,
                                      void* stream);
+int vk_groupnorm_apply_units_bf16(const void* x, const void* x2, int32_t C1, void* y, const float* gamma, const float* beta, const float* part1, int32_t unit1,
+                                  const float* part2, int32_t unit2, int32_t n_img, int32_t S, int32_t C, int32_t nchunks, float eps, int32_t silu, void* stream);
 
 int vk_layernorm_bf16(const void* x, void* y, void* sum_out, const float* gamma, const float* beta,
                       const float* addvec, int32_t rows, int32_t C, int32_t rows_per_vec, int32_t ldv, float eps,
diff --git a/vista_amd/_lib.py b/vista_amd/_lib.py
--- a/vista_amd/_lib.py
+++ b/vista_amd/_lib.py
@@ -41,6 +41,7 @@
         ("m_begin", _i32), ("m_end", _i32),
         ("gnstat_out", _vp), ("gn_rows", _i32),
         ("alt_cols_from", _i32),
+        ("gn_unit", _i32),
     ]
 
 
@@ -110,6 +111,7 @@
     "vk_groupnorm_finalize_partials": [_vp, _vp, _i32, _i32, _i32, _vp],
     "vk_groupnorm_fold_max": [],
     "vk_groupnorm_apply_partials_bf16": [_vp, _vp, _vp, _vp, _vp, _i32, _i32, _i32, _i32, _i32, _f32, _f32, _i32, _vp],
+    "vk_groupnorm_apply_units_bf16": [_vp, _vp, _i32, _vp, _vp, _vp, _vp, _i32, _vp, _i32, _i32, _i32, _i32, _i32, _f32, _i32, _vp],
     "vk_layernorm_bf16": [_vp, _vp, _vp, _vp, _vp, _vp, _i32, _i32, _i32, _i32, _f32, _vp],
     "vk_rowstats_bf16": [_vp, _vp, _i32, _i32, _i64, _vp],
     "vk_groupnorm_silu_cat_bf16": [_vp, _vp, _vp, _vp, _vp, _vp, _i32, _i32, _i32, _i32, _i32, _f32, _i32, _vp],
diff --git a/vista_amd/csrc/gemm.hip b/vista_amd/csrc/gemm.hip
--- a/vista_amd/csrc/gemm.hip
+++ b/vista_amd/csrc/gemm.hip
@@ -360,6 +360,11 @@
 }
 
 struct TileChoice { int cfg, ksplit; };
+inline bool gn_route_pipe(const VkGemmDesc* d, bool gnstat) {
+    static const bool pipe_on = [] { const char* e = getenv("VISTA_GEMM_PIPE"); return !e || atoi(e) != 0; }();
+    return gnstat && pipe_on && d->gn_unit > 0 && d->amode == AMODE_DENSE && ((d->tile_cfg & 7) == 0 || (d->tile_cfg & 7) == 7) &&
+           vk_gemm_pipe_gnstat_ok(d, 1) > 0;
+}
 
 inline bool cfg5_ok(const VkGemmDesc* d) { return d->amode == AMODE_DENSE && d->epi == EPI_LINEAR && !d->out_f32 && (d->N % 160) == 0; }
 inline TileChoice choose_tile(const VkGemmDesc* d, bool rowstat, bool gnstat) {
@@ -379,7 +384,8 @@
         const bool ok320 = (epi != EPI_GEGLU) && (amode != AMODE_CONV3D) && (d->N % 320 == 0);
         const bool ok256 = n256 * 10 <= d->N * 11;
         const long long need = 192;
-        if (cfg5_ok(d) && tile5_max_k > 0 && d->K <= tile5_max_k && d->N <= d->K && wgs(128, 160) >= 1024) cfg = 5;
+        if (gn_route_pipe(d, gnstat) && wgs(256, 320) >= need) cfg = 4;
+        else if (cfg5_ok(d) && tile5_max_k > 0 && d->K <= tile5_max_k && d->N <= d->K && wgs(128, 160) >= 1024) cfg = 5;
         else if (ok320 && wgs(256, 320) >= need) cfg = 4;
         else if (ok256 && wgs(256, 256) >= need) cfg = 3;
         else if (wgs(256, 128) >= need) cfg = 2;
@@ -388,7 +394,7 @@
             const long long r3 = (wgs(256, 256) + 255) / 256, r4 = (wgs(256, 320) + 255) / 256;
             if (r4 * 320 * 100 < r3 * 256 * (d->K >= 640 ? 103 : 95)) cfg = 4;
         }
-        if (cfg5_ok(d) && cfg != 5 && tile5_max_k > 0 && wgs(128, 160) >= need) {
+        if (cfg5_ok(d) && cfg != 5 && tile5_max_k > 0 && wgs(128, 160) >= need && !gn_route_pipe(d, gnstat)) {
             int bm = 256, bn = 320, slots = 256;
             if (cfg == 3) bn = 256;
             else if (cfg == 2) bn = 128;
@@ -467,10 +473,11 @@
         nine.K = 9 * d.Cin;
         nine.tile_cfg &= ~8;
         const TileChoice t = choose_tile(&nine, false, false);
-        const bool ok = t.cfg == 7 && t.ksplit == 1 && !rowstat && !gnstat && vk_gemm_pipe_fit(&d);
-        return {ok ? FAM_PIPE : FAM_NONE, 7, 1, 0, 0, 0};
-    }
-    if (d.m_begin == 0 && d.m_end == d.M && !(d.tile_cfg & 16) && (force == 6 || (stream_on && !rowstat))) {
+        const bool ok = t.cfg == 7 && t.ksplit == 1 && !rowstat && (!gnstat || d.gn_unit > 0) && vk_gemm_pipe_fit(&d);
+        const int gn_floats = (ok && gnstat) ? vk_gemm_pipe_gnstat_ok(&d, 1) : 0;
+        return {ok ? FAM_PIPE : FAM_NONE, 7, 1, 0, 0, (d.M / 64) * gn_floats / 64};
+    }
+    if (d.m_begin == 0 && d.m_end == d.M && !(d.tile_cfg & 16) && (force == 6 || (stream_on && !rowstat && !gn_route_pipe(&d, gnstat)))) {
         if (const int fit = vk_gemm_stream_fit(&d)) return {FAM_STREAM, 6, 1, 0, d.N / (32 * fit), 0};
     }
     if (force == 6) d.tile_cfg &= ~7;
@@ -482,7 +489,7 @@
     int bn, wn;
     tile_geometry(t.cfg, bn, wn);
     p.rowstat_slabs = ((d.N + bn - 1) / bn) * wn;
-    if (p.family == FAM_PIPE && p.ksplit == 1 && p.tail_row == 0 && !rowstat && vk_gemm_pipe_gnstat_ok(&d, 1)) p.gnstat_slots = d.M / 64;
+    if (p.family == FAM_PIPE && p.ksplit == 1 && p.tail_row == 0 && !rowstat) p.gnstat_slots = (d.M / 64) * vk_gemm_pipe_gnstat_ok(&d, 1) / 64;
     return p;
 }
 
@@ -554,7 +561,7 @@
         if (d->K != 4 * d->Cin || d->ups != 2 || d->stride != 1 || d->asym_pad || d->H <= 0 || d->Wd <= 0 || d->Hout != 2 * d->H || d->Wout != 2 * d->Wd) return VK_EINVAL;
         const long long hw4 = 4ll * d->H * d->Wd;
         if ((d->M % hw4) != 0 || (d->rowvec && d->rows_per_vec != hw4)) return VK_EINVAL;
-        if (d->epi != EPI_LINEAR || d->out_f32 || d->res1 || d->res2 || d->rowvec2 || d->gnstat_out || d->rowstat_out || d->mx8_out || d->ln_stats || d->A2 ||
+        if (d->epi != EPI_LINEAR || d->out_f32 || d->res1 || d->res2 || d->rowvec2 || (d->gnstat_out && d->gn_unit <= 0) || d->rowstat_out || d->mx8_out || d->ln_stats || d->A2 ||
             d->halo_prev || d->halo_next || d->act || d->alt_cols_from)
             return VK_EINVAL;
         if (d->m_begin != 0 || (d->m_end != 0 && d->m_end != d->M)) return VK_EINVAL;
@@ -562,6 +569,7 @@
     }
     if (d->amode == AMODE_CONV3D && (d->K != 27 * d->Cin || d->T <= 0 || d->H <= 0 || d->Wd <= 0 || d->H >= 4096 || d->Wd >= 4096 ||
                                      (long long)d->M != (long long)(d->M / (d->H * d->Wd)) * d->H * d->Wd)) return VK_EINVAL;
+    if (d->gn_unit < 0) return VK_EINVAL;
     if ((d->rowvec || d->rowvec2) && d->rows_per_vec <= 0) return VK_EINVAL;
     if (d->rowvec2 && (!d->res2 || d->epi != EPI_LINEAR)) return VK_EINVAL;
     if (d->A2 && (d->amode != AMODE_DENSE || d->k_split <= 0 || d->k_split >= d->K || (d->k_split % BK) != 0 || (d->lda2 % 8) != 0)) return VK_EINVAL;
diff --git a/vista_amd/csrc/gemm_common.h b/vista_amd/csrc/gemm_common.h
--- a/vista_amd/csrc/gemm_common.h
+++ b/vista_amd/csrc/gemm_common.h
@@ -360,7 +360,7 @@
 }
 
 template <int NG>
-__device__ __forceinline__ void gn_reduce_store(float (&gs)[NG], float (&gq)[NG], float* __restrict__ slot, int gb, int lane, bool valid) {
+__device__ __forceinline__ void gn_reduce_store(float (&gs)[NG], float (&gq)[NG], float* __restrict__ slot, int gb, int lane, bool valid, int nu = 32) {
     static_assert(NG == 16 || NG == 8 || NG == 4, "160-column wave tiles of 10 / 20 / 40-channel groups");
     float r[NG];
 #pragma unroll
@@ -384,7 +384,7 @@
 #pragma unroll
     for (; k >= 1; k >>= 1) r[0] += __shfl_xor(r[0], k, 64);
     constexpr int SH = NG == 16 ? 1 : (NG == 8 ? 2 : 3);
-    if (valid && (lane & ((1 << SH) - 1)) == 0) slot[32 * (lane >> 5) + gb + ((lane & 31) >> SH)] = r[0];
+    if (valid && (lane & ((1 << SH) - 1)) == 0) slot[nu * (lane >> 5) + gb + ((lane & 31) >> SH)] = r[0];
 }
 
 template <int CPG, int NG>
@@ -447,6 +447,15 @@
         for (int i = 0; i < GN_NG; ++i) { gs[i] = 0.f; gq[i] = 0.f; }
     }
     const uint32_t gn_lo_mask = lh ? 0u : 0xffffffffu;
+    const int gn_nu = GNC ? p.N / GNC : 32;
+    auto gn_slot = [&](int mb) -> float* {
+        int blk = mb >> 6;
+        if constexpr (UPC) {
+            const int per = (p.H * p.Wd) >> 6, img = blk / per;
+            blk = img * 4 * per + cls * per + (blk - img * per);
+        }
+        return (float*)p.gnstat_out + (size_t)blk * (2 * gn_nu);
+    };
     uint4 wa[U][2], wb[U][2];
     auto issue = [&](int fj, int fi, int u) {
         if (NRES >= 1) { wa[u][0] = *(const uint4*)((const char*)ra + rao[fj] + fi * 64); wa[u][1] = *(const uint4*)((const char*)ra + rao[fj] + fi * 64 + 32); }
@@ -540,7 +549,7 @@
         if constexpr (GNC != 0 && FY > 2) {
             if ((fj & 1) == 1) {
                 const int mb = m0 + wm * MW + (fj >> 1) * 64;
-                gn_reduce_store<GN_NG>(gs, gq, (float*)p.gnstat_out + (size_t)(mb >> 6) * 64, (n0 + wn * NW) / GNC, l31 | (lh << 5), mb < p.m_end);
+                gn_reduce_store<GN_NG>(gs, gq, gn_slot(mb), (n0 + wn * NW) / GNC, l31 | (lh << 5), mb < p.m_end, gn_nu);
 #pragma unroll
                 for (int i = 0; i < GN_NG; ++i) { gs[i] = 0.f; gq[i] = 0.f; }
             }
@@ -548,7 +557,7 @@
     }
     if constexpr (GNC != 0 && FY == 2) {
         const int mb = m0 + wm * MW;
-        gn_reduce_store<GN_NG>(gs, gq, (float*)p.gnstat_out + (size_t)(mb >> 6) * 64, (n0 + wn * NW) / GNC, l31 | (lh << 5), mb < p.m_end);
+        gn_reduce_store<GN_NG>(gs, gq, gn_slot(mb), (n0 + wn * NW) / GNC, l31 | (lh << 5), mb < p.m_end, gn_nu);
     }
 }
 
@@ -556,7 +565,7 @@
 __device__ __forceinline__ void gemm_epilogue_linear_lds(const VkGemmDesc& p, f32x16_t (&acc)[FX][FY], int m0, int n0, int wm, int wn, int l31, int lh,
                                                          int stat_part, const float2* lnrow, const float* ev, int img0, int cls = 0) {
     if constexpr (UPC) {
-        epilogue_linear_lds_body<0, false, false, FX, FY, FM, FN, BN, CAP, 0, true>(p, acc, m0, n0, wm, wn, l31, lh, stat_part, nullptr, ev, img0, cls);
+        epilogue_linear_lds_body<0, false, false, FX, FY, FM, FN, BN, CAP, GN_CPG, true>(p, acc, m0, n0, wm, wn, l31, lh, stat_part, nullptr, ev, img0, cls);
         return;
     }
     if constexpr (GN_CPG != 0) {
diff --git a/vista_amd/csrc/gemm_pipe.hip b/vista_amd/csrc/gemm_pipe.hip
--- a/vista_amd/csrc/gemm_pipe.hip
+++ b/vista_amd/csrc/gemm_pipe.hip
@@ -29,7 +29,7 @@
     constexpr int LN_OFF = 2 * PSTAGE, EV_OFF = LN_OFF + PBM * 8;
     constexpr int NTAPS = (AMODE == AMODE_CONV3X3) ? 9 : (AMODE == AMODE_TEMPORAL3) ? 3 : (AMODE == AMODE_UPCONV2X2) ? 4 : 1;
     constexpr bool UPC = (AMODE == AMODE_UPCONV2X2);
-    static_assert(!UPC || (EPI == EPI_LINEAR && !SPLIT && GN_CPG == 0), "the folded upsample convolution: plain LINEAR epilogue, one launch");
+    static_assert(!UPC || (EPI == EPI_LINEAR && !SPLIT && GN_NRES == 0), "the folded upsample convolution: plain LINEAR epilogue (GN_CPG: + statistics), one launch");
     constexpr bool WALK = (EPI == EPI_GEGLU);
     __shared__ __attribute__((aligned(16))) char smem[2 * PSTAGE + PBM * 8 + epi_vec_floats(PBN) * 4];
 #ifdef PIPE_TIMING
@@ -401,6 +401,12 @@
 #endif
 }
 
+inline bool pipe_prefetch_ok(const VkGemmDesc* d, int ntiles) {
+    return ntiles <= 256 && d->K >= 3 * BK && (d->lda % 64) == 0 && (((size_t)d->A) & 127) == 0;
+}
+
+inline int gn_unit_of(const VkGemmDesc* d) { return d->gn_unit > 0 ? d->gn_unit : d->N / 32; }
+
 template <int AMODE, int EPI>
 int pipe_launch(const VkGemmDesc* d, hipStream_t stream, int ksplit) {
     const int tilesN = d->N / PBN, tilesM = (d->m_end - d->m_begin + PBM - 1) / PBM;
@@ -420,16 +426,28 @@
         if (d->gnstat_out) {
             const int nres = (d->res1 != nullptr) + (d->res2 != nullptr);
 #define VK_PIPE_GN(CPG, NR) hipLaunchKernelGGL((gemm_pipe_kernel<AMODE, EPI, false, false, CPG, NR>), dim3(grid), dim3(PNT), 0, stream, *d, 1)
-            if (d->N == 320) { if (nres == 0) VK_PIPE_GN(10, 0); else VK_PIPE_GN(10, 1); }
-            else if (d->N == 640) { if (nres == 0) VK_PIPE_GN(20, 0); else VK_PIPE_GN(20, 1); }
+            const int unit = gn_unit_of(d);
+            if (unit == 10) { if (nres == 0) VK_PIPE_GN(10, 0); else VK_PIPE_GN(10, 1); }
+            else if (unit == 20) { if (nres == 0) VK_PIPE_GN(20, 0); else VK_PIPE_GN(20, 1); }
             else { if (nres == 0) VK_PIPE_GN(40, 0); else VK_PIPE_GN(40, 1); }
 #undef VK_PIPE_GN
             VK_CHECK_LAUNCH();
             return VK_OK;
         }
     }
+    if constexpr (EPI == EPI_LINEAR && AMODE == AMODE_DENSE) {
+        if (d->gnstat_out) {
+#define VK_PIPE_GN(U) hipLaunchKernelGGL((gemm_pipe_kernel<AMODE, EPI, true, false, U, 1, false>), dim3(grid), dim3(PNT), 0, stream, *d, 1)
+            if (d->gn_unit == 10) VK_PIPE_GN(10);
+            else if (d->gn_unit == 20) VK_PIPE_GN(20);
+            else VK_PIPE_GN(40);
+#undef VK_PIPE_GN
+            VK_CHECK_LAUNCH();
+            return VK_OK;
+        }
+    }
     if constexpr (AMODE == AMODE_DENSE) {
-        if (ntiles <= 256 && d->K >= 3 * BK && (d->lda % 64) == 0 && (((size_t)d->A) & 127) == 0) {
+        if (pipe_prefetch_ok(d, ntiles)) {
             if (nt_a) hipLaunchKernelGGL((gemm_pipe_kernel<AMODE, EPI, true, false, 0, 0, true>), dim3(grid), dim3(PNT), 0, stream, *d, 1);
             else hipLaunchKernelGGL((gemm_pipe_kernel<AMODE, EPI, false, false, 0, 0, true>), dim3(grid), dim3(PNT), 0, stream, *d, 1);
             VK_CHECK_LAUNCH();
@@ -452,8 +470,8 @@
 }
 
 int upconv_fit(const VkGemmDesc* d) {
-    if (d->epi != EPI_LINEAR || d->out_f32 || (d->N % PBN) != 0 || d->mx8_out || d->A2 || d->res1 || d->res2 || d->rowvec2 || d->gnstat_out || d->rowstat_out ||
-        d->ln_stats || d->act || d->alt_cols_from || d->halo_prev || d->halo_next)
+    if (d->epi != EPI_LINEAR || d->out_f32 || (d->N % PBN) != 0 || d->mx8_out || d->A2 || d->res1 || d->res2 || d->rowvec2 || (d->gnstat_out && d->gn_unit <= 0) ||
+        d->rowstat_out || d->ln_stats || d->act || d->alt_cols_from || d->halo_prev || d->halo_next)
         return 0;
     if (d->m_begin != 0 || (d->m_end != 0 && d->m_end != d->M)) return 0;
     VkGemmDesc q = *d;
@@ -466,7 +484,13 @@
 int upconv_launch(const VkGemmDesc* d, hipStream_t stream) {
     const VkGemmDesc q = upconv_class_desc(d);
     const int tilesN = q.N / PBN, tilesM = (q.M + PBM - 1) / PBM;
-    hipLaunchKernelGGL((gemm_pipe_kernel<AMODE_UPCONV2X2, EPI_LINEAR, false, false>), dim3(4 * tilesM * tilesN), dim3(PNT), 0, stream, q, 1);
+    const dim3 grid(4 * tilesM * tilesN);
+    if (d->gnstat_out) {
+        if (d->gn_unit == 10) hipLaunchKernelGGL((gemm_pipe_kernel<AMODE_UPCONV2X2, EPI_LINEAR, false, false, 10>), grid, dim3(PNT), 0, stream, q, 1);
+        else if (d->gn_unit == 20) hipLaunchKernelGGL((gemm_pipe_kernel<AMODE_UPCONV2X2, EPI_LINEAR, false, false, 20>), grid, dim3(PNT), 0, stream, q, 1);
+        else hipLaunchKernelGGL((gemm_pipe_kernel<AMODE_UPCONV2X2, EPI_LINEAR, false, false, 40>), grid, dim3(PNT), 0, stream, q, 1);
+    } else
+    hipLaunchKernelGGL((gemm_pipe_kernel<AMODE_UPCONV2X2, EPI_LINEAR, false, false>), grid, dim3(PNT), 0, stream, q, 1);
     VK_CHECK_LAUNCH();
     return VK_OK;
 }
@@ -494,21 +518,31 @@
 }
 
 extern "C" int vk_gemm_pipe_gnstat_ok(const VkGemmDesc* d, int ksplit) {
-    if (!vk_gemm_pipe_fit(d) || ksplit != 1 || d->epi != EPI_LINEAR || d->out_f32) return 0;
-    if (d->amode != AMODE_CONV3X3 && d->amode != AMODE_TEMPORAL3) return 0;
+    if (d->gn_unit < 0 || ksplit != 1 || d->epi != EPI_LINEAR || d->out_f32) return 0;
+    if (d->amode == AMODE_UPCONV2X2 && d->gn_unit == 0) return 0;
+    VkGemmDesc q = *d;
+    q.gnstat_out = nullptr;
+    if (!vk_gemm_pipe_fit(&q)) return 0;
     if (d->N != 320 && d->N != 640 && d->N != 1280) return 0;
+    const int unit = gn_unit_of(d);
+    if (unit != d->N / 32 && (unit != d->N / 64 || unit < 10)) return 0;
+    if (d->amode == AMODE_DENSE) {
+        if (d->gn_unit == 0 || (d->res1 != nullptr) == (d->res2 != nullptr)) return 0;
+    } else if (d->amode == AMODE_UPCONV2X2) {
+        if (((d->H * d->Wd) % 64) != 0 || d->gn_rows != 4 * d->H * d->Wd) return 0;
+    } else if (d->amode != AMODE_CONV3X3 && d->amode != AMODE_TEMPORAL3) return 0;
     if (d->ln_stats || d->mx8_out || d->act || d->rowstat_out || (d->res1 && d->res2)) return 0;
     if (d->gn_rows <= 0 || (d->gn_rows % 64) != 0 || (d->M % d->gn_rows) != 0) return 0;
     if (d->m_begin != 0 || (d->m_end != 0 && d->m_end != d->M)) return 0;
-    return 1;
+    return 2 * d->N / unit;
 }
 
 extern "C" int vk_gemm_pipe_launch(const VkGemmDesc* d, void* stream_, int ksplit) {
     hipStream_t stream = (hipStream_t)stream_;
     if (!vk_gemm_pipe_fit(d)) return VK_EINVAL;
+    if (d->gnstat_out && !vk_gemm_pipe_gnstat_ok(d, ksplit)) return VK_EINVAL;
     if (d->amode == AMODE_UPCONV2X2) return ksplit == 1 ? upconv_launch(d, stream) : VK_EINVAL;
     if (ksplit > 1 && (d->epi != EPI_LINEAR || !d->splitk_ws || d->ln_stats || d->rowstat_out || d->act)) return VK_EINVAL;
-    if (d->gnstat_out && !vk_gemm_pipe_gnstat_ok(d, ksplit)) return VK_EINVAL;
     if (d->amode == AMODE_DENSE) return d->epi == EPI_GEGLU ? pipe_launch<AMODE_DENSE, EPI_GEGLU>(d, stream, ksplit) : pipe_launch<AMODE_DENSE, EPI_LINEAR>(d, stream, ksplit);
     if (d->amode == AMODE_CONV3X3) return pipe_launch<AMODE_CONV3X3, EPI_LINEAR>(d, stream, ksplit);
     if (d->amode == AMODE_TEMPORAL3) return pipe_launch<AMODE_TEMPORAL3, EPI_LINEAR>(d, stream, ksplit);
diff --git a/vista_amd/csrc/norm.hip b/vista_amd/csrc/norm.hip
--- a/vista_amd/csrc/norm.hip
+++ b/vista_amd/csrc/norm.hip
@@ -153,10 +153,11 @@
 }
 
 constexpr int GN_FOLD_MAX = 256;
-template <bool NTL, bool NTS, bool FOLD, bool PIVOT>
+struct GnUnitArgs { const float* part2; int nu1, u1, nu2, u2; };
+template <bool NTL, bool NTS, int FOLD, bool PIVOT>
 __global__ void gn_apply_kernel(const uint16_t* __restrict__ x, const uint16_t* __restrict__ x2, int C1, uint16_t* __restrict__ y, const float* __restrict__ gamma,
                                 const float* __restrict__ beta, const float* __restrict__ stats, int S, int C, int CG, int R,
-                                int frames_per_group, float inv_cnt, float eps, int do_silu, int tok_per_wg, int nparts) {
+                                int frames_per_group, float inv_cnt, float eps, int do_silu, int tok_per_wg, int nparts, const GnUnitArgs ua) {
     __shared__ float fold_red[FOLD ? 4 : 1][64];
     __shared__ float fold_tot[64];
     const int tid = threadIdx.x;
@@ -165,7 +166,27 @@
     const int tok1 = min(tok0 + tok_per_wg, S);
     const int chunk = tid % CG, r = tid / CG;
     const float* st = stats + (size_t)(img / frames_per_group) * 64;
-    if constexpr (FOLD) {
+    if constexpr (FOLD == 2) {
+        const int cpg = C >> 5, c1 = ua.nu1 * ua.u1;
+        for (int idx = tid; idx < 256; idx += blockDim.x) {
+            const int v = idx & 63, j = idx >> 6, g = v & 31, sq = v >> 5;
+            const int lo = g * cpg, hi = lo + cpg;
+            const int a0 = min(lo, c1) / ua.u1, a1 = min(hi, c1) / ua.u1;
+            const int b0 = ua.part2 ? (max(lo, c1) - c1) / ua.u2 : 0, b1 = ua.part2 ? (max(hi, c1) - c1) / ua.u2 : 0;
+            const float* s1 = stats + (size_t)img * nparts * 2 * ua.nu1 + sq * ua.nu1;
+            const float* s2 = ua.part2 ? ua.part2 + (size_t)img * nparts * 2 * ua.nu2 + sq * ua.nu2 : nullptr;
+            float a = 0.f;
+            for (int i = j; i < nparts; i += 4) {
+                for (int u = a0; u < a1; ++u) a += s1[(size_t)i * 2 * ua.nu1 + u];
+                for (int u = b0; u < b1; ++u) a += s2[(size_t)i * 2 * ua.nu2 + u];
+            }
+            fold_red[j][v] = a;
+        }
+        __syncthreads();
+        if (tid < 64) fold_tot[tid] = (fold_red[0][tid] + fold_red[1][tid]) + (fold_red[2][tid] + fold_red[3][tid]);
+        __syncthreads();
+        st = fold_tot;
+    } else if constexpr (FOLD == 1) {
         const float* src = stats + (size_t)(img / frames_per_group) * nparts * 64;
         for (int idx = tid; idx < 256; idx += blockDim.x) {
             const int v = idx & 63, j = idx >> 6;
@@ -522,7 +543,7 @@
 }
 
 int gn_apply(const void* x, const void* x2, int C1, void* y, const float* gamma, const float* beta, const float* sums, int32_t n_img, int32_t S,
-             int32_t C, int32_t frames_per_group, float count, float eps, int32_t silu, void* stream_, int fold_nparts = 0, bool pivot = false) {
+             int32_t C, int32_t frames_per_group, float count, float eps, int32_t silu, void* stream_, int fold_nparts = 0, bool pivot = false, const GnUnitArgs* units = nullptr) {
     hipStream_t stream = (hipStream_t)stream_;
     GnGeom g;
     if (!x || !y || !gamma || !beta || !sums || count <= 0.f || !gn_geom(n_img, S, C, frames_per_group, g)) return VK_EINVAL;
@@ -534,18 +555,25 @@
     if (fold_nparts < 0 || fold_nparts > GN_FOLD_MAX) return VK_EINVAL;
     if (pivot && (y == x || y == x2)) return VK_EINVAL;
 #define VK_GN_APPLY_(NL, NS, FO, PV) hipLaunchKernelGGL((gn_apply_kernel<NL, NS, FO, PV>), grid, dim3(g.threads), 0, stream, (const uint16_t*)x, (const uint16_t*)x2, C1, \
-                                                       (uint16_t*)y, gamma, beta, sums, S, C, g.CG, g.R, frames_per_group, 1.f / count, eps, silu, tok_per_wg, fold_nparts)
+                                                       (uint16_t*)y, gamma, beta, sums, S, C, g.CG, g.R, frames_per_group, 1.f / count, eps, silu, tok_per_wg, fold_nparts, ua)
 #define VK_GN_APPLY(NL, NS, FO) do { if (pivot) VK_GN_APPLY_(NL, NS, FO, GN_PIVOT); else VK_GN_APPLY_(NL, NS, FO, false); } while (0)
-    if (fold_nparts > 0) {
-        if (nt_mode == 3) VK_GN_APPLY(true, true, true);
-        else if (nt_mode == 2) VK_GN_APPLY(false, true, true);
-        else if (nt_mode == 1) VK_GN_APPLY(true, false, true);
-        else VK_GN_APPLY(false, false, true);
+    const GnUnitArgs ua = units ? *units : GnUnitArgs{nullptr, 0, 0, 0, 0};
+    if (units) {
+        if (pivot || fold_nparts <= 0 || frames_per_group != 1) return VK_EINVAL;
+        if (nt_mode == 3) VK_GN_APPLY_(true, true, 2, false);
+        else if (nt_mode == 2) VK_GN_APPLY_(false, true, 2, false);
+        else if (nt_mode == 1) VK_GN_APPLY_(true, false, 2, false);
+        else VK_GN_APPLY_(false, false, 2, false);
+    } else if (fold_nparts > 0) {
+        if (nt_mode == 3) VK_GN_APPLY(true, true, 1);
+        else if (nt_mode == 2) VK_GN_APPLY(false, true, 1);
+        else if (nt_mode == 1) VK_GN_APPLY(true, false, 1);
+        else VK_GN_APPLY(false, false, 1);
     } else {
-        if (nt_mode == 3) VK_GN_APPLY(true, true, false);
-        else if (nt_mode == 2) VK_GN_APPLY(false, true, false);
-        else if (nt_mode == 1) VK_GN_APPLY(true, false, false);
-        else VK_GN_APPLY(false, false, false);
+        if (nt_mode == 3) VK_GN_APPLY(true, true, 0);
+        else if (nt_mode == 2) VK_GN_APPLY(false, true, 0);
+        else if (nt_mode == 1) VK_GN_APPLY(true, false, 0);
+        else VK_GN_APPLY(false, false, 0);
     }
 #undef VK_GN_APPLY
 #undef VK_GN_APPLY_
@@ -571,6 +599,23 @@
                                                 void* stream_) {
     if (!partial || nchunks <= 0 || frames_per_group <= 0 || (long long)frames_per_group * nchunks > GN_FOLD_MAX) return VK_EINVAL;
     return gn_apply(x, nullptr, 0, y, gamma, beta, partial, n_img, S, C, frames_per_group, count, eps, silu, stream_, frames_per_group * nchunks);
+}
+
+extern "C" int vk_groupnorm_apply_units_bf16(const void* x, const void* x2, int32_t C1, void* y, const float* gamma, const float* beta, const float* part1,
+                                             int32_t unit1, const float* part2, int32_t unit2, int32_t n_img, int32_t S, int32_t C, int32_t nchunks, float eps,
+                                             int32_t silu, void* stream_) {
+    if (!part1 || nchunks <= 0 || nchunks > GN_FOLD_MAX || C <= 0 || (C % 32) != 0 || unit1 <= 0 || (x2 == nullptr) != (part2 == nullptr)) return VK_EINVAL;
+    if (x2 ? (C1 <= 0 || C1 >= C || unit2 <= 0 || (C1 % 8) != 0) : C1 != C) return VK_EINVAL;
+    if (!aligned_to(part1, 4) || !aligned_to(part2, 4) || (C1 % unit1) != 0 || (x2 && ((C - C1) % unit2) != 0)) return VK_EINVAL;
+    const int cpg = C / 32;
+    for (int g = 0; g < 32; ++g) {
+        const int lo = g * cpg, hi = lo + cpg;
+        const int l1 = lo < C1 ? lo : C1, h1 = hi < C1 ? hi : C1, l2 = (lo > C1 ? lo : C1) - C1, h2 = (hi > C1 ? hi : C1) - C1;
+        if ((l1 % unit1) != 0 || (h1 % unit1) != 0 || (x2 && ((l2 % unit2) != 0 || (h2 % unit2) != 0))) return VK_EINVAL;
+    }
+    const GnUnitArgs ua{part2, C1 / unit1, unit1, x2 ? (C - C1) / unit2 : 0, x2 ? unit2 : 1};
+    const float count = (float)cpg * (float)S;
+    return gn_apply(x, x2, x2 ? C1 : 0, y, gamma, beta, part1, n_img, S, C, 1, count, eps, silu, stream_, nchunks, false, &ua);
 }
 
 extern "C" int vk_groupnorm_finalize_partials(float* partial, float* sums, int32_t n_img, int32_t nchunks, int32_t frames_per_group, void* stream_) {
diff --git a/vista_amd/modules/diffusionmodules/openaimodel.py b/vista_amd/modules/diffusionmodules/openaimodel.py
--- a/vista_amd/modules/diffusionmodules/openaimodel.py
+++ b/vista_amd/modules/diffusionmodules/openaimodel.py
@@ -14,7 +14,7 @@
 
 class TimestepEmbedSequential(nn.Sequential, TimestepBlock):
 
-    def forward(self, x, emb_silu, context=None, frame_idx=None, num_frames=None, H=None, W=None, shard=None, full=None):
+    def forward(self, x, emb_silu, context=None, frame_idx=None, num_frames=None, H=None, W=None, shard=None, full=None, in_gn=None, out_gn=None):
         from ..video_attention import SpatialVideoTransformer
         from .video_model import VideoResBlock
         layers = list(self)
@@ -22,12 +22,13 @@
         for i, layer in enumerate(layers):
             if isinstance(layer, VideoResBlock):
                 x_gn = ops.GnPartials() if i + 1 < len(layers) and isinstance(layers[i + 1], SpatialVideoTransformer) else None
-                x = layer(x, emb_silu, num_frames, H, W, shard=shard, full=full, out_gn=x_gn)
+                x = layer(x, emb_silu, num_frames, H, W, shard=shard, full=full, x_gn=in_gn if i == 0 else None,
+                          out_gn=out_gn if i + 1 == len(layers) else x_gn)
             elif isinstance(layer, SpatialVideoTransformer):
-                x = layer(x, context, frame_idx, num_frames, H, W, shard=shard, full=full, x_gn=x_gn)
+                x = layer(x, context, frame_idx, num_frames, H, W, shard=shard, full=full, x_gn=x_gn, out_gn=out_gn if i + 1 == len(layers) else None)
                 x_gn = None
             elif isinstance(layer, (Upsample, Downsample)):
-                x, H, W = layer(x, H, W)
+                x, H, W = layer(x, H, W, gn=out_gn if i + 1 == len(layers) else None)
             else:
                 raise TypeError(f"unexpected layer {type(layer).__name__} in TimestepEmbedSequential")
         return x, H, W
@@ -50,16 +51,16 @@
             return ops.pack_upconv2x2(self.conv.weight, self.conv.bias, device=dev)
         return ops.pack_conv3x3(self.conv.weight, self.conv.bias, device=dev)
 
-    def forward(self, x, H, W):
+    def forward(self, x, H, W, gn=None):
         assert x.shape[-1] == self.channels
         pw = self.packed()
         if pw.classes == 4:
             if ops.upconv2x2_fits(x, pw, x.shape[0], H, W):
-                return ops.upconv2x2(x, pw, x.shape[0], H, W)
+                return ops.upconv2x2(x, pw, x.shape[0], H, W, gn=gn)
             if self._nine is None or self._nine[1] is not pw:
                 object.__setattr__(self, "_nine", (ops.pack_conv3x3(self.conv.weight, self.conv.bias, device=x.device), pw))
             pw = self._nine[0]
-        out, Ho, Wo = ops.conv3x3(x, pw, x.shape[0], H, W, ups=2)
+        out, Ho, Wo = ops.conv3x3(x, pw, x.shape[0], H, W, ups=2, gn=gn)
         return out, Ho, Wo
 
 
@@ -76,9 +77,9 @@
     def _pack(self, dev):
         return ops.pack_conv3x3(self.op.weight, self.op.bias, device=dev)
 
-    def forward(self, x, H, W):
+    def forward(self, x, H, W, gn=None):
         assert x.shape[-1] == self.channels
-        out, Ho, Wo = ops.conv3x3(x, self.packed(), x.shape[0], H, W, stride=2)
+        out, Ho, Wo = ops.conv3x3(x, self.packed(), x.shape[0], H, W, stride=2, gn=gn)
         return out, Ho, Wo
 
 
@@ -170,7 +171,7 @@
             h = ops.conv_t3_fp8(h8, hs, pk["conv1_8"], T, S, rowvec=emb_out)
             h8, hs = ops.groupnorm_fp8(h, gn2.weight, gn2.bias, gn2.eps, True, fpg)
             return ops.conv_t3_fp8(h8, hs, pk["conv2_8"], T, S, alpha=out_alpha, res2=x, beta=1.0)
-        h = gnorm(x, gn1, x_gn) if xb is None else ops.groupnorm_cat(x, xb, gn1.weight, gn1.bias, gn1.eps, silu=True)
+        h = gnorm(x, gn1, x_gn) if xb is None else ops.groupnorm_cat(x, xb, gn1.weight, gn1.bias, gn1.eps, silu=True, gn=x_gn)
         mid_gn = ops.GnPartials()
         if self.dims == 2:
             h, _, _ = ops.conv3x3(h, pk["conv1"], n_img, H, W, rowvec=emb_out, gn=mid_gn)
diff --git a/vista_amd/modules/diffusionmodules/sampling.py b/vista_amd/modules/diffusionmodules/sampling.py
--- a/vista_amd/modules/diffusionmodules/sampling.py
+++ b/vista_amd/modules/diffusionmodules/sampling.py
@@ -204,7 +204,7 @@
         from .. import attention as _att
         if ctx is None:
             ctx, y, mask = self.ctx2, self.y2, self.mask2
-        switches = (tuple(sorted(_att.FP8.items())), _att.FF_FUSED, _att.QKV_SPLIT, _att.Q_LOG2, ops.TILE_CFG, ops.GN_EPI,
+        switches = (tuple(sorted(_att.FP8.items())), _att.FF_FUSED, _att.QKV_SPLIT, _att.Q_LOG2, ops.TILE_CFG, ops.GN_EPI, ops.GN_UNITS, ops.GN_DENSE_MIN_N,
                     None if self.unet_shard is None else getattr(self.unet_shard, "a2a_chunks", None))
         key = (tuple(net_in.shape), n_ts, tuple(ctx.shape), tuple(y.shape), tuple(mask.shape), self.T, self.H, self.W,
                None if self.unet_shard is None else id(self.unet_shard), str(net_in.device), switches, slot)
diff --git a/vista_amd/modules/diffusionmodules/video_model.py b/vista_amd/modules/diffusionmodules/video_model.py
--- a/vista_amd/modules/diffusionmodules/video_model.py
+++ b/vista_amd/modules/diffusionmodules/video_model.py
@@ -58,9 +58,9 @@
         pk["alpha"] = self.time_mixer.alpha_value()
         return pk
 
-    def forward(self, x, emb_silu, num_frames, H, W, shard=None, full=None, out_gn=None):
+    def forward(self, x, emb_silu, num_frames, H, W, shard=None, full=None, out_gn=None, x_gn=None):
         mid = ops.GnPartials()
-        x = super().forward(x, emb_silu, H, W, out_gn=mid)
+        x = super().forward(x, emb_silu, H, W, x_gn=x_gn, out_gn=mid)
         alpha = self.packed()["alpha"]
         if shard is None:
             return self.time_stack(x, emb_silu, H, W, T=num_frames, out_alpha=1.0 - alpha, x_gn=mid, out_gn=out_gn)
@@ -314,22 +314,37 @@
                                "ctx_s": ops.linear(ctx, pk["ctx_s"], out_f32=True) if "ctx_s" in pk else None,
                                "ctx_t": ops.linear(clip_ctx, pk["ctx_t"], out_f32=True) if "ctx_t" in pk else None}
         try:
+            from ..attention import FP8
+            units = not FP8["conv"]
             hs = []
-            h = tokens
+            h, h_gn = tokens, None
             for module in self.input_blocks:
-                h, H, W = module(h, emb_silu, context=ctx, H=H, W=W, **kw)
-                hs.append(h)
-            h, H, W = self.middle_block(h, emb_silu, context=ctx, H=H, W=W, **kw)
+                out_gn = ops.GnUnits() if units else None
+                h, H, W = module(h, emb_silu, context=ctx, H=H, W=W, in_gn=h_gn, out_gn=out_gn, **kw)
+                hs.append((h, out_gn))
+                h_gn = out_gn
+            mid_gn = ops.GnUnits() if units else None
+            h, H, W = self.middle_block(h, emb_silu, context=ctx, H=H, W=W, in_gn=h_gn, out_gn=mid_gn, **kw)
+            h_gn = mid_gn
             for module in self.output_blocks:
-                h, H, W = module((h, hs.pop()), emb_silu, context=ctx, H=H, W=W, **kw)
+                skip, skip_gn = hs.pop()
+                half = bool(hs) and _out_width(module) == 2 * hs[-1][0].shape[-1]
+                out_gn = ops.GnUnits(half=half) if units and (not hs or (hs[-1][1] is not None and hs[-1][1].t is not None)) else None
+                h, H, W = module((h, skip), emb_silu, context=ctx, H=H, W=W, in_gn=(h_gn, skip_gn) if units else None, out_gn=out_gn, **kw)
+                h_gn = out_gn
         finally:
             self._emb_tls.table = None
         gn = self.out[0]
-        h = ops.groupnorm(h, gn.weight, gn.bias, gn.eps, silu=True)
+        h = ops.groupnorm(h, gn.weight, gn.bias, gn.eps, silu=True, gn=h_gn)
         out, _, _ = ops.conv3x3(h, pk["out"], tokens.shape[0], H, W, out_f32=True)
         return out
 
 
+def _out_width(module):
+    last = list(module)[-1]
+    return last.in_channels if hasattr(last, "time_pos_embed") else last.out_channels
+
+
 class _InputConv(TimestepEmbedSequential, Packable):
 
     def __init__(self, in_channels, model_channels):
@@ -338,6 +353,6 @@
     def _pack(self, dev):
         return ops.pack_conv3x3(self[0].weight, self[0].bias, cin_pad=CIN_PAD, device=dev)
 
-    def forward(self, x, emb_silu, context=None, frame_idx=None, num_frames=None, H=None, W=None, shard=None, full=None):
-        out, H, W = ops.conv3x3(x, self.packed(), x.shape[0], H, W)
+    def forward(self, x, emb_silu, context=None, frame_idx=None, num_frames=None, H=None, W=None, shard=None, full=None, in_gn=None, out_gn=None):
+        out, H, W = ops.conv3x3(x, self.packed(), x.shape[0], H, W, gn=out_gn)
         return out, H, W
diff --git a/vista_amd/modules/video_attention.py b/vista_amd/modules/video_attention.py
--- a/vista_amd/modules/video_attention.py
+++ b/vista_amd/modules/video_attention.py
@@ -111,7 +111,7 @@
                 "tpe2": ops.pack_linear(self.time_pos_embed[2].weight, self.time_pos_embed[2].bias, dev),
                 "alpha": self.time_mixer.alpha_value()}
 
-    def forward(self, x, context, frame_idx, T, H, W, shard=None, full=None, x_gn=None):
+    def forward(self, x, context, frame_idx, T, H, W, shard=None, full=None, x_gn=None, out_gn=None):
         pk = self.packed()
         n_img, S, C = x.shape
         x_in = x
@@ -152,5 +152,5 @@
                         shard.to_frames_end(pnd, out)
                     h = out.view(-1, C)
                 st = ops.rowstats(h) if i != last else None
-        out = ops.linear(h, pk["proj_out"], res1=x_in)
+        out = ops.linear(h, pk["proj_out"], res1=x_in, gn=out_gn, gn_rows=S)
         return out.view(n_img, S, C)
diff --git a/vista_amd/ops.py b/vista_amd/ops.py
--- a/vista_amd/ops.py
+++ b/vista_amd/ops.py
@@ -360,6 +360,19 @@
         self.t, self.nchunks, self.rows, self.C = None, 0, 0, 0
 
 
+GN_UNITS = int(os.environ.get("VISTA_GN_UNITS", "1"))
+GN_DENSE_MIN_N = int(os.environ.get("VISTA_GN_DENSE_MIN_N", "640"))
+
+
+class GnUnits(GnPartials):
+
+    __slots__ = ("half", "unit")
+
+    def __init__(self, half=False):
+        super().__init__()
+        self.half, self.unit = bool(half), 0
+
+
 def _prepare(desc):
     desc.tile_cfg = TILE_CFG
     if ROW_RANGE is not None:
@@ -374,6 +387,10 @@
 def _ask_gn(d, gn, rows_per_image, device):
     if gn is None or not GN_EPI or ROW_RANGE is not None:
         return
+    if isinstance(gn, GnUnits):
+        if not GN_UNITS or d.N % 64 or (d.amode == AMODE_DENSE and d.N < GN_DENSE_MIN_N):
+            return
+        gn.unit = d.gn_unit = d.N // (64 if gn.half else 32)
     d.gn_rows = int(rows_per_image)
     _prepare(d)
     slots = _lib.load().vk_gemm_gnstat_fit(C.byref(d))
@@ -443,7 +460,7 @@
 
 
 def linear(x, pw, *, out=None, out_f32=False, rowvec=None, rows_per_vec=0, res1=None, res2=None, alpha=1.0, beta=0.0, rowvec2=None,
-           x2=None, ln=None, emit_stats=False, act=None, mx8_cols=0, alt_cols_from=0):
+           x2=None, ln=None, emit_stats=False, act=None, mx8_cols=0, alt_cols_from=0, gn=None, gn_rows=0):
     x2d, lda = _rows2d(x, "x")
     M = x2d.shape[0]
     k_in = x2d.shape[1]
@@ -482,6 +499,8 @@
             raise ValueError("linear: act must be None or 'gelu' (exact-erf GELU in the LINEAR epilogue)")
         d.act = 1
     d.alt_cols_from = int(alt_cols_from)
+    if gn is not None and not (emit_stats or mx8_cols or pw.geglu or out_f32):
+        _ask_gn(d, gn, gn_rows, x.device)
     stats = _gemm(d, emit_stats, x.device)
     if mx is not None:
         return out, mx[0], mx[1]
@@ -607,7 +626,7 @@
     return _lib.load().vk_gemm_tile_choice(C.byref(d)) > 0
 
 
-def upconv2x2(x, pw, n_img, H, W, rowvec=None, out=None):
+def upconv2x2(x, pw, n_img, H, W, rowvec=None, out=None, gn=None):
     cin = x.shape[-1]
     _dense(x, "x", BF16, pw.wt.get_device(), 16, n_img * H * W * cin)
     if pw.classes != 4 or pw.K != 4 * cin:
@@ -616,6 +635,9 @@
     if out is None:
         out = torch.empty((M, pw.N), dtype=BF16, device=x.device)
     d, stream = _upconv_desc(x, pw, n_img, H, W, rowvec, out)
+    _ask_gn(d, gn, 4 * H * W, x.device)
+    if UPCONV_CLASS_FASTEST:
+        d.tile_cfg |= 8
     check(_lib.load().vk_gemm_bf16(C.byref(d), stream), "vk_gemm_bf16 (folded upsample convolution)")
     return (out.view(n_img, 4 * H * W, pw.N) if out.is_contiguous() else out), 2 * H, 2 * W
 
@@ -993,6 +1015,24 @@
     return out
 
 
+def gn_unit_map(c1, u1, c2, u2):
+    C = c1 + c2
+    if C % 32 or u1 <= 0 or c1 % u1 or (c2 and (u2 <= 0 or c2 % u2)):
+        return None
+    w, out = C // 32, []
+    for g in range(32):
+        lo, hi = g * w, (g + 1) * w
+        l1, h1, l2, h2 = min(lo, c1), min(hi, c1), max(lo, c1) - c1, max(hi, c1) - c1
+        if l1 % u1 or h1 % u1 or (c2 and (l2 % u2 or h2 % u2)):
+            return None
+        out.append((range(l1 // u1, h1 // u1), range(l2 // u2, h2 // u2) if c2 else range(0)))
+    return out
+
+
+def gn_units_tile(c1, u1, c2, u2):
+    return gn_unit_map(c1, u1, c2, u2) is not None
+
+
 def _gn_partials_ok(gn, n_img, S, Cc):
     if gn is None or gn.t is None:
         return False
@@ -1011,6 +1051,12 @@
         out = torch.empty_like(x)
     else:
         _dense(out, "out", BF16, x.get_device(), 16, n_img * S * Cc)
+    if isinstance(gn, GnUnits):
+        if frames_per_group == 1 and _gn_partials_ok(gn, n_img, S, Cc) and gn.nchunks <= _lib.load().vk_groupnorm_fold_max():
+            check(_lib.load().vk_groupnorm_apply_units_bf16(_p(x), None, Cc, _p(out), _p(gamma), _p(beta), _p(gn.t), gn.unit, None, 0, n_img, S, Cc, gn.nchunks,
+                                                            float(eps), 1 if silu else 0, _stream()), "vk_groupnorm_apply_units_bf16")
+            return out
+        gn = None
     if _gn_partials_ok(gn, n_img, S, Cc):
         lib = _lib.load()
         count = float(Cc // 32) * float(S) * float(frames_per_group)
@@ -1032,7 +1078,7 @@
     return out
 
 
-def groupnorm_cat(a, b, gamma, beta, eps, silu, frames_per_group=1):
+def groupnorm_cat(a, b, gamma, beta, eps, silu, frames_per_group=1, gn=None):
     if a.dim() != 3 or b.dim() != 3 or a.shape[:2] != b.shape[:2]:
         raise ValueError("groupnorm_cat: contiguous (n_img, S, C) inputs with equal n_img, S required")
     n_img, S, c1 = a.shape
@@ -1041,6 +1087,13 @@
     _dense(b, "b", BF16, a.get_device(), 16, n_img * S * c2)
     _affine(gamma, beta, c1 + c2, a.get_device())
     out = torch.empty((n_img, S, c1 + c2), dtype=BF16, device=a.device)
+    if gn is not None and frames_per_group == 1 and GN_UNITS:
+        ga, gb = gn
+        if (isinstance(ga, GnUnits) and isinstance(gb, GnUnits) and _gn_partials_ok(ga, n_img, S, c1) and _gn_partials_ok(gb, n_img, S, c2)
+                and ga.nchunks <= _lib.load().vk_groupnorm_fold_max() and gn_units_tile(c1, ga.unit, c2, gb.unit)):
+            check(_lib.load().vk_groupnorm_apply_units_bf16(_p(a), _p(b), c1, _p(out), _p(gamma), _p(beta), _p(ga.t), ga.unit, _p(gb.t), gb.unit, n_img, S,
+                                                            c1 + c2, ga.nchunks, float(eps), 1 if silu else 0, _stream()), "vk_groupnorm_apply_units_bf16")
+            return out
     ws = torch.empty(((n_img // frames_per_group) + n_img * ((S + 31) // 32)) * 64, dtype=F32, device=a.device)
     check(_lib.load().vk_groupnorm_silu_cat_bf16(_p(a), _p(b), _p(out), _p(gamma), _p(beta), _p(ws), n_img, S, c1, c2, frames_per_group,
                                                  float(eps), 1 if silu else 0, _stream()), "vk_groupnorm_silu_cat_bf16")
```

Result: no change. 6.490 steps/s (median of 6 runs) (+0.3%).
